# tataganesh/Query-Efficient-Approx-to-improve-OCR

Measured on AMD Instinct MI355X. Metric: patch-images/sec UNet->CRNN->CTC fwd+bwd, 32x128 grey, higher is better.
Workload: dtype f32 (GEMMs as scaled 2 x fp16 split products — three fp16 MFMAs per fp32 multiply-add — fp32 accumulate); 1 GPU; BASELINE configs[2]: full minibatch step of train_nn_area.py:212-287 — Phase A (UNet eval fwd, TopKCER k = 5 % of the minibatch, inner_limit = 4 jitter replicas fused in the batch dim, CRNN train-BN fwd+bwd, Adam(CRNN)) + Phase B (UNet train-BN -> CRNN BN-eval -> CTC mean + MSE -> backward -> Adam(UNet)) + greedy decode -> CER -> update_cer (:290-304) on synthetic POS-style 32x128 patches; batch_per_gpu=2048, global_batch=2048, full_step=True, crnn_wgrad=True, parallelism=dp1, hipgraph=False

## Files before the change

include/qea_hip.h:

```cpp
#ifndef QEA_HIP_H
#define QEA_HIP_H
#include <stddef.h>
#include <stdint.h>

#ifdef __cplusplus
extern "C" {
#endif

#define QEA_OK 0
#define QEA_ERR_INVALID (-1)
#define QEA_ERR_LAUNCH (-2)
#define QEA_ERR_WORKSPACE (-3)

int qea_version(void);
const char* qea_last_error(void);

#define QEA_PROF_CONV_IGEMM 0
#define QEA_PROF_CONV_WGRAD 1
#define QEA_PROF_LSTM_STEP 2
#define QEA_PROF_NCLASS 3
int qea_prof_enable(int klass, int on);
int qea_prof_reset(void);
int qea_prof_read(int klass, double* ms, double* flops, double* bytes, int64_t* launches);
int qea_prof_read_launches(int klass, double* ms, double* flops, int64_t capacity, int64_t* count);
#define QEA_PROF_TAG_HALO_BF3(cin_chunk, cout_group, stats) (24000 + ((cin_chunk) == 64 ? 1000 : 0) + (cout_group) + ((stats) ? 500 : 0))
int qea_prof_read_tagged(int klass, int32_t tag, double* ms, double* flops, double* bytes, int64_t* launches);
int qea_prof_read_split_bf16(int klass, double* flops);
int qea_prof_read_split_f16(int klass, double* flops);

#define QEA_MFMA_SPLIT_BF16 0
#define QEA_MFMA_F32 1
int qea_set_mfma_mode(int mode);

#define QEA_OUT_NHWC 0
#define QEA_OUT_TBC 1
#define QEA_OUT_CONVT 2

typedef struct qea_conv_desc {
  const float* x;
  const float* w;
  float* y;
  const float* scale;
  const float* bias;
  const float* mask;
  int32_t B, H, W, Cin;
  int32_t OH, OW, N;
  int32_t KH, KW, pad_h, pad_w, stride_h, stride_w;
  int32_t ldx, ldy, ldmask;
  int32_t relu;
  int32_t accumulate;
  int32_t out_mode;
  int32_t tile;
  const void* x_planes;
  const void* w_planes;
  double* stats;
  const void* w_frag_planes;
  const float* x_absmax;
  float* y_absmax;
  float* pool_y;
  int32_t ldpool;
  int32_t pool_kw;
  float* pool_absmax;
  const float* bst_y;
  int32_t ldbst;
  const double* bst_stat64;
  const float* bst_scale;
  const float* bst_shift;
} qea_conv_desc;

int qea_conv_igemm(const qea_conv_desc* d, void* stream);
int qea_conv_igemm_uses_split_bf16(const qea_conv_desc* d);
int qea_conv_igemm_stats_blocks(const qea_conv_desc* d);
int qea_conv_igemm_can_pool(const qea_conv_desc* d, int32_t kw);
int qea_conv_igemm_wants_frag_planes(const qea_conv_desc* d);
size_t qea_pack_frag_planes_f16_1x1_bytes(int32_t N, int32_t K);
int qea_pack_frag_planes_f16_1x1(const float* w, int32_t N, int32_t K, const float* wmax, void* planes, void* stream);
int qea_absmax(const float* x, int32_t ld, int64_t M, int32_t C, float* out, void* stream);
size_t qea_pack_frag_planes_f16_bytes(int32_t N, int32_t Cin);
size_t qea_split_planes_f16_bytes(int64_t M, int32_t C);
int qea_split_planes_f16(const float* x, int32_t ld, int64_t M, int32_t C, const float* xmax, void* planes, void* stream);
int qea_pack_frag_planes_f16(const float* w, int32_t N, int32_t Cin, const float* wmax, void* planes, void* stream);
size_t qea_pack_frag_planes_bytes(int32_t N, int32_t Cin);
int qea_pack_frag_planes(const float* w, int32_t N, int32_t Cin, void* planes, void* stream);

size_t qea_split_planes_bytes(int64_t M, int32_t C);
int qea_split_planes(const float* x, int32_t ld, int64_t M, int32_t C, void* planes, void* stream);

typedef struct qea_wgrad_desc {
  const float* p;
  const float* q;
  float* dw;
  void* workspace;
  size_t workspace_bytes;
  int32_t B, PH, PW, QH, QW, R, C;
  int32_t KH, KW, pad_h, pad_w, stride_h, stride_w;
  int32_t ldp, ldq;
  int32_t accumulate;
  int32_t splits;
  int32_t tile;
  const float* p_absmax;
  const float* q_absmax;
  float* dbias;
} qea_wgrad_desc;

int qea_conv_wgrad_fuses_bias(const qea_wgrad_desc* d);
int qea_conv_wgrad_wants_absmax(const qea_wgrad_desc* d);
size_t qea_conv_wgrad_workspace_bytes(const qea_wgrad_desc* d);
int qea_conv_wgrad(const qea_wgrad_desc* d, void* stream);

size_t qea_colreduce_workspace_bytes(int64_t M, int32_t C);
int qea_bn_train_stats(const float* y, int32_t ldy, int64_t M, int32_t C, const float* gamma, const float* beta,
                       float eps, float momentum, float* running_mean, float* running_var, float* mean_out,
                       float* invstd_out, float* scale_out, float* shift_out, double* stat64, void* workspace,
                       size_t workspace_bytes, void* stream);
#define QEA_BN_PARTIAL_SCRATCH_ROWS 256
int qea_bn_train_stats_from_partials(const double* partials, int32_t blocks, int64_t M, int32_t C, const float* gamma,
                                     const float* beta, float eps, float momentum, float* running_mean, float* running_var,
                                     float* mean_out, float* invstd_out, float* scale_out, float* shift_out, double* stat64,
                                     void* stream);
int qea_bn_eval_coeff(int32_t C, const float* gamma, const float* beta, const float* running_mean,
                      const float* running_var, float eps, const float* conv_bias, float* mean_out,
                      float* invstd_out, float* scale_out, float* shift_out, void* stream);
int qea_bn_apply(const float* y, int32_t ldy, float* a, int32_t lda, int64_t M, int32_t C, const float* scale,
                 const float* shift, int32_t relu, float* absmax_out, void* stream);
int qea_bn_bwd(const float* da, int32_t ldda, const float* a, int32_t lda, const float* relu_scale,
               const float* relu_shift, const float* y, int32_t ldy, int64_t M, int32_t C, const float* gamma, const float* mean, const float* invstd, const double* stat64,
               int32_t training, float* dgamma, float* dbeta, int32_t accumulate_param_grads, float* dy,
               int32_t lddy, void* workspace, size_t workspace_bytes, float* absmax_out, void* stream);
int qea_bn_bwd_pool(const float* da, int32_t ldda, const float* dpool, int32_t lddp, int32_t kw, const float* relu_scale,
                    const float* relu_shift, const float* y, int32_t ldy, int32_t B, int32_t H, int32_t W, int32_t C, const float* gamma,
                    const float* mean, const float* invstd, const double* stat64, int32_t training, float* dgamma, float* dbeta,
                    int32_t accumulate_param_grads, float* dy, int32_t lddy, void* workspace, size_t workspace_bytes, float* absmax_out,
                    void* stream);
int qea_bn_bwd_from_partials(const double* partials, int32_t blocks, const float* da, int32_t ldda, const float* relu_scale,
                             const float* relu_shift, const float* y, int32_t ldy, int64_t M, int32_t C, const float* gamma,
                             const float* mean, const float* invstd, const double* stat64, int32_t training, float* dgamma, float* dbeta,
                             int32_t accumulate_param_grads, float* dy, int32_t lddy, void* workspace, size_t workspace_bytes,
                             float* absmax_out, void* stream);
int qea_colsum(const float* x, int32_t ldx, int64_t M, int32_t C, float* out, int32_t accumulate, void* workspace,
               size_t workspace_bytes, void* stream);

int qea_maxpool_fwd(const float* x, int32_t ldx, float* y, int32_t ldy, int32_t B, int32_t H, int32_t W, int32_t C,
                    int32_t kh, int32_t kw, float* absmax_out, void* stream);
int qea_bn_apply_pool(const float* y, int32_t ldy, float* a, int32_t lda, float* pooled, int32_t ldp, int32_t B, int32_t H, int32_t W,
                      int32_t C, const float* scale, const float* shift, int32_t relu, int32_t kh, int32_t kw, float* absmax_a,
                      float* absmax_pooled, void* stream);
int qea_maxpool_bwd(const float* x, int32_t ldx, const float* dy, int32_t lddy, float* dx, int32_t lddx, int32_t B,
                    int32_t H, int32_t W, int32_t C, int32_t kh, int32_t kw, int32_t relu_mask, int32_t accumulate,
                    float* absmax_out, void* stream);

int qea_transpose2d(const float* in, float* out, int32_t R, int32_t Cc, void* stream);
int qea_filter_flip_transpose(const float* w, float* wt, int32_t Co, int32_t Ci, int32_t KH, int32_t KW, void* stream);

int qea_conv_c1_fwd(const float* x, const float* w, const float* bias, float* y, int32_t ldy, int32_t B, int32_t H,
                    int32_t W, int32_t Co, int32_t relu, void* stream);
int qea_conv_c1_fwd_pool(const float* x, const float* w, const float* bias, float* y, int32_t ldy, float* pooled, int32_t ldp, int32_t B,
                         int32_t H, int32_t W, int32_t Co, int32_t relu, float* absmax_pooled, void* stream);
size_t qea_conv_c1_pool_bwd_workspace_bytes(int32_t B, int32_t H, int32_t W, int32_t Co, int32_t need_dx);
int qea_conv_c1_pool_bwd(const float* x, const float* w, const float* bias, float* dpool, int32_t lddp, float* dw, float* db, float* dx,
                         int32_t B, int32_t H, int32_t W, int32_t Co, int32_t accumulate, void* workspace, size_t workspace_bytes, void* stream);
size_t qea_conv_c1_wgrad_workspace_bytes(int32_t B, int32_t H, int32_t W, int32_t Co);
int qea_conv_c1_wgrad(const float* x, const float* dy, int32_t lddy, float* dw, float* db, int32_t B, int32_t H,
                      int32_t W, int32_t Co, int32_t accumulate, void* workspace, size_t workspace_bytes,
                      void* stream);
int qea_conv_c1_dgrad(const float* dy, int32_t lddy, const float* w, float* dx, int32_t B, int32_t H, int32_t W,
                      int32_t Co, int32_t accumulate, void* stream);

int qea_head_fwd(const float* x, int32_t ldx, const float* w, const float* b, float* y, int64_t M, int32_t C,
                 void* stream);
size_t qea_head_bwd_workspace_bytes(int64_t M, int32_t C);
int qea_head_bwd(const float* x, int32_t ldx, const float* y, const float* dyy, const float* w, float* dx,
                 int32_t lddx, float* dw, float* db, int32_t accumulate, int64_t M, int32_t C, void* workspace,
                 size_t workspace_bytes, void* stream);

int qea_lstm_pack_whh(const float* w_hh, float* packed_fwd, float* packed_bwd, void* stream);
int qea_lstm_layer_fwd(float* gates, float* c, float* y, const float* packed_fwd, int32_t T, int32_t B, void* stream);
int qea_lstm_layer_bwd(float* gates, const float* c, const float* dy, const float* packed_bwd, float* dc_scratch,
                       int32_t T, int32_t B, void* stream);
size_t qea_lstm_pack_whh_split_bytes(void);
int qea_lstm_pack_whh_split(const float* w_hh, void* planes_fwd, void* planes_bwd, void* stream);
int qea_lstm_layer_fwd_split(float* gates, float* c, float* y, const void* planes_fwd, int32_t T, int32_t B, void* stream);
int qea_lstm_layer_bwd_split(float* gates, const float* c, const float* dy, const void* planes_bwd, float* dc_scratch,
                             int32_t T, int32_t B, void* stream);

size_t qea_lstm_seq_pack_bytes(void);
size_t qea_lstm_seq_workspace_bytes(int32_t B);
int qea_lstm_seq_pack(const float* w_hh, void* planes_fwd, void* planes_bwd, const float* w_absmax, void* stream);
int qea_lstm_seq_fwd(float* gates, float* c, float* y, const void* planes_fwd, const float* w_absmax, int32_t T, int32_t B,
                     void* workspace, float* y_absmax, void* stream);
int qea_lstm_seq_bwd(float* gates, const float* c, const float* dy, const void* planes_bwd, const float* w_absmax, int32_t T,
                     int32_t B, void* workspace, float* dgates_absmax, void* stream);
int qea_lstm_seq_timeout_index(int32_t B, int32_t backward);

typedef struct qea_wform_job {
  const float* src;
  void* dst;
  const float* amax;
  int32_t kind, a, b, c, d;
} qea_wform_job;
int qea_weight_forms_multi(const qea_wform_job* jobs, int32_t n, void* stream);

int qea_log_softmax_fwd(const float* x, int32_t ldx, float* y, int32_t ldy, int64_t M, int32_t C, void* stream);
int qea_log_softmax_bwd(const float* g, int32_t ldg, const float* lp, int32_t ldlp, float* dx, int32_t lddx, int64_t M,
                        int32_t C, int32_t Cpad, int32_t nan_scrub, void* stream);

size_t qea_ctc_workspace_bytes(int32_t T, int32_t N, int32_t S_max);
int qea_ctc_loss(const float* lp, int32_t ld_t, int32_t ld_n, const int32_t* targets, const int64_t* target_offsets,
                 const int32_t* input_lengths, const int32_t* target_lengths, int32_t T, int32_t N, int32_t C,
                 int32_t blank, int32_t S_max, int32_t reduction, float grad_scale, float* nll, float* loss,
                 float* grad, int32_t gld_t, int32_t gld_n, void* workspace, size_t workspace_bytes, void* stream);

int qea_adam_step(float* p, const float* g, float* m, float* v, int64_t n, float lr, float beta1, float beta2,
                  float eps, float weight_decay, int64_t step, float grad_scale, void* stream);
int qea_adam_step_capturable(float* p, const float* g, float* m, float* v, int64_t n, float lr, float beta1,
                             float beta2, float eps, float weight_decay, float* step, float* coef, float grad_scale,
                             void* stream);

int qea_jitter(const float* img, const float* sigma, float* out, float* noise_out, int32_t K, int32_t R, int32_t HW,
               float coef, uint64_t seed, uint64_t offset, void* stream);
int qea_jitter_apply(const float* img, const float* noise, float* out, int32_t K, int32_t R, int32_t HW, float coef,
                     void* stream);

int qea_topk_desc_stable(const float* keys, int32_t n, int32_t k, int64_t* idx_out, void* stream);

int qea_crop_pad_gather(const float* img, int32_t H, int32_t W, const int32_t* boxes, int32_t N, int32_t OH, int32_t OW,
                        float* out, void* stream);
int qea_crop_pad_scatter(const float* dout, const int32_t* boxes, int32_t N, int32_t OH, int32_t OW, float* dimg,
                         int32_t H, int32_t W, void* stream);

int qea_greedy_decode(const float* scores, int32_t ld_t, int32_t ld_n, int32_t T, int32_t N, int32_t C, int32_t blank,
                      int32_t* tokens, int32_t* lengths, void* stream);

int qea_ctc_beam_decode(const float* scores, int32_t ld_t, int32_t ld_n, int32_t T, int32_t N, int32_t C, int32_t blank, int32_t K,
                        int32_t* tokens, int32_t* lengths, double* beam_scores, void* stream);

int qea_ctc_beam_decode_lm(const float* scores, int32_t ld_t, int32_t ld_n, int32_t T, int32_t N, int32_t C, int32_t blank, int32_t K,
                           const double* lm_table, int32_t lm_context, int32_t* tokens, int32_t* lengths, double* ctc_scores,
                           double* total_scores, void* stream);

int qea_ctc_beam_decode_dfa(const float* scores, int32_t ld_t, int32_t ld_n, int32_t T, int32_t N, int32_t C, int32_t blank, int32_t K,
                            const int32_t* first, const int32_t* label, const int32_t* child, int32_t S, int32_t E, int32_t* tokens,
                            int32_t* lengths, double* beam_scores, int32_t* states, void* stream);

int qea_edit_distance(const int32_t* pred_tokens, int32_t ldp, const int32_t* pred_len, const int32_t* gt_tokens,
                      const int64_t* gt_offsets, const int32_t* gt_len, int32_t N, int32_t* out, void* stream);

size_t qea_facility_workspace_bytes(int32_t n, int32_t d);
int qea_facility_select(const double* x, int32_t n, int32_t d, int32_t k, int32_t* ranking_out, double* gain_out, void* workspace,
                        void* stream);
int qea_facility_status(const void* workspace, void* stream);

#define QEA_HISTORY_MAX_WINDOW 8
#define QEA_HISTORY_MAX_LEN 128
#define QEA_HISTORY_ATTN_MAX_TABLE 12288
#define QEA_HISTORY_ACT_SIGMOID 0
#define QEA_HISTORY_ACT_SOFTMAX 1
#define QEA_HISTORY_ACT_RELU 2
int qea_history_lev_weights(const int32_t* tokens, const int32_t* lens, const int32_t* count, int32_t n, int32_t W, float* out,
                            void* stream);
int qea_history_attn_weights(const int32_t* char_idx, const int32_t* count, int32_t n, int32_t W, int32_t n_chars,
                             const float* embedding, int32_t V1, int32_t E, const float* wq_weight, const float* wq_bias, int32_t Dq,
                             const float* coef_weight, const float* coef_bias, const float* positional_encodings, int32_t activation,
                             float* out, void* stream);

size_t qea_ctc_history_workspace_bytes(int32_t T, int32_t N, int32_t W, int32_t S_max);
int qea_ctc_history_loss(const float* lp, int32_t ld_t, int32_t ld_n, const int32_t* input_lengths, const int32_t* lens,
                         const int32_t* offs, const int32_t* chars, const int32_t* depth_n, const float* weights,
                         int32_t w_stride_n, int32_t w_stride_i, int32_t mean_by_length, int32_t T, int32_t N, int32_t C, int32_t W,
                         int32_t blank, int32_t S_max, float* loss, float* grad, int32_t gld_t, int32_t gld_n, float* nll,
                         void* workspace, size_t workspace_bytes, void* stream);

#define QEA_STRIP_ANCHOR_CENTRE 0
#define QEA_STRIP_ANCHOR_LEFT 1
int qea_strip_batch(const uint8_t* pixels, const int64_t* offset, const int32_t* h, const int32_t* w, int32_t n, const int64_t* idx,
                    int32_t B, int32_t OH, int32_t OW, int32_t anchor, const float* table, float* out, void* stream);

int qea_doc_crops_gather(const float* imgs, int32_t N, int32_t H, int32_t W, const int32_t* box, const int32_t* box_first, int32_t n_docs,
                         int32_t n_boxes, const int64_t* doc, const int32_t* strip_first, int32_t S, int32_t OH, int32_t OW, float* out,
                         void* stream);
int qea_doc_crops_scatter(const float* dout, int32_t S, int32_t OH, int32_t OW, const int32_t* box, const int32_t* box_first,
                          int32_t n_docs, int32_t n_boxes, const int64_t* doc, const int32_t* strip_first, float* dimg, int32_t N, int32_t H,
                          int32_t W, int32_t accumulate, void* stream);

#define QEA_SPREAD_WAVE_MAX_N 1536
#define QEA_SPREAD_LDS4_MAX_N 24576
#define QEA_SPREAD_LDS_MAX_N 32768
#define QEA_SPREAD_MAX_N (1 << 24)
size_t qea_spread_pick_workspace_bytes(int32_t n);
int qea_spread_pick(const float* est, int32_t n, const float* pts, int32_t k, int64_t* idx, void* workspace, void* stream);
int qea_seq_entropy(const float* lp, int64_t ld_t, int64_t ld_n, int32_t T, int32_t B, int32_t C, int32_t num_classes, float* out,
                    void* stream);

int qea_page_tiles_gather(const void* store, int32_t store_is_f32, int64_t store_elems, const int64_t* offset, const int32_t* h,
                          const int32_t* w, int32_t n_pages, const int32_t* tile, int32_t N, int32_t TH, int32_t TW, const float* table,
                          float* out, void* stream);
int qea_page_tiles_scatter(const float* tiles, int32_t N, int32_t TH, int32_t TW, const int32_t* tile, const int64_t* offset,
                           const int32_t* h, const int32_t* w, int32_t n_pages, int64_t store_elems, float* out_f32, uint8_t* out_u8,
                           void* stream);

#define QEA_BINARIZE_TILE_H 32
#define QEA_BINARIZE_TILE_W 64
#define QEA_BINARIZE_CHUNK 32768
#define QEA_BINARIZE_MAX_WINDOW 127
#define QEA_BINARIZE_MAX_PAGE_PIXELS (1 << 27)
int qea_binarize_sauvola(const void* store, int32_t store_is_f32, int64_t store_elems, const int64_t* offset, const int32_t* h,
                         const int32_t* w, int32_t n_pages, const int32_t* host_h, const int32_t* host_w, const int32_t* tile_first,
                         int32_t win, double k, double R, float* out_f32, uint8_t* out_u8, void* stream);
int qea_otsu_histogram(const void* store, int32_t store_is_f32, int64_t store_elems, const int64_t* offset, const int32_t* h,
                       const int32_t* w, int32_t n_pages, const int32_t* host_h, const int32_t* host_w, const int32_t* chunk_first,
                       uint32_t* hist, void* stream);
int qea_binarize_otsu(const void* store, int32_t store_is_f32, int64_t store_elems, const int64_t* offset, const int32_t* h,
                      const int32_t* w, int32_t n_pages, const int32_t* host_h, const int32_t* host_w, const int32_t* chunk_first,
                      const uint32_t* hist, float* out_f32, uint8_t* out_u8, int32_t* thresholds, void* stream);

#define QEA_CC_MAX_GAP 127
int qea_cc_label(const void* store, int32_t store_is_f32, int64_t store_elems, const int64_t* offset, const int32_t* h, const int32_t* w,
                 int32_t n_pages, const int32_t* host_h, const int32_t* host_w, const int32_t* tile_first, const uint8_t* ink_mask,
                 int32_t ink_max, int32_t connectivity, int32_t* labels, int32_t* area, void* stream);
int qea_cc_stats(const void* store, int32_t store_is_f32, int64_t store_elems, const int64_t* offset, const int32_t* h, const int32_t* w,
                 int32_t n_pages, const int32_t* host_h, const int32_t* host_w, const int32_t* tile_first, const int32_t* labels,
                 int32_t* area, void* stream);
int qea_cc_despeckle(const void* store, int32_t store_is_f32, int64_t store_elems, const int64_t* offset, const int32_t* h,
                     const int32_t* w, int32_t n_pages, const int32_t* host_h, const int32_t* host_w, const int32_t* tile_first,
                     const int32_t* labels, const int32_t* area, int32_t min_area, float* out_f32, uint8_t* out_u8, void* stream);
int qea_cc_smear(const void* store, int32_t store_is_f32, int64_t store_elems, const int64_t* offset, const int32_t* h, const int32_t* w,
                 int32_t n_pages, const int32_t* host_h, const int32_t* host_w, const int32_t* tile_first, const uint8_t* in_mask,
                 int32_t ink_max, int32_t gap, int32_t vertical, uint8_t* out_mask, void* stream);
int qea_cc_boxes(const void* store, int32_t store_is_f32, int64_t store_elems, const int64_t* offset, const int32_t* h, const int32_t* w,
                 int32_t n_pages, const int32_t* host_h, const int32_t* host_w, const int32_t* tile_first, const int32_t* labels,
                 const int32_t* roots, const int32_t* root_first, int32_t n_roots, int32_t* boxes, void* stream);

#define QEA_DESKEW_MAX_SIDE 32767
#define QEA_DESKEW_MAX_SLOPE 256
#define QEA_DESKEW_MAX_GAIN 10000
int qea_skew_strip_sums(const void* store, int32_t store_is_f32, int64_t store_elems, const int64_t* offset, const int32_t* h,
                        const int32_t* w, int32_t n_pages, const int32_t* host_h, const int32_t* host_w, const int32_t* ink_max_dev,
                        int32_t ink_max, uint8_t* C, void* stream);
int qea_skew_scores(const uint8_t* C, int64_t store_elems, const int64_t* offset, const int32_t* h, const int32_t* w, int32_t n_pages,
                    const int32_t* host_h, const int32_t* host_w, int32_t A, int64_t* scores, void* stream);
int qea_skew_pick(const int64_t* scores, int32_t n_pages, int32_t A, int32_t g, int32_t* slopes, void* stream);
int qea_deskew_rotate(const void* store, int32_t store_is_f32, int64_t store_elems, const int64_t* offset, const int32_t* h,
                      const int32_t* w, int32_t n_pages, const int32_t* host_h, const int32_t* host_w, const int32_t* tile_first,
                      const int32_t* slopes, const int32_t* table, int32_t A, int32_t nearest, int32_t fill, const float* norm,
                      float* out_f32, uint8_t* out_u8, void* stream);

#define QEA_WORD_STRIP_H 32
#define QEA_WORD_STRIP_MIN_W 64
#define QEA_WORD_STRIP_MAX_W 512
#define QEA_WORD_STRIP_MAX_BOXES (1 << 20)
#define QEA_WORD_STRIP_MAX_SIDE 32767
int qea_word_strips(const void* store, int32_t store_is_f32, int64_t store_elems, const int64_t* offset, const int32_t* h,
                    const int32_t* w, int32_t n_pages, const int32_t* boxes, int32_t n, int32_t OW, const float* norm, float* out,
                    void* stream);

#ifdef __cplusplus
}
#endif
#endif
```

query-efficient-approx-to-improve-ocr_amd/csrc/conv_c1.hip:

```cpp
#include "common.h"

namespace {

__global__ void conv_c1_fwd_kernel(const float* __restrict__ x, const float* __restrict__ w, const float* __restrict__ bias,
                                   float* __restrict__ y, int ldy, int B, int H, int W, int Co, int relu) {
  extern __shared__ __attribute__((aligned(16))) float sw[];
  for (int i = threadIdx.x; i < Co * 9; i += blockDim.x) {
    const int co = i / 9, tap = i - co * 9;
    sw[tap * Co + co] = w[i];
  }
  __syncthreads();
  const int cols = Co / 4;
  const long long n = (long long)B * H * W * cols;
  for (long long i = (long long)blockIdx.x * blockDim.x + threadIdx.x; i < n; i += (long long)gridDim.x * blockDim.x) {
    const int ct = (int)(i % cols);
    const long long pix = i / cols;
    const int pw = (int)(pix % W);
    const int ph = (int)((pix / W) % H);
    const float* xb = x + (pix - (long long)ph * W - pw);
    f32x4 acc = {0.f, 0.f, 0.f, 0.f};
    if (bias) acc = *reinterpret_cast<const f32x4*>(bias + ct * 4);
#pragma unroll
    for (int kh = 0; kh < 3; ++kh) {
      const int ih = ph + kh - 1;
#pragma unroll
      for (int kw = 0; kw < 3; ++kw) {
        const int iw = pw + kw - 1;
        float xv = 0.f;
        if ((unsigned)ih < (unsigned)H && (unsigned)iw < (unsigned)W) xv = xb[ih * W + iw];
        const f32x4 wv = *reinterpret_cast<const f32x4*>(sw + (kh * 3 + kw) * Co + ct * 4);
        acc += wv * xv;
      }
    }
    if (relu) {
#pragma unroll
      for (int k = 0; k < 4; ++k) acc[k] = fmaxf(acc[k], 0.f);
    }
    *reinterpret_cast<f32x4*>(y + pix * ldy + ct * 4) = acc;
  }
}

template <int COLS>
__global__ __launch_bounds__(256) void conv_c1_fwd4_kernel(const float* __restrict__ x, const float* __restrict__ w, const float* __restrict__ bias,
                                                           float* __restrict__ y, int ldy, int B, int H, int W, int relu) {
  constexpr int GPB = 256 / COLS;
  const int ct = threadIdx.x % COLS;
  f32x4 wr[9];
#pragma unroll
  for (int t = 0; t < 9; ++t)
#pragma unroll
    for (int k = 0; k < 4; ++k) wr[t][k] = w[(ct * 4 + k) * 9 + t];
  f32x4 bv = {0.f, 0.f, 0.f, 0.f};
  if (bias) bv = *reinterpret_cast<const f32x4*>(bias + ct * 4);
  const unsigned W4 = (unsigned)W >> 2;
  const unsigned groups = (unsigned)B * (unsigned)H * W4;
  const unsigned gstride = gridDim.x * GPB;
  for (unsigned g = blockIdx.x * GPB + threadIdx.x / COLS; g < groups; g += gstride) {
    const unsigned row = g / W4;
    const int pw0 = (int)(g - row * W4) * 4;
    const int ph = (int)(row % (unsigned)H);
    const float* xr = x + (size_t)row * W;
    float xv[3][6];
#pragma unroll
    for (int kh = 0; kh < 3; ++kh) {
      const bool rok = (unsigned)(ph + kh - 1) < (unsigned)H;
#pragma unroll
      for (int c = 0; c < 6; ++c) {
        const int iw = pw0 + c - 1;
        xv[kh][c] = (rok && (unsigned)iw < (unsigned)W) ? xr[(kh - 1) * W + iw] : 0.f;
      }
    }
    float* yo = y + ((size_t)row * W + pw0) * ldy + ct * 4;
#pragma unroll
    for (int j = 0; j < 4; ++j) {
      f32x4 acc = bv;
#pragma unroll
      for (int kh = 0; kh < 3; ++kh)
#pragma unroll
        for (int kw = 0; kw < 3; ++kw) acc += wr[kh * 3 + kw] * xv[kh][j + kw];
      if (relu) {
#pragma unroll
        for (int k = 0; k < 4; ++k) acc[k] = fmaxf(acc[k], 0.f);
      }
      *reinterpret_cast<f32x4*>(yo + (size_t)j * ldy) = acc;
    }
  }
}

template <int COLS>
__global__ __launch_bounds__(256) void conv_c1_fwd4_pool_kernel(const float* __restrict__ x, const float* __restrict__ w, const float* __restrict__ bias,
                                                                float* __restrict__ y, int ldy, float* __restrict__ pooled, int ldp, int B, int H,
                                                                int W, int relu, float* __restrict__ amax_p) {
  constexpr int GPB = 256 / COLS;
  const int ct = threadIdx.x % COLS;
  f32x4 wr[9];
#pragma unroll
  for (int t = 0; t < 9; ++t)
#pragma unroll
    for (int k = 0; k < 4; ++k) wr[t][k] = w[(ct * 4 + k) * 9 + t];
  f32x4 bv = {0.f, 0.f, 0.f, 0.f};
  if (bias) bv = *reinterpret_cast<const f32x4*>(bias + ct * 4);
  const unsigned W4 = (unsigned)W >> 2, H2 = (unsigned)H >> 1;
  const unsigned groups = (unsigned)B * H2 * W4;
  const unsigned gstride = gridDim.x * GPB;
  float pm = 0.f;
  for (unsigned g = blockIdx.x * GPB + threadIdx.x / COLS; g < groups; g += gstride) {
    const unsigned prow = g / W4;
    const int pw0 = (int)(g - prow * W4) * 4;
    const int ph = (int)(prow % H2) * 2;
    const size_t row = (size_t)prow * 2;
    const float* xr = x + row * W;
    float xv[4][6];
#pragma unroll
    for (int kh = 0; kh < 4; ++kh) {
      const bool rok = (unsigned)(ph + kh - 1) < (unsigned)H;
#pragma unroll
      for (int c = 0; c < 6; ++c) {
        const int iw = pw0 + c - 1;
        xv[kh][c] = (rok && (unsigned)iw < (unsigned)W) ? xr[(kh - 1) * W + iw] : 0.f;
      }
    }
    f32x4 o[2][4];
#pragma unroll
    for (int r = 0; r < 2; ++r)
#pragma unroll
      for (int j = 0; j < 4; ++j) {
        f32x4 acc = bv;
#pragma unroll
        for (int kh = 0; kh < 3; ++kh)
#pragma unroll
          for (int kw = 0; kw < 3; ++kw) acc += wr[kh * 3 + kw] * xv[r + kh][j + kw];
        if (relu) {
#pragma unroll
          for (int k = 0; k < 4; ++k) acc[k] = fmaxf(acc[k], 0.f);
        }
        o[r][j] = acc;
        if (y) *reinterpret_cast<f32x4*>(y + ((row + r) * W + pw0 + j) * ldy + ct * 4) = acc;
      }
#pragma unroll
    for (int q = 0; q < 2; ++q) {
      f32x4 m = {-INFINITY, -INFINITY, -INFINITY, -INFINITY};
#pragma unroll
      for (int r = 0; r < 2; ++r)
#pragma unroll
        for (int j = 0; j < 2; ++j)
#pragma unroll
          for (int k = 0; k < 4; ++k) {
            const float v = o[r][2 * q + j][k];
            m[k] = (v > m[k] || v != v) ? v : m[k];
          }
      *reinterpret_cast<f32x4*>(pooled + ((size_t)prow * (W >> 1) + (pw0 >> 1) + q) * ldp + ct * 4) = m;
#pragma unroll
      for (int k = 0; k < 4; ++k) pm = qea_amax_acc(pm, m[k]);
    }
  }
  qea_amax_commit_block(pm, amax_p);
}


__global__ __launch_bounds__(256) void conv_c1_wgrad_kernel(const float* __restrict__ x, const float* __restrict__ dy, int lddy, int B, int H,
                                                            int W, int Co, int rt_n, int rows_per_thread, float* __restrict__ ws) {
  extern __shared__ __attribute__((aligned(16))) float sacc[];
  const int cols = Co / 4;
  const int ct = threadIdx.x % cols, rt = threadIdx.x / cols;
  const long long M = (long long)B * H * W;
  f32x4 acc[10];
#pragma unroll
  for (int t = 0; t < 10; ++t) acc[t] = (f32x4){0.f, 0.f, 0.f, 0.f};
  if (rt < rt_n) {
    const long long r0 = (long long)blockIdx.x * rt_n * rows_per_thread;
    int pw = (int)((r0 + rt) % W);
    int ph = (int)(((r0 + rt) / W) % H);
    const int dph = rt_n / W, dpw = rt_n - dph * W;
    for (int j = 0; j < rows_per_thread; ++j) {
      const long long pix = r0 + (long long)j * rt_n + rt;
      if (pix >= M) break;
      if (j) {
        pw += dpw;
        ph += dph;
        if (pw >= W) {
          pw -= W;
          ++ph;
        }
        ph = ph >= H ? ph % H : ph;
      }
      const float* xb = x + (pix - (long long)ph * W - pw);
      const f32x4 g = *reinterpret_cast<const f32x4*>(dy + pix * lddy + ct * 4);
#pragma unroll
      for (int kh = 0; kh < 3; ++kh) {
        const int ih = ph + kh - 1;
#pragma unroll
        for (int kw = 0; kw < 3; ++kw) {
          const int iw = pw + kw - 1;
          float xv = 0.f;
          if ((unsigned)ih < (unsigned)H && (unsigned)iw < (unsigned)W) xv = xb[ih * W + iw];
          acc[kh * 3 + kw] += g * xv;
        }
      }
      acc[9] += g;
    }
#pragma unroll
    for (int t = 0; t < 10; ++t) *reinterpret_cast<f32x4*>(sacc + ((size_t)rt * 10 + t) * Co + ct * 4) = acc[t];
  }
  __syncthreads();
  for (int e = threadIdx.x; e < 10 * Co; e += blockDim.x) {
    float s = 0.f;
    for (int r = 0; r < rt_n; ++r) s += sacc[(size_t)r * 10 * Co + e];
    ws[(size_t)blockIdx.x * 10 * Co + e] = s;
  }
}

__global__ void conv_c1_wgrad_finalize_kernel(const float* __restrict__ ws, int nblk, int Co, float* dw, float* db, int accumulate) {
  const int e = blockIdx.x * (blockDim.x >> 6) + (threadIdx.x >> 6);
  if (e >= 10 * Co) return;
  const double s = qea_wave_partial_sum(ws, nblk, (size_t)10 * Co, e);
  if ((threadIdx.x & 63) != 0) return;
  const int tap = e / Co, co = e - tap * Co;
  if (tap < 9) {
    float* d = dw + co * 9 + tap;
    *d = accumulate ? *d + (float)s : (float)s;
  } else if (db) {
    db[co] = accumulate ? db[co] + (float)s : (float)s;
  }
}

template <bool NEED_T>
__global__ __launch_bounds__(256) void c1_pool_route_kernel(const float* __restrict__ x, const float* __restrict__ w, const float* __restrict__ bias,
                                                            float* __restrict__ g, int ldg, unsigned* __restrict__ idx, float* __restrict__ T, int B,
                                                            int H, int W) {
  constexpr int Co = 64;
  __shared__ __attribute__((aligned(16))) float Wl[Co * 12];
  for (int e = threadIdx.x; e < Co * 12; e += 256) {
    const int c = e / 12, t = e - c * 12;
    Wl[e] = t < 9 ? w[c * 9 + t] : (t == 9 && bias ? bias[c] : 0.f);
  }
  __syncthreads();
  const int OH = H >> 1, OW = W >> 1;
  const long long NW = (long long)B * OH * OW;
  const long long M = (long long)B * H * W;
  for (long long wi = (long long)blockIdx.x * 256 + threadIdx.x; wi < NW; wi += (long long)gridDim.x * 256) {
    const int ow = (int)(wi % OW);
    const int oh = (int)((wi / OW) % OH);
    const long long b = wi / ((long long)OW * OH);
    const int wy = oh * 2, wx = ow * 2;
    const float* xb = x + b * H * W;
    float xp[4][4];
#pragma unroll
    for (int r = 0; r < 4; ++r)
#pragma unroll
      for (int c = 0; c < 4; ++c) {
        const int iy = wy + r - 1, ix = wx + c - 1;
        xp[r][c] = ((unsigned)iy < (unsigned)H && (unsigned)ix < (unsigned)W) ? xb[iy * W + ix] : 0.f;
      }
    float Tacc[4][9];
    if (NEED_T) {
#pragma unroll
      for (int j = 0; j < 4; ++j)
#pragma unroll
        for (int t = 0; t < 9; ++t) Tacc[j][t] = 0.f;
    }
    float* grow = g + wi * ldg;
    unsigned* irow = idx + wi * (Co / 4);
#pragma unroll 2
    for (int c4 = 0; c4 < Co / 4; ++c4) {
      f32x4 gv = *reinterpret_cast<const f32x4*>(grow + c4 * 4);
      unsigned packed = 0;
#pragma unroll
      for (int k = 0; k < 4; ++k) {
        const float* wc = Wl + (c4 * 4 + k) * 12;
        const f32x4 w0 = *reinterpret_cast<const f32x4*>(wc), w1 = *reinterpret_cast<const f32x4*>(wc + 4), w2 = *reinterpret_cast<const f32x4*>(wc + 8);
        const float wt[9] = {w0[0], w0[1], w0[2], w0[3], w1[0], w1[1], w1[2], w1[3], w2[0]};
        float m = -INFINITY;
        int arg = 0;
#pragma unroll
        for (int j = 0; j < 4; ++j) {
          const int jr = j >> 1, jc = j & 1;
          float acc = w2[1];
#pragma unroll
          for (int kh = 0; kh < 3; ++kh)
#pragma unroll
            for (int kw = 0; kw < 3; ++kw) acc = __builtin_fmaf(wt[kh * 3 + kw], xp[jr + kh][jc + kw], acc);
          const float v = fmaxf(acc, 0.f);
          if (v > m || v != v) {
            m = v;
            arg = j;
          }
        }
        const float gm = (m > 0.f) ? gv[k] : 0.f;
        gv[k] = gm;
        packed |= (unsigned)arg << (8 * k);
        if (NEED_T) {
#pragma unroll
          for (int j = 0; j < 4; ++j) {
            const float mj = (arg == j) ? gm : 0.f;
#pragma unroll
            for (int t = 0; t < 9; ++t) Tacc[j][t] = __builtin_fmaf(mj, wt[t], Tacc[j][t]);
          }
        }
      }
      *reinterpret_cast<f32x4*>(grow + c4 * 4) = gv;
      irow[c4] = packed;
    }
    if (NEED_T) {
      const long long p0 = (b * H + wy) * (long long)W + wx;
#pragma unroll
      for (int t = 0; t < 9; ++t) {
        float* Tp = T + (long long)t * M;
        *reinterpret_cast<float2*>(Tp + p0) = make_float2(Tacc[0][t], Tacc[1][t]);
        *reinterpret_cast<float2*>(Tp + p0 + W) = make_float2(Tacc[2][t], Tacc[3][t]);
      }
    }
  }
}

__global__ __launch_bounds__(256) void c1_pool_wgrad_kernel(const float* __restrict__ x, const float* __restrict__ g, int ldg,
                                                            const unsigned char* __restrict__ idx, int B, int H, int W, int win_per_wave,
                                                            float* __restrict__ ws) {
  constexpr int Co = 64;
  const int c = threadIdx.x & 63;
  const int wave = __builtin_amdgcn_readfirstlane(threadIdx.x >> 6);
  const int OH = H >> 1, OW = W >> 1;
  const long long NW = (long long)B * OH * OW;
  const long long w0 = ((long long)blockIdx.x * 4 + wave) * win_per_wave;
  long long w1 = w0 + win_per_wave;
  if (w1 > NW) w1 = NW;
  float acc[10];
#pragma unroll
  for (int t = 0; t < 10; ++t) acc[t] = 0.f;
  float gq[4];
  int aq[4];
  auto load_group = [&](long long wi, float* gv, int* av) {
#pragma unroll
    for (int k = 0; k < 4; ++k) {
      gv[k] = g[(wi + k) * ldg + c];
      av[k] = idx[(wi + k) * Co + c];
    }
  };
  if (w0 < w1) load_group(w0, gq, aq);
  for (long long wi = w0; wi < w1; wi += 4) {
    float gn[4] = {0.f, 0.f, 0.f, 0.f};
    int an[4] = {0, 0, 0, 0};
    if (wi + 4 < w1) load_group(wi + 4, gn, an);
    const int ow = (int)(wi % OW);
    const int oh = (int)((wi / OW) % OH);
    const long long b = wi / ((long long)OW * OH);
    const int wy = oh * 2, wx = ow * 2;
    const float* xb = x + b * H * W;
    float xr[4][10];
#pragma unroll
    for (int r = 0; r < 4; ++r)
#pragma unroll
      for (int cc = 0; cc < 10; ++cc) {
        const int iy = wy + r - 1, ix = wx + cc - 1;
        xr[r][cc] = ((unsigned)iy < (unsigned)H && (unsigned)ix < (unsigned)W) ? xb[iy * W + ix] : 0.f;
      }
#pragma unroll
    for (int k = 0; k < 4; ++k) {
      const float gm = gq[k];
      const int arg = aq[k];
#pragma unroll
      for (int j = 0; j < 4; ++j) {
        const float mj = (arg == j) ? gm : 0.f;
        const int jr = j >> 1, jc = j & 1;
#pragma unroll
        for (int kh = 0; kh < 3; ++kh)
#pragma unroll
          for (int kw = 0; kw < 3; ++kw) acc[kh * 3 + kw] = __builtin_fmaf(mj, xr[jr + kh][2 * k + jc + kw], acc[kh * 3 + kw]);
      }
      acc[9] += gm;
    }
#pragma unroll
    for (int k = 0; k < 4; ++k) {
      gq[k] = gn[k];
      aq[k] = an[k];
    }
  }
  float* o = ws + ((size_t)blockIdx.x * 4 + wave) * 10 * Co;
#pragma unroll
  for (int t = 0; t < 10; ++t) o[t * Co + c] = acc[t];
}

__global__ void c1_pool_dx_kernel(const float* __restrict__ T, float* __restrict__ dx, int B, int H, int W, int accumulate) {
  const long long M = (long long)B * H * W;
  for (long long p = (long long)blockIdx.x * blockDim.x + threadIdx.x; p < M; p += (long long)gridDim.x * blockDim.x) {
    const int px = (int)(p % W);
    const int py = (int)((p / W) % H);
    float s = 0.f;
#pragma unroll
    for (int kh = 0; kh < 3; ++kh) {
      const int qy = py + 1 - kh;
#pragma unroll
      for (int kw = 0; kw < 3; ++kw) {
        const int qx = px + 1 - kw;
        if ((unsigned)qy < (unsigned)H && (unsigned)qx < (unsigned)W) s += T[(long long)(kh * 3 + kw) * M + p + (long long)(1 - kh) * W + (1 - kw)];
      }
    }
    dx[p] = accumulate ? dx[p] + s : s;
  }
}

template <int COLS>
__global__ __launch_bounds__(256) void conv_c1_dgrad_kernel(const float* __restrict__ dy, int lddy, const float* __restrict__ w,
                                                            float* __restrict__ dx, int B, int H, int W, int accumulate) {
  constexpr int Co = COLS * 4;
  const int ct = threadIdx.x % COLS;
  f32x4 wr[9];
#pragma unroll
  for (int t = 0; t < 9; ++t)
#pragma unroll
    for (int k = 0; k < 4; ++k) wr[t][k] = w[(ct * 4 + k) * 9 + t];
  const long long M = (long long)B * H * W;
  const long long n = M * COLS;
  const long long stride = (long long)gridDim.x * blockDim.x;
  for (long long i = (long long)blockIdx.x * blockDim.x + threadIdx.x; i < (n + stride - 1) / stride * stride; i += stride) {
    const bool live = i < n;
    const long long pix = live ? i / COLS : 0;
    const int pw = (int)(pix % W);
    const int ph = (int)((pix / W) % H);
    float s = 0.f;
    if (live) {
#pragma unroll
      for (int kh = 0; kh < 3; ++kh) {
        const int oh = ph + 1 - kh;
#pragma unroll
        for (int kw = 0; kw < 3; ++kw) {
          const int ow = pw + 1 - kw;
          if ((unsigned)oh < (unsigned)H && (unsigned)ow < (unsigned)W) {
            const f32x4 g = *reinterpret_cast<const f32x4*>(dy + (pix + (long long)(oh - ph) * W + (ow - pw)) * lddy + ct * 4);
            const f32x4 wv = wr[kh * 3 + kw];
            s += g[0] * wv[0] + g[1] * wv[1] + g[2] * wv[2] + g[3] * wv[3];
          }
        }
      }
    }
#pragma unroll
    for (int o = COLS / 2; o > 0; o >>= 1) s += __shfl_xor(s, o, 64);
    if (live && ct == 0) dx[pix] = accumulate ? dx[pix] + s : s;
  }
  (void)Co;
}

constexpr int C1D_TH = 8, C1D_TW = 64, C1D_HW = C1D_TW + 2, C1D_HP = (C1D_TH + 2) * C1D_HW;
template <int COLS>
__global__ __launch_bounds__(256) void conv_c1_dgrad_tile_kernel(const float* __restrict__ dy, int lddy, const float* __restrict__ w,
                                                                 float* __restrict__ dx, int H, int W, int tiles_x, int tiles_y, int accumulate) {
  __shared__ float T[C1D_HP * 9];
  __shared__ __attribute__((aligned(16))) float Wl[COLS * 9 * 4];
  for (int e = threadIdx.x; e < COLS * 36; e += 256) {
    const int k = e & 3, t = (e >> 2) % 9, c4 = e / 36;
    Wl[e] = w[(c4 * 4 + k) * 9 + t];
  }
  int bid = blockIdx.x;
  const int tx = bid % tiles_x;
  bid /= tiles_x;
  const int ty = bid % tiles_y;
  const int b = bid / tiles_y;
  const int x0 = tx * C1D_TW, y0 = ty * C1D_TH;
  const float* dyb = dy + (size_t)b * H * W * lddy;
  __syncthreads();
  for (int hq = threadIdx.x; hq < C1D_HP; hq += 256) {
    const int hy = hq / C1D_HW, hx = hq - hy * C1D_HW;
    const int iy = y0 + hy - 1, ix = x0 + hx - 1;
    float d[9];
#pragma unroll
    for (int t = 0; t < 9; ++t) d[t] = 0.f;
    if ((unsigned)iy < (unsigned)H && (unsigned)ix < (unsigned)W) {
      const float* row = dyb + ((size_t)iy * W + ix) * lddy;
#pragma unroll 4
      for (int c4 = 0; c4 < COLS; ++c4) {
        const f32x4 g = *reinterpret_cast<const f32x4*>(row + c4 * 4);
#pragma unroll
        for (int t = 0; t < 9; ++t) {
          const f32x4 wv = *reinterpret_cast<const f32x4*>(Wl + (c4 * 9 + t) * 4);
          d[t] += g[0] * wv[0] + g[1] * wv[1] + g[2] * wv[2] + g[3] * wv[3];
        }
      }
    }
#pragma unroll
    for (int t = 0; t < 9; ++t) T[hq * 9 + t] = d[t];
  }
  __syncthreads();
  float* dxb = dx + (size_t)b * H * W;
  for (int q = threadIdx.x; q < C1D_TH * C1D_TW; q += 256) {
    const int qy = q / C1D_TW, qx = q - qy * C1D_TW;
    const int oy = y0 + qy, ox = x0 + qx;
    if (oy >= H || ox >= W) continue;
    float sacc = 0.f;
#pragma unroll
    for (int kh = 0; kh < 3; ++kh)
#pragma unroll
      for (int kw = 0; kw < 3; ++kw) sacc += T[((qy + 2 - kh) * C1D_HW + qx + 2 - kw) * 9 + kh * 3 + kw];
    float* o = dxb + (size_t)oy * W + ox;
    *o = accumulate ? *o + sacc : sacc;
  }
}

template <int COLS>
__global__ __launch_bounds__(256) void head_fwd_kernel(const float* __restrict__ x, int ldx, const float* __restrict__ w,
                                                       const float* __restrict__ b, float* __restrict__ y, long long M) {
  const int ct = threadIdx.x % COLS;
  const f32x4 wv = *reinterpret_cast<const f32x4*>(w + ct * 4);
  const float bias = b[0];
  const long long n = M * COLS;
  const long long stride = (long long)gridDim.x * blockDim.x;
  for (long long i = (long long)blockIdx.x * blockDim.x + threadIdx.x; i < (n + stride - 1) / stride * stride; i += stride) {
    const bool live = i < n;
    const long long pix = live ? i / COLS : 0;
    float s = 0.f;
    if (live) {
      const f32x4 xv = *reinterpret_cast<const f32x4*>(x + pix * ldx + ct * 4);
      s = xv[0] * wv[0] + xv[1] * wv[1] + xv[2] * wv[2] + xv[3] * wv[3];
    }
#pragma unroll
    for (int o = COLS / 2; o > 0; o >>= 1) s += __shfl_xor(s, o, 64);
    if (live && ct == 0) y[pix] = 1.f / (1.f + expf(-(s + bias)));
  }
}

template <int COLS>
__global__ __launch_bounds__(256) void head_bwd_kernel(const float* __restrict__ x, int ldx, const float* __restrict__ y,
                                                       const float* __restrict__ dyy, const float* __restrict__ w, float* __restrict__ dx,
                                                       int lddx, long long M, double* __restrict__ ws) {
  constexpr int C = COLS * 4;
  constexpr int RT = 256 / COLS;
  __shared__ double sred[RT][C + 1];
  const int ct = threadIdx.x % COLS, rt = threadIdx.x / COLS;
  const f32x4 wv = *reinterpret_cast<const f32x4*>(w + ct * 4);
  double aw[4] = {0, 0, 0, 0}, ab = 0;
  const long long n = M * COLS;
  for (long long i = (long long)blockIdx.x * blockDim.x + threadIdx.x; i < n; i += (long long)gridDim.x * blockDim.x) {
    const long long pix = i / COLS;
    const float yy = y[pix];
    const float dz = dyy[pix] * yy * (1.f - yy);
    const f32x4 xv = *reinterpret_cast<const f32x4*>(x + pix * ldx + ct * 4);
    *reinterpret_cast<f32x4*>(dx + pix * lddx + ct * 4) = wv * dz;
#pragma unroll
    for (int k = 0; k < 4; ++k) aw[k] += (double)(dz * xv[k]);
    if (ct == 0) ab += (double)dz;
  }
#pragma unroll
  for (int k = 0; k < 4; ++k) sred[rt][ct * 4 + k] = aw[k];
  if (ct == 0) sred[rt][C] = ab;
  __syncthreads();
  for (int e = threadIdx.x; e <= C; e += blockDim.x) {
    double s = 0;
    for (int r = 0; r < RT; ++r) s += sred[r][e];
    ws[(size_t)blockIdx.x * (C + 1) + e] = s;
  }
}

__global__ void head_bwd_finalize_kernel(const double* __restrict__ ws, int nblk, int C, float* dw, float* db, int accumulate) {
  const int e = blockIdx.x * (blockDim.x >> 6) + (threadIdx.x >> 6);
  if (e > C) return;
  const double s = qea_wave_partial_sum(ws, nblk, (size_t)C + 1, e);
  if ((threadIdx.x & 63) != 0) return;
  float* d = (e < C) ? dw + e : db;
  *d = accumulate ? *d + (float)s : (float)s;
}

}

extern "C" int qea_conv_c1_fwd(const float* x, const float* w, const float* bias, float* y, int32_t ldy, int32_t B, int32_t H, int32_t W,
                               int32_t Co, int32_t relu, void* stream) {
  QEA_REQUIRE(x && w && y && B > 0 && H > 0 && W > 0 && Co > 0 && Co % 4 == 0 && ldy % 4 == 0 && ldy >= Co, "qea_conv_c1_fwd: bad arguments");
  const long long n = (long long)B * H * W * (Co / 4);
  if (W % 4 == 0 && (long long)B * H * W < 0x7fffffffLL && (Co == 32 || Co == 64 || Co == 128) && ((uintptr_t)y & 15) == 0 &&
      (!bias || ((uintptr_t)bias & 15) == 0)) {
    const int cols = Co / 4;
    const long long groups = (long long)B * H * (W / 4);
    const int grid = (int)((groups + 256 / cols - 1) / (256 / cols) > 16384 ? 16384 : (groups + 256 / cols - 1) / (256 / cols));
    hipStream_t s = (hipStream_t)stream;
    if (Co == 32) hipLaunchKernelGGL(conv_c1_fwd4_kernel<8>, dim3(grid), dim3(256), 0, s, x, w, bias, y, ldy, B, H, W, relu);
    else if (Co == 64) hipLaunchKernelGGL(conv_c1_fwd4_kernel<16>, dim3(grid), dim3(256), 0, s, x, w, bias, y, ldy, B, H, W, relu);
    else hipLaunchKernelGGL(conv_c1_fwd4_kernel<32>, dim3(grid), dim3(256), 0, s, x, w, bias, y, ldy, B, H, W, relu);
    QEA_CHECK_LAUNCH();
    return QEA_OK;
  }
  hipLaunchKernelGGL(conv_c1_fwd_kernel, dim3(qea_grid_for(n, 8192)), dim3(256), (size_t)Co * 9 * sizeof(float), (hipStream_t)stream, x, w, bias, y,
                     ldy, B, H, W, Co, relu);
  QEA_CHECK_LAUNCH();
  return QEA_OK;
}

extern "C" int qea_conv_c1_fwd_pool(const float* x, const float* w, const float* bias, float* y, int32_t ldy, float* pooled, int32_t ldp, int32_t B,
                                    int32_t H, int32_t W, int32_t Co, int32_t relu, float* absmax_pooled, void* stream) {
  QEA_REQUIRE(x && w && pooled && B > 0 && H > 0 && W > 0 && H % 2 == 0 && W % 4 == 0 && (Co == 32 || Co == 64 || Co == 128) && ldy % 4 == 0 &&
                  ldy >= Co && ldp % 4 == 0 && ldp >= Co && (long long)B * H * W < 0x7fffffffLL,
              "qea_conv_c1_fwd_pool: needs H %% 2 == 0, W %% 4 == 0, Co in {32, 64, 128}, fewer than 2^31 pixels");
  QEA_REQUIRE(((uintptr_t)y & 15) == 0 && ((uintptr_t)pooled & 15) == 0 && (!bias || ((uintptr_t)bias & 15) == 0), "qea_conv_c1_fwd_pool: 16-byte alignment");
  const int cols = Co / 4;
  const long long groups = (long long)B * (H / 2) * (W / 4);
  const long long blocks = (groups + 256 / cols - 1) / (256 / cols);
  const int grid = (int)(blocks > 16384 ? 16384 : blocks);
  hipStream_t s = (hipStream_t)stream;
  if (Co == 32) hipLaunchKernelGGL(conv_c1_fwd4_pool_kernel<8>, dim3(grid), dim3(256), 0, s, x, w, bias, y, ldy, pooled, ldp, B, H, W, relu, absmax_pooled);
  else if (Co == 64) hipLaunchKernelGGL(conv_c1_fwd4_pool_kernel<16>, dim3(grid), dim3(256), 0, s, x, w, bias, y, ldy, pooled, ldp, B, H, W, relu, absmax_pooled);
  else hipLaunchKernelGGL(conv_c1_fwd4_pool_kernel<32>, dim3(grid), dim3(256), 0, s, x, w, bias, y, ldy, pooled, ldp, B, H, W, relu, absmax_pooled);
  QEA_CHECK_LAUNCH();
  return QEA_OK;
}

static int c1_wgrad_geom(long long M, int Co, int* rt_n, int* rows_per_thread) {
  const int cols = Co / 4;
  *rt_n = 256 / cols;
  long long rpt = M / ((long long)(*rt_n) * 4096);
  rpt = rpt < 32 ? 32 : (rpt > 128 ? 128 : rpt);
  *rows_per_thread = (int)rpt;
  const long long per_block = (long long)(*rt_n) * rpt;
  return (int)((M + per_block - 1) / per_block);
}

extern "C" size_t qea_conv_c1_wgrad_workspace_bytes(int32_t B, int32_t H, int32_t W, int32_t Co) {
  if (B <= 0 || H <= 0 || W <= 0 || Co <= 0 || Co % 4 || Co / 4 > 256) return 0;
  int rt, rpt;
  const int grid = c1_wgrad_geom((long long)B * H * W, Co, &rt, &rpt);
  return (size_t)grid * 10 * Co * sizeof(float);
}

extern "C" int qea_conv_c1_wgrad(const float* x, const float* dy, int32_t lddy, float* dw, float* db, int32_t B, int32_t H, int32_t W,
                                 int32_t Co, int32_t accumulate, void* workspace, size_t workspace_bytes, void* stream) {
  QEA_REQUIRE(x && dy && dw && B > 0 && H > 0 && W > 0 && Co > 0 && Co % 4 == 0 && Co / 4 <= 256 && lddy % 4 == 0, "qea_conv_c1_wgrad: bad arguments");
  int rt, rpt;
  const int grid = c1_wgrad_geom((long long)B * H * W, Co, &rt, &rpt);
  QEA_REQUIRE(workspace && workspace_bytes >= (size_t)grid * 10 * Co * sizeof(float), "qea_conv_c1_wgrad: workspace too small");
  const size_t lds = (size_t)rt * 10 * Co * sizeof(float);
  QEA_REQUIRE(lds <= 160 * 1024, "qea_conv_c1_wgrad: Co too large for LDS");
  static bool attr = false;
  if (!attr) {
    (void)hipFuncSetAttribute((const void*)conv_c1_wgrad_kernel, hipFuncAttributeMaxDynamicSharedMemorySize, 160 * 1024);
    attr = true;
  }
  hipStream_t s = (hipStream_t)stream;
  hipLaunchKernelGGL(conv_c1_wgrad_kernel, dim3(grid), dim3(256), lds, s, x, dy, lddy, B, H, W, Co, rt, rpt, (float*)workspace);
  hipLaunchKernelGGL(conv_c1_wgrad_finalize_kernel, dim3(qea_cdiv(10 * Co, 4)), dim3(256), 0, s, (const float*)workspace, grid, Co, dw, db,
                     accumulate);
  QEA_CHECK_LAUNCH();
  return QEA_OK;
}

static long long c1pb_win_per_wave(long long NW) {
  long long wpw = (NW + 4 * 2048 - 1) / (4 * 2048);
  wpw = wpw < 16 ? 16 : wpw;
  return (wpw + 3) & ~3LL;
}

extern "C" size_t qea_conv_c1_pool_bwd_workspace_bytes(int32_t B, int32_t H, int32_t W, int32_t Co, int32_t need_dx) {
  if (B <= 0 || H <= 0 || W <= 0 || Co != 64 || H % 2 || W % 8) return 0;
  const long long NW = (long long)B * (H / 2) * (W / 2);
  const long long wpw = c1pb_win_per_wave(NW);
  const long long blocks = (NW + 4 * wpw - 1) / (4 * wpw);
  size_t b = ((size_t)NW * 64 + 255) & ~(size_t)255;
  if (need_dx) b += (size_t)9 * B * H * W * sizeof(float);
  b += (size_t)blocks * 4 * 640 * sizeof(float);
  return b;
}

extern "C" int qea_conv_c1_pool_bwd(const float* x, const float* w, const float* bias, float* dpool, int32_t lddp, float* dw, float* db, float* dx,
                                    int32_t B, int32_t H, int32_t W, int32_t Co, int32_t accumulate, void* workspace, size_t workspace_bytes,
                                    void* stream) {
  QEA_REQUIRE(x && w && dpool && B > 0 && H > 0 && W > 0 && H % 2 == 0 && W % 8 == 0 && Co == 64 && lddp % 4 == 0 && lddp >= Co &&
                  ((uintptr_t)dpool & 15) == 0 && ((uintptr_t)x & 7) == 0 && (long long)B * H * W < 0x7fffffffLL,
              "qea_conv_c1_pool_bwd: needs Co == 64, even H, W %% 8 == 0, 16-byte aligned dpool rows, fewer than 2^31 pixels");
  const size_t need = qea_conv_c1_pool_bwd_workspace_bytes(B, H, W, Co, dx != nullptr);
  QEA_REQUIRE(workspace && workspace_bytes >= need && ((uintptr_t)workspace & 255) == 0, "qea_conv_c1_pool_bwd: workspace of %zu bytes (256-byte aligned) required", need);
  const long long NW = (long long)B * (H / 2) * (W / 2);
  const long long wpw = c1pb_win_per_wave(NW);
  const long long blocks = (NW + 4 * wpw - 1) / (4 * wpw);
  char* wsb = (char*)workspace;
  unsigned* idx = (unsigned*)wsb;
  wsb += ((size_t)NW * 64 + 255) & ~(size_t)255;
  float* T = nullptr;
  if (dx) {
    T = (float*)wsb;
    wsb += (size_t)9 * B * H * W * sizeof(float);
  }
  float* part = (float*)wsb;
  hipStream_t s = (hipStream_t)stream;
  const int rgrid = qea_grid_for(NW, 8192);
  if (dx) hipLaunchKernelGGL(c1_pool_route_kernel<true>, dim3(rgrid), dim3(256), 0, s, x, w, bias, dpool, lddp, idx, T, B, H, W);
  else hipLaunchKernelGGL(c1_pool_route_kernel<false>, dim3(rgrid), dim3(256), 0, s, x, w, bias, dpool, lddp, idx, T, B, H, W);
  if (dw) {
    hipLaunchKernelGGL(c1_pool_wgrad_kernel, dim3((unsigned)blocks), dim3(256), 0, s, x, (const float*)dpool, lddp, (const unsigned char*)idx, B, H, W,
                       (int)wpw, part);
    hipLaunchKernelGGL(conv_c1_wgrad_finalize_kernel, dim3(qea_cdiv(10 * Co, 4)), dim3(256), 0, s, (const float*)part, (int)(blocks * 4), Co, dw, db,
                       accumulate);
  }
  if (dx) hipLaunchKernelGGL(c1_pool_dx_kernel, dim3(qea_grid_for((long long)B * H * W, 8192)), dim3(256), 0, s, (const float*)T, dx, B, H, W, 0);
  QEA_CHECK_LAUNCH();
  return QEA_OK;
}

extern "C" int qea_conv_c1_dgrad(const float* dy, int32_t lddy, const float* w, float* dx, int32_t B, int32_t H, int32_t W, int32_t Co,
                                 int32_t accumulate, void* stream) {
  QEA_REQUIRE(dy && w && dx && B > 0 && H > 0 && W > 0 && lddy % 4 == 0, "qea_conv_c1_dgrad: bad arguments");
  const long long n = (long long)B * H * W * (Co / 4);
  const int grid = qea_grid_for(n, 8192);
  hipStream_t s = (hipStream_t)stream;
  const int tiles_x = qea_cdiv(W, C1D_TW), tiles_y = qea_cdiv(H, C1D_TH);
  const long long tiles = (long long)B * tiles_x * tiles_y;
  if (tiles < 0x7fffffffLL && (Co == 32 || Co == 64 || Co == 128) && ((uintptr_t)dy & 15) == 0) {
    if (Co == 32) hipLaunchKernelGGL(conv_c1_dgrad_tile_kernel<8>, dim3((unsigned)tiles), dim3(256), 0, s, dy, lddy, w, dx, H, W, tiles_x, tiles_y, accumulate);
    else if (Co == 64) hipLaunchKernelGGL(conv_c1_dgrad_tile_kernel<16>, dim3((unsigned)tiles), dim3(256), 0, s, dy, lddy, w, dx, H, W, tiles_x, tiles_y, accumulate);
    else hipLaunchKernelGGL(conv_c1_dgrad_tile_kernel<32>, dim3((unsigned)tiles), dim3(256), 0, s, dy, lddy, w, dx, H, W, tiles_x, tiles_y, accumulate);
    QEA_CHECK_LAUNCH();
    return QEA_OK;
  }
  switch (Co) {
    case 32: hipLaunchKernelGGL(conv_c1_dgrad_kernel<8>, dim3(grid), dim3(256), 0, s, dy, lddy, w, dx, B, H, W, accumulate); break;
    case 64: hipLaunchKernelGGL(conv_c1_dgrad_kernel<16>, dim3(grid), dim3(256), 0, s, dy, lddy, w, dx, B, H, W, accumulate); break;
    case 128: hipLaunchKernelGGL(conv_c1_dgrad_kernel<32>, dim3(grid), dim3(256), 0, s, dy, lddy, w, dx, B, H, W, accumulate); break;
    default: qea_set_error("qea_conv_c1_dgrad: Co=%d not in {32,64,128}", Co); return QEA_ERR_INVALID;
  }
  QEA_CHECK_LAUNCH();
  return QEA_OK;
}

extern "C" int qea_head_fwd(const float* x, int32_t ldx, const float* w, const float* b, float* y, int64_t M, int32_t C, void* stream) {
  QEA_REQUIRE(x && w && b && y && M > 0 && ldx % 4 == 0, "qea_head_fwd: bad arguments");
  const int grid = qea_grid_for(M * (C / 4), 8192);
  hipStream_t s = (hipStream_t)stream;
  switch (C) {
    case 32: hipLaunchKernelGGL(head_fwd_kernel<8>, dim3(grid), dim3(256), 0, s, x, ldx, w, b, y, (long long)M); break;
    case 64: hipLaunchKernelGGL(head_fwd_kernel<16>, dim3(grid), dim3(256), 0, s, x, ldx, w, b, y, (long long)M); break;
    default: qea_set_error("qea_head_fwd: C=%d not in {32,64}", C); return QEA_ERR_INVALID;
  }
  QEA_CHECK_LAUNCH();
  return QEA_OK;
}

extern "C" size_t qea_head_bwd_workspace_bytes(int64_t M, int32_t C) {
  if (M <= 0 || C <= 0) return 0;
  return (size_t)qea_grid_for(M * (C / 4), 1024) * (C + 1) * sizeof(double);
}

extern "C" int qea_head_bwd(const float* x, int32_t ldx, const float* y, const float* dyy, const float* w, float* dx, int32_t lddx,
                            float* dw, float* db, int32_t accumulate, int64_t M, int32_t C, void* workspace, size_t workspace_bytes,
                            void* stream) {
  QEA_REQUIRE(x && y && dyy && w && dx && dw && db && M > 0 && ldx % 4 == 0 && lddx % 4 == 0, "qea_head_bwd: bad arguments");
  const int grid = qea_grid_for(M * (C / 4), 1024);
  QEA_REQUIRE(workspace && workspace_bytes >= (size_t)grid * (C + 1) * sizeof(double), "qea_head_bwd: workspace too small");
  hipStream_t s = (hipStream_t)stream;
  switch (C) {
    case 32: hipLaunchKernelGGL(head_bwd_kernel<8>, dim3(grid), dim3(256), 0, s, x, ldx, y, dyy, w, dx, lddx, (long long)M, (double*)workspace); break;
    case 64: hipLaunchKernelGGL(head_bwd_kernel<16>, dim3(grid), dim3(256), 0, s, x, ldx, y, dyy, w, dx, lddx, (long long)M, (double*)workspace); break;
    default: qea_set_error("qea_head_bwd: C=%d not in {32,64}", C); return QEA_ERR_INVALID;
  }
  hipLaunchKernelGGL(head_bwd_finalize_kernel, dim3(qea_cdiv(C + 1, 4)), dim3(256), 0, s, (const double*)workspace, grid, C, dw, db, accumulate);
  QEA_CHECK_LAUNCH();
  return QEA_OK;
}
```

query-efficient-approx-to-improve-ocr_amd/csrc/norm_pool.hip:

```cpp
#include "common.h"

namespace {

constexpr int RED_THREADS = 256;

struct ColGeom {
  int cols;
  int rt;
  int grid;
  int rows_per_block;
};

ColGeom col_geom(long long M, int C) {
  ColGeom g;
  g.cols = C / 4;
  g.rt = RED_THREADS / g.cols;
  if (g.rt < 1) g.rt = 1;
  long long want = (M + (long long)g.rt * 16 - 1) / ((long long)g.rt * 16);
  if (want > 1024) want = 1024;
  if (want < 1) want = 1;
  g.grid = (int)want;
  g.rows_per_block = (int)((M + g.grid - 1) / g.grid);
  g.grid = (int)((M + g.rows_per_block - 1) / g.rows_per_block);
  return g;
}

__device__ __forceinline__ float bn_affine(float v, float sc, float sh) { return __fmaf_rn(v, sc, sh); }

__device__ __forceinline__ float bn_masked_dz(float d, bool has_a, float av, bool remask = false, float yv = 0.f, float sc = 0.f, float sh = 0.f) {
  if (has_a) return av > 0.f ? d : 0.f;
  if (remask) return bn_affine(yv, sc, sh) > 0.f ? d : 0.f;
  return d;
}
__device__ __forceinline__ void bn_bwd_acc(double& s0, double& s1, float dz, float yv, double mu, double is) {
  s0 += (double)dz;
  s1 += (double)dz * (((double)yv - mu) * is);
}
__device__ __forceinline__ float bn_dy(double c0, double c1, double c2, float dz, float yv) {
  return (float)(c0 * (double)dz + (c1 * (double)yv + c2));
}
__device__ __forceinline__ void bn_load_mu_is(const double* __restrict__ stat64, const float* __restrict__ mean, const float* __restrict__ invstd,
                                              int C, int c4, double (&mu)[4], double (&is)[4]) {
#pragma unroll
  for (int k = 0; k < 4; ++k) {
    mu[k] = stat64 ? stat64[c4 + k] : (double)mean[c4 + k];
    is[k] = stat64 ? stat64[C + c4 + k] : (double)invstd[c4 + k];
  }
}
__device__ __forceinline__ void block_partials_store(double* sred, const double (&s0)[4], const double (&s1)[4], int rt, int rt_n, int ct, int C,
                                                     double* __restrict__ ws) {
  if (rt < rt_n) {
#pragma unroll
    for (int k = 0; k < 4; ++k) {
      sred[((size_t)rt * C + ct * 4 + k) * 2 + 0] = s0[k];
      sred[((size_t)rt * C + ct * 4 + k) * 2 + 1] = s1[k];
    }
  }
  __syncthreads();
  for (int c = threadIdx.x; c < C; c += blockDim.x) {
    double t0 = 0, t1 = 0;
    for (int r = 0; r < rt_n; ++r) {
      t0 += sred[((size_t)r * C + c) * 2 + 0];
      t1 += sred[((size_t)r * C + c) * 2 + 1];
    }
    ws[((size_t)blockIdx.x * C + c) * 2 + 0] = t0;
    ws[((size_t)blockIdx.x * C + c) * 2 + 1] = t1;
  }
}

__device__ __forceinline__ bool pool_take(float v, float m) { return v > m || v != v; }
__device__ __forceinline__ long long pool_window_origin(long long op, int OW, int W, int kh, int kw) {
  return (op / OW) * kh * W + (op % OW) * kw;
}

template <int MODE>
__global__ __launch_bounds__(RED_THREADS) void colreduce_kernel(const float* __restrict__ x, int ldx, const float* __restrict__ a,
                                                                  int lda, const float* __restrict__ y, int ldy,
                                                                  const float* __restrict__ mean, const float* __restrict__ invstd,
                                                                  const double* __restrict__ stat64, const float* __restrict__ msc,
                                                                  const float* __restrict__ msh, long long M, int C,
                                                                  int rows_per_block, int rt_n, double* __restrict__ ws) {
  extern __shared__ __attribute__((aligned(16))) double sred[];
  const int cols = C / 4;
  const int ct = threadIdx.x % cols, rt = threadIdx.x / cols;
  double s0[4] = {0, 0, 0, 0}, s1[4] = {0, 0, 0, 0};
  if (rt < rt_n) {
    const long long r0 = (long long)blockIdx.x * rows_per_block;
    long long r1 = r0 + rows_per_block;
    if (r1 > M) r1 = M;
    double mu[4] = {0, 0, 0, 0}, is[4] = {0, 0, 0, 0};
    const f32x4 zero = {0.f, 0.f, 0.f, 0.f};
    f32x4 sc = zero, sh = zero;
    const bool remask = !a && msc;
    if (MODE == 1) {
      bn_load_mu_is(stat64, mean, invstd, C, ct * 4, mu, is);
      if (remask) {
        sc = *reinterpret_cast<const f32x4*>(msc + ct * 4);
        sh = *reinterpret_cast<const f32x4*>(msh + ct * 4);
      }
    }
#pragma unroll 2
    for (long long r = r0 + rt; r < r1; r += rt_n) {
      const f32x4 v = *reinterpret_cast<const f32x4*>(x + r * ldx + ct * 4);
      if (MODE == 0) {
#pragma unroll
        for (int k = 0; k < 4; ++k) {
          s0[k] += (double)v[k];
          s1[k] += (double)v[k] * (double)v[k];
        }
      } else if (MODE == 1) {
        const f32x4 yv = *reinterpret_cast<const f32x4*>(y + r * ldy + ct * 4);
        const f32x4 av = a ? *reinterpret_cast<const f32x4*>(a + r * lda + ct * 4) : zero;
#pragma unroll
        for (int k = 0; k < 4; ++k)
          bn_bwd_acc(s0[k], s1[k], bn_masked_dz(v[k], a, av[k], remask, yv[k], sc[k], sh[k]), yv[k], mu[k], is[k]);
      } else {
#pragma unroll
        for (int k = 0; k < 4; ++k) s0[k] += (double)v[k];
      }
    }
  }
  block_partials_store(sred, s0, s1, rt, rt_n, ct, C, ws);
}

__device__ __forceinline__ void partial_sums(const double* __restrict__ ws, int nblk, int C, int c, double& s, double& q) {
  const int lane = threadIdx.x & 63;
  double a = 0, b = 0;
  for (int k = lane; k < nblk; k += 64) {
    a += ws[((size_t)k * C + c) * 2 + 0];
    b += ws[((size_t)k * C + c) * 2 + 1];
  }
  s = qea_wave_sum_d(a);
  q = qea_wave_sum_d(b);
}

__global__ void bn_stats_finalize_kernel(const double* __restrict__ ws, int nblk, int C, long long M, const float* __restrict__ gamma,
                                         const float* __restrict__ beta, float eps, float momentum, float* running_mean,
                                         float* running_var, float* mean_out, float* invstd_out, float* scale_out, float* shift_out,
                                         double* stat64) {
  const int c = blockIdx.x * (blockDim.x >> 6) + (threadIdx.x >> 6);
  if (c >= C) return;
  double s, q;
  partial_sums(ws, nblk, C, c, s, q);
  if ((threadIdx.x & 63) != 0) return;
  const double mean = s / (double)M;
  double var = q / (double)M - mean * mean;
  if (var < 0) var = 0;
  const double invstd_d = 1.0 / sqrt(var + (double)eps);
  if (stat64) {
    stat64[c] = mean;
    stat64[C + c] = invstd_d;
  }
  const float invstd = (float)invstd_d;
  const float g = gamma ? gamma[c] : 1.f, b = beta ? beta[c] : 0.f;
  mean_out[c] = (float)mean;
  invstd_out[c] = invstd;
  scale_out[c] = g * invstd;
  shift_out[c] = b - (float)mean * g * invstd;
  if (running_mean) {
    const double unb = (M > 1) ? var * (double)M / (double)(M - 1) : var;
    running_mean[c] = (1.f - momentum) * running_mean[c] + momentum * (float)mean;
    running_var[c] = (1.f - momentum) * running_var[c] + momentum * (float)unb;
  }
}

__global__ void bn_eval_coeff_kernel(int C, const float* __restrict__ gamma, const float* __restrict__ beta,
                                     const float* __restrict__ rmean, const float* __restrict__ rvar, float eps,
                                     const float* __restrict__ conv_bias, float* mean_out, float* invstd_out, float* scale_out,
                                     float* shift_out) {
  const int c = blockIdx.x * blockDim.x + threadIdx.x;
  if (c >= C) return;
  const float invstd = 1.f / sqrtf(rvar[c] + eps);
  const float g = gamma ? gamma[c] : 1.f, b = beta ? beta[c] : 0.f;
  mean_out[c] = rmean[c];
  invstd_out[c] = invstd;
  scale_out[c] = g * invstd;
  shift_out[c] = b + ((conv_bias ? conv_bias[c] : 0.f) - rmean[c]) * g * invstd;
}

__global__ void colsum_finalize_kernel(const double* __restrict__ ws, int nblk, int C, float* out, int accumulate) {
  const int c = blockIdx.x * (blockDim.x >> 6) + (threadIdx.x >> 6);
  if (c >= C) return;
  double s, q;
  partial_sums(ws, nblk, C, c, s, q);
  if ((threadIdx.x & 63) != 0) return;
  out[c] = accumulate ? out[c] + (float)s : (float)s;
}

__global__ void bn_bwd_finalize_kernel(const double* __restrict__ ws, int nblk, int C, long long M, const float* __restrict__ gamma,
                                       const float* __restrict__ mean, const float* __restrict__ invstd,
                                       const double* __restrict__ stat64, int training, float* dgamma, float* dbeta, int accumulate,
                                       double* k0, double* k1, double* k2) {
  const int c = blockIdx.x * (blockDim.x >> 6) + (threadIdx.x >> 6);
  if (c >= C) return;
  double s, q;
  partial_sums(ws, nblk, C, c, s, q);
  if ((threadIdx.x & 63) != 0) return;
  if (dgamma) dgamma[c] = accumulate ? dgamma[c] + (float)q : (float)q;
  if (dbeta) dbeta[c] = accumulate ? dbeta[c] + (float)s : (float)s;
  const double g = gamma ? (double)gamma[c] : 1.0;
  const double is = stat64 ? stat64[C + c] : (double)invstd[c];
  const double mu = stat64 ? stat64[c] : (double)mean[c];
  const double m0 = training ? s / (double)M : 0.0;
  const double m1 = training ? q / (double)M : 0.0;
  k0[c] = g * is;
  k1[c] = -g * is * is * m1;
  k2[c] = g * is * (mu * is * m1 - m0);
}

__global__ void bn_apply_kernel(const float* __restrict__ y, int ldy, float* __restrict__ a, int lda, long long M, int C,
                                const float* __restrict__ scale, const float* __restrict__ shift, int relu, float* __restrict__ amax) {
  const int cols = C / 4;
  const long long n = M * cols;
  float am = 0.f;
  for (long long i = (long long)blockIdx.x * blockDim.x + threadIdx.x; i < n; i += (long long)gridDim.x * blockDim.x) {
    const long long r = i / cols;
    const int ct = (int)(i - r * cols);
    const f32x4 v = *reinterpret_cast<const f32x4*>(y + r * ldy + ct * 4);
    const f32x4 sc = *reinterpret_cast<const f32x4*>(scale + ct * 4);
    const f32x4 sh = *reinterpret_cast<const f32x4*>(shift + ct * 4);
    f32x4 o;
#pragma unroll
    for (int k = 0; k < 4; ++k) {
      o[k] = bn_affine(v[k], sc[k], sh[k]);
      if (relu) o[k] = fmaxf(o[k], 0.f);
      am = qea_amax_acc(am, o[k]);
    }
    *reinterpret_cast<f32x4*>(a + r * lda + ct * 4) = o;
  }
  qea_amax_commit_block(am, amax);
}

__global__ __launch_bounds__(RED_THREADS) void bn_bwd_apply_kernel(const float* __restrict__ da, int ldda, const float* __restrict__ a, int lda,
                                                                    const float* __restrict__ y, int ldy, float* __restrict__ dy, int lddy,
                                                                    long long M, int C, const float* __restrict__ msc,
                                                                    const float* __restrict__ msh, const double* __restrict__ k0,
                                                                    const double* __restrict__ k1, const double* __restrict__ k2,
                                                                    int rows_per_block, int rt_n, float* __restrict__ amax) {
  const int cols = C / 4;
  const int ct = threadIdx.x % cols, rt = threadIdx.x / cols;
  const bool idle = rt >= rt_n;
  float am = 0.f;
  double c0[4], c1[4], c2[4];
#pragma unroll
  for (int k = 0; k < 4; ++k) {
    c0[k] = k0[ct * 4 + k];
    c1[k] = k1[ct * 4 + k];
    c2[k] = k2[ct * 4 + k];
  }
  f32x4 sc = {0.f, 0.f, 0.f, 0.f}, sh = {0.f, 0.f, 0.f, 0.f};
  const bool remask = !a && msc;
  if (remask) {
    sc = *reinterpret_cast<const f32x4*>(msc + ct * 4);
    sh = *reinterpret_cast<const f32x4*>(msh + ct * 4);
  }
  const long long r0 = (long long)blockIdx.x * rows_per_block;
  long long r1 = r0 + rows_per_block;
  if (r1 > M) r1 = M;
  auto one = [&](long long r, f32x4 dz, const f32x4 yv, const f32x4 av) {
    f32x4 o;
#pragma unroll
    for (int k = 0; k < 4; ++k) {
      o[k] = bn_dy(c0[k], c1[k], c2[k], bn_masked_dz(dz[k], a, av[k], remask, yv[k], sc[k], sh[k]), yv[k]);
      am = qea_amax_acc(am, o[k]);
    }
    *reinterpret_cast<f32x4*>(dy + r * lddy + ct * 4) = o;
  };
  const f32x4 zero = {0.f, 0.f, 0.f, 0.f};
  long long r = idle ? r1 : r0 + rt;
  for (; r + rt_n < r1; r += 2 * rt_n) {
    const long long rb = r + rt_n;
    const f32x4 dza = *reinterpret_cast<const f32x4*>(da + r * ldda + ct * 4);
    const f32x4 dzb = *reinterpret_cast<const f32x4*>(da + rb * ldda + ct * 4);
    const f32x4 ya = *reinterpret_cast<const f32x4*>(y + r * ldy + ct * 4);
    const f32x4 yb = *reinterpret_cast<const f32x4*>(y + rb * ldy + ct * 4);
    f32x4 aa = zero, ab = zero;
    if (a) {
      aa = *reinterpret_cast<const f32x4*>(a + r * lda + ct * 4);
      ab = *reinterpret_cast<const f32x4*>(a + rb * lda + ct * 4);
    }
    one(r, dza, ya, aa);
    one(rb, dzb, yb, ab);
  }
  if (r < r1) {
    const f32x4 dza = *reinterpret_cast<const f32x4*>(da + r * ldda + ct * 4);
    const f32x4 ya = *reinterpret_cast<const f32x4*>(y + r * ldy + ct * 4);
    const f32x4 aa = a ? *reinterpret_cast<const f32x4*>(a + r * lda + ct * 4) : zero;
    one(r, dza, ya, aa);
  }
  qea_amax_commit_block(am, amax);
}

template <int KW, bool APPLY>
__global__ __launch_bounds__(RED_THREADS) void bn_bwd_pool_kernel(const float* __restrict__ da, int ldda, const float* __restrict__ dpool, int lddp,
                                                                   const float* __restrict__ y, int ldy, float* __restrict__ dy, int lddy, int B, int H,
                                                                   int W, int C, const float* __restrict__ msc, const float* __restrict__ msh,
                                                                   const float* __restrict__ mean, const float* __restrict__ invstd,
                                                                   const double* __restrict__ stat64, const double* __restrict__ k0,
                                                                   const double* __restrict__ k1, const double* __restrict__ k2,
                                                                   int win_per_block, int rt_n, double* __restrict__ ws, float* __restrict__ amax) {
  extern __shared__ __attribute__((aligned(16))) double sred[];
  constexpr int NP = 2 * KW;
  const int cols = C / 4;
  const int ct = threadIdx.x % cols, rt = threadIdx.x / cols;
  const int OH = H / 2, OW = W / KW;
  const long long NWIN = (long long)B * OH * OW;
  const bool idle = rt >= rt_n;
  float am = 0.f;
  double s0[4] = {0, 0, 0, 0}, s1[4] = {0, 0, 0, 0};
  double mu[4] = {0, 0, 0, 0}, is[4] = {0, 0, 0, 0}, c0[4] = {0, 0, 0, 0}, c1[4] = {0, 0, 0, 0}, c2[4] = {0, 0, 0, 0};
  const f32x4 sc = *reinterpret_cast<const f32x4*>(msc + ct * 4);
  const f32x4 sh = *reinterpret_cast<const f32x4*>(msh + ct * 4);
  if constexpr (APPLY) {
#pragma unroll
    for (int k = 0; k < 4; ++k) {
      c0[k] = k0[ct * 4 + k];
      c1[k] = k1[ct * 4 + k];
      c2[k] = k2[ct * 4 + k];
    }
  } else {
    bn_load_mu_is(stat64, mean, invstd, C, ct * 4, mu, is);
  }
  const long long w0 = (long long)blockIdx.x * win_per_block;
  long long w1 = w0 + win_per_block;
  if (w1 > NWIN) w1 = NWIN;
  for (long long wi = idle ? w1 : w0 + rt; wi < w1; wi += rt_n) {
    const long long r00 = pool_window_origin(wi, OW, W, 2, KW);
    long long rows[NP];
#pragma unroll
    for (int j = 0; j < NP; ++j) rows[j] = r00 + (j / KW) * (long long)W + (j % KW);
    f32x4 yv[NP], dv[NP];
#pragma unroll
    for (int j = 0; j < NP; ++j) {
      yv[j] = *reinterpret_cast<const f32x4*>(y + rows[j] * ldy + ct * 4);
      const f32x4 zero = {0.f, 0.f, 0.f, 0.f};
      dv[j] = da ? *reinterpret_cast<const f32x4*>(da + rows[j] * ldda + ct * 4) : zero;
    }
    const f32x4 g = *reinterpret_cast<const f32x4*>(dpool + wi * lddp + ct * 4);
    f32x4 m = {-INFINITY, -INFINITY, -INFINITY, -INFINITY};
    int arg[4] = {0, 0, 0, 0};
    f32x4 av[NP];
#pragma unroll
    for (int j = 0; j < NP; ++j)
#pragma unroll
      for (int k = 0; k < 4; ++k) {
        const float v = fmaxf(bn_affine(yv[j][k], sc[k], sh[k]), 0.f);
        av[j][k] = v;
        if (pool_take(v, m[k])) {
          m[k] = v;
          arg[k] = j;
        }
      }
#pragma unroll
    for (int j = 0; j < NP; ++j) {
      f32x4 o;
#pragma unroll
      for (int k = 0; k < 4; ++k) {
        const float d = bn_masked_dz((arg[k] == j ? g[k] : 0.f) + dv[j][k], true, av[j][k]);
        if (APPLY) {
          o[k] = bn_dy(c0[k], c1[k], c2[k], d, yv[j][k]);
          am = qea_amax_acc(am, o[k]);
        } else {
          bn_bwd_acc(s0[k], s1[k], d, yv[j][k], mu[k], is[k]);
        }
      }
      if (APPLY) *reinterpret_cast<f32x4*>(dy + rows[j] * lddy + ct * 4) = o;
    }
  }
  if constexpr (APPLY) {
    qea_amax_commit_block(am, amax);
  } else {
    block_partials_store(sred, s0, s1, rt, rt_n, ct, C, ws);
  }
}

__global__ void maxpool_fwd_kernel(const float* __restrict__ x, int ldx, float* __restrict__ y, int ldy, int B, int H, int W, int C,
                                   int kh, int kw, float* __restrict__ amax) {
  const int OH = H / kh, OW = W / kw, cols = C / 4;
  const long long n = (long long)B * OH * OW * cols;
  float am = 0.f;
  for (long long i = (long long)blockIdx.x * blockDim.x + threadIdx.x; i < n; i += (long long)gridDim.x * blockDim.x) {
    const int ct = (int)(i % cols);
    const long long op = i / cols;
    const long long ip0 = pool_window_origin(op, OW, W, kh, kw);
    f32x4 m = {-INFINITY, -INFINITY, -INFINITY, -INFINITY};
    for (int i2 = 0; i2 < kh; ++i2)
      for (int j2 = 0; j2 < kw; ++j2) {
        const f32x4 v = *reinterpret_cast<const f32x4*>(x + (ip0 + i2 * W + j2) * ldx + ct * 4);
#pragma unroll
        for (int k = 0; k < 4; ++k) m[k] = pool_take(v[k], m[k]) ? v[k] : m[k];
      }
    *reinterpret_cast<f32x4*>(y + op * ldy + ct * 4) = m;
#pragma unroll
    for (int k = 0; k < 4; ++k) am = qea_amax_acc(am, m[k]);
  }
  qea_amax_commit_block(am, amax);
}

__global__ void bn_apply_pool_kernel(const float* __restrict__ y, int ldy, float* __restrict__ a, int lda, float* __restrict__ pooled, int ldp,
                                     int B, int H, int W, int C, const float* __restrict__ scale, const float* __restrict__ shift, int relu,
                                     int kh, int kw, float* __restrict__ amax_a, float* __restrict__ amax_p) {
  const int OH = H / kh, OW = W / kw, cols = C / 4;
  const long long n = (long long)B * OH * OW * cols;
  float am = 0.f, pm = 0.f;
  for (long long i = (long long)blockIdx.x * blockDim.x + threadIdx.x; i < n; i += (long long)gridDim.x * blockDim.x) {
    const int ct = (int)(i % cols);
    const long long op = i / cols;
    const long long ip0 = pool_window_origin(op, OW, W, kh, kw);
    const f32x4 sc = *reinterpret_cast<const f32x4*>(scale + ct * 4);
    const f32x4 sh = *reinterpret_cast<const f32x4*>(shift + ct * 4);
    f32x4 m = {-INFINITY, -INFINITY, -INFINITY, -INFINITY};
    for (int i2 = 0; i2 < kh; ++i2)
      for (int j2 = 0; j2 < kw; ++j2) {
        const long long ip = ip0 + i2 * W + j2;
        const f32x4 v = *reinterpret_cast<const f32x4*>(y + ip * ldy + ct * 4);
        f32x4 o;
#pragma unroll
        for (int k = 0; k < 4; ++k) {
          o[k] = bn_affine(v[k], sc[k], sh[k]);
          if (relu) o[k] = fmaxf(o[k], 0.f);
          am = qea_amax_acc(am, o[k]);
          m[k] = pool_take(o[k], m[k]) ? o[k] : m[k];
        }
        *reinterpret_cast<f32x4*>(a + ip * lda + ct * 4) = o;
      }
    *reinterpret_cast<f32x4*>(pooled + op * ldp + ct * 4) = m;
#pragma unroll
    for (int k = 0; k < 4; ++k) pm = qea_amax_acc(pm, m[k]);
  }
  qea_amax_commit_block(am, amax_a);
  qea_amax_commit_block(pm, amax_p);
}

__global__ void maxpool_bwd_kernel(const float* __restrict__ x, int ldx, const float* __restrict__ dy, int lddy, float* __restrict__ dx,
                                   int lddx, int B, int H, int W, int C, int kh, int kw, int relu_mask, int accumulate,
                                   float* __restrict__ amax) {
  const int OH = H / kh, OW = W / kw, cols = C / 4;
  const long long n = (long long)B * OH * OW * cols;
  float am = 0.f;
  for (long long i = (long long)blockIdx.x * blockDim.x + threadIdx.x; i < n; i += (long long)gridDim.x * blockDim.x) {
    const int ct = (int)(i % cols);
    const long long op = i / cols;
    const long long ip0 = pool_window_origin(op, OW, W, kh, kw);
    f32x4 m = {-INFINITY, -INFINITY, -INFINITY, -INFINITY};
    int arg[4] = {0, 0, 0, 0};
    for (int i2 = 0; i2 < kh; ++i2)
      for (int j2 = 0; j2 < kw; ++j2) {
        const f32x4 v = *reinterpret_cast<const f32x4*>(x + (ip0 + i2 * W + j2) * ldx + ct * 4);
#pragma unroll
        for (int k = 0; k < 4; ++k)
          if (pool_take(v[k], m[k])) {
            m[k] = v[k];
            arg[k] = i2 * kw + j2;
          }
      }
    const f32x4 g = *reinterpret_cast<const f32x4*>(dy + op * lddy + ct * 4);
    for (int i2 = 0; i2 < kh; ++i2)
      for (int j2 = 0; j2 < kw; ++j2) {
        f32x4 o;
#pragma unroll
        for (int k = 0; k < 4; ++k) {
          float t = (arg[k] == i2 * kw + j2) ? g[k] : 0.f;
          if (relu_mask && !(m[k] > 0.f)) t = 0.f;
          o[k] = t;
        }
        f32x4* dst = reinterpret_cast<f32x4*>(dx + (ip0 + i2 * W + j2) * lddx + ct * 4);
        if (accumulate) o += *dst;
        *dst = o;
#pragma unroll
        for (int k = 0; k < 4; ++k) am = qea_amax_acc(am, o[k]);
      }
  }
  qea_amax_commit_block(am, amax);
}

__global__ void transpose_kernel(const float* __restrict__ in, float* __restrict__ out, int R, int Cc) {
  __shared__ float t[32][33];
  const int bx = blockIdx.x * 32, by = blockIdx.y * 32;
  const int tx = threadIdx.x & 31, ty = threadIdx.x >> 5;
  for (int j = ty; j < 32; j += 8) {
    const int r = by + j, c = bx + tx;
    t[j][tx] = (r < R && c < Cc) ? in[(size_t)r * Cc + c] : 0.f;
  }
  __syncthreads();
  for (int j = ty; j < 32; j += 8) {
    const int c = bx + j, r = by + tx;
    if (c < Cc && r < R) out[(size_t)c * R + r] = t[tx][j];
  }
}

size_t ws_need(int rows, int consts, int C) { return ((size_t)rows * 2 + consts) * C * sizeof(double); }

int check_cols(const char* who, long long M, int C, int strides, const void* ws, size_t ws_bytes, int consts, ColGeom* g) {
  QEA_REQUIRE(M > 0 && C > 0 && C % 4 == 0 && C / 4 <= RED_THREADS, "%s: need C %% 4 == 0 and C <= %d (C=%d)", who, 4 * RED_THREADS, C);
  QEA_REQUIRE(strides % 4 == 0, "%s: strides must be multiples of 4", who);
  const int rows = g ? (*g = col_geom(M, C)).grid : 0;
  QEA_REQUIRE(ws && ws_bytes >= ws_need(rows, consts, C), "%s: workspace too small (%zu bytes)", who, ws_need(rows, consts, C));
  return QEA_OK;
}

struct ApplyGeom {
  unsigned grid;
  int per_block;
};
ApplyGeom apply_geom(long long items, int rt, int per_thread) {
  long long grid = (items + (long long)rt * per_thread - 1) / ((long long)rt * per_thread);
  if (grid > 4096) grid = 4096;
  if (grid < 1) grid = 1;
  const int per = (int)((items + grid - 1) / grid);
  return {(unsigned)((items + per - 1) / per), per};
}

}

extern "C" size_t qea_colreduce_workspace_bytes(int64_t M, int32_t C) {
  if (M <= 0 || C <= 0 || C % 4) return 0;
  return ws_need(col_geom(M, C).grid, 3, C);
}

extern "C" int qea_bn_train_stats(const float* y, int32_t ldy, int64_t M, int32_t C, const float* gamma, const float* beta, float eps,
                                  float momentum, float* running_mean, float* running_var, float* mean_out, float* invstd_out,
                                  float* scale_out, float* shift_out, double* stat64, void* workspace, size_t workspace_bytes,
                                  void* stream) {
  QEA_REQUIRE(y && mean_out && invstd_out && scale_out && shift_out, "qea_bn_train_stats: null pointer");
  QEA_REQUIRE(((uintptr_t)y & 15) == 0, "qea_bn_train_stats: alignment");
  ColGeom g;
  if (int rc = check_cols("qea_bn_train_stats", M, C, ldy, workspace, workspace_bytes, 0, &g)) return rc;
  hipStream_t s = (hipStream_t)stream;
  const size_t lds = (size_t)g.rt * C * 2 * sizeof(double);
  hipLaunchKernelGGL(colreduce_kernel<0>, dim3(g.grid), dim3(RED_THREADS), lds, s, y, ldy, nullptr, 0, nullptr, 0, nullptr, nullptr,
                     nullptr, nullptr, nullptr, (long long)M, C, g.rows_per_block, g.rt, (double*)workspace);
  hipLaunchKernelGGL(bn_stats_finalize_kernel, dim3(qea_cdiv(C, 4)), dim3(256), 0, s, (const double*)workspace, g.grid, C,
                     (long long)M, gamma, beta, eps, momentum, running_mean, running_var, mean_out, invstd_out, scale_out, shift_out,
                     stat64);
  QEA_CHECK_LAUNCH();
  return QEA_OK;
}

__global__ __launch_bounds__(256) void partials_reduce_kernel(const double* __restrict__ ws, int nblk, int C, int per, double* __restrict__ out) {
  extern __shared__ __attribute__((aligned(16))) double sp[];
  const int b0 = blockIdx.x * per;
  const int b1 = min(nblk, b0 + per);
  for (int cbase = 0; cbase < C; cbase += 256) {
    const int cw = min(256, C - cbase);
    const int st = cw < 256 ? 256 / cw : 1;
    const int c = threadIdx.x % cw, stripe = threadIdx.x / cw;
    double a = 0, b = 0;
    if (stripe < st) {
      for (int k = b0 + stripe; k < b1; k += st) {
        const double* src = ws + ((size_t)k * C + cbase + c) * 2;
        a += src[0];
        b += src[1];
      }
      sp[((size_t)stripe * cw + c) * 2 + 0] = a;
      sp[((size_t)stripe * cw + c) * 2 + 1] = b;
    }
    __syncthreads();
    if (threadIdx.x < cw) {
      double t0 = 0, t1 = 0;
      for (int r = 0; r < st; ++r) {
        t0 += sp[((size_t)r * cw + threadIdx.x) * 2 + 0];
        t1 += sp[((size_t)r * cw + threadIdx.x) * 2 + 1];
      }
      out[((size_t)blockIdx.x * C + cbase + threadIdx.x) * 2 + 0] = t0;
      out[((size_t)blockIdx.x * C + cbase + threadIdx.x) * 2 + 1] = t1;
    }
    __syncthreads();
  }
}

namespace {

void fold_partials(const double* partials, int blocks, int C, hipStream_t s, const double** src, int* nblk) {
  *src = partials;
  *nblk = blocks;
  if (blocks <= QEA_BN_PARTIAL_SCRATCH_ROWS * 2) return;
  const int per = qea_cdiv(blocks, QEA_BN_PARTIAL_SCRATCH_ROWS);
  *nblk = qea_cdiv(blocks, per);
  double* scratch = const_cast<double*>(partials) + (size_t)blocks * C * 2;
  hipLaunchKernelGGL(partials_reduce_kernel, dim3(*nblk), dim3(256), (size_t)256 * 2 * sizeof(double), s, partials, blocks, C, per, scratch);
  *src = scratch;
}

struct BnChannels {
  const float *gamma, *mean, *invstd;
  const double* stat64;
  int training;
  float *dgamma, *dbeta;
  int accumulate;
};

template <class Apply>
int bn_bwd_tail(const double* rows, int nrows, double* k, long long M, int C, const BnChannels& ch, hipStream_t s, Apply apply) {
  double *k0 = k, *k1 = k0 + C, *k2 = k1 + C;
  hipLaunchKernelGGL(bn_bwd_finalize_kernel, dim3(qea_cdiv(C, 4)), dim3(256), 0, s, rows, nrows, C, M, ch.gamma, ch.mean, ch.invstd, ch.stat64,
                     ch.training, ch.dgamma, ch.dbeta, ch.accumulate, k0, k1, k2);
  apply(k0, k1, k2);
  QEA_CHECK_LAUNCH();
  return QEA_OK;
}

void bn_bwd_apply_launch(const float* da, int ldda, const float* a, int lda, const float* y, int ldy, float* dy, int lddy, long long M, int C,
                         const float* relu_scale, const float* relu_shift, const double* k0, const double* k1, const double* k2, int rt,
                         float* absmax_out, hipStream_t s) {
  const ApplyGeom ag = apply_geom(M, rt, 8);
  hipLaunchKernelGGL(bn_bwd_apply_kernel, dim3(ag.grid), dim3(RED_THREADS), 0, s, da, ldda, a, lda, y, ldy, dy, lddy, M, C, relu_scale, relu_shift,
                     k0, k1, k2, ag.per_block, rt, absmax_out);
}

}

extern "C" int qea_bn_train_stats_from_partials(const double* partials, int32_t blocks, int64_t M, int32_t C, const float* gamma,
                                                const float* beta, float eps, float momentum, float* running_mean, float* running_var,
                                                float* mean_out, float* invstd_out, float* scale_out, float* shift_out, double* stat64,
                                                void* stream) {
  QEA_REQUIRE(partials && blocks > 0 && M > 0 && C > 0 && mean_out && invstd_out && scale_out && shift_out,
              "qea_bn_train_stats_from_partials: bad arguments");
  hipStream_t s = (hipStream_t)stream;
  const double* src;
  int nblk;
  fold_partials(partials, blocks, C, s, &src, &nblk);
  hipLaunchKernelGGL(bn_stats_finalize_kernel, dim3(qea_cdiv(C, 4)), dim3(256), 0, s, src, nblk, C, (long long)M,
                     gamma, beta, eps, momentum, running_mean, running_var, mean_out, invstd_out, scale_out, shift_out, stat64);
  QEA_CHECK_LAUNCH();
  return QEA_OK;
}

extern "C" int qea_bn_eval_coeff(int32_t C, const float* gamma, const float* beta, const float* running_mean, const float* running_var,
                                 float eps, const float* conv_bias, float* mean_out, float* invstd_out, float* scale_out,
                                 float* shift_out, void* stream) {
  QEA_REQUIRE(C > 0 && running_mean && running_var && mean_out && invstd_out && scale_out && shift_out, "qea_bn_eval_coeff: null pointer");
  hipLaunchKernelGGL(bn_eval_coeff_kernel, dim3(qea_cdiv(C, 128)), dim3(128), 0, (hipStream_t)stream, C, gamma, beta, running_mean,
                     running_var, eps, conv_bias, mean_out, invstd_out, scale_out, shift_out);
  QEA_CHECK_LAUNCH();
  return QEA_OK;
}

extern "C" int qea_bn_apply(const float* y, int32_t ldy, float* a, int32_t lda, int64_t M, int32_t C, const float* scale,
                            const float* shift, int32_t relu, float* absmax_out, void* stream) {
  QEA_REQUIRE(y && a && scale && shift && M > 0 && C > 0 && C % 4 == 0 && ldy % 4 == 0 && lda % 4 == 0, "qea_bn_apply: bad arguments");
  hipLaunchKernelGGL(bn_apply_kernel, dim3(qea_grid_for(M * (C / 4))), dim3(256), 0, (hipStream_t)stream, y, ldy, a, lda, (long long)M, C,
                     scale, shift, relu, absmax_out);
  QEA_CHECK_LAUNCH();
  return QEA_OK;
}

extern "C" int qea_bn_bwd(const float* da, int32_t ldda, const float* a, int32_t lda, const float* relu_scale, const float* relu_shift,
                          const float* y, int32_t ldy, int64_t M, int32_t C, const float* gamma, const float* mean, const float* invstd, const double* stat64, int32_t training,
                          float* dgamma, float* dbeta, int32_t accumulate_param_grads, float* dy, int32_t lddy, void* workspace,
                          size_t workspace_bytes, float* absmax_out, void* stream) {
  QEA_REQUIRE(da && y && mean && invstd && dy, "qea_bn_bwd: null pointer");
  QEA_REQUIRE(!a || !relu_scale, "qea_bn_bwd: give the ReLU mask either as a or as relu_scale/relu_shift, not both");
  QEA_REQUIRE((relu_scale == nullptr) == (relu_shift == nullptr), "qea_bn_bwd: relu_scale and relu_shift go together");
  ColGeom g;
  if (int rc = check_cols("qea_bn_bwd", M, C, ldda | ldy | lddy | (a ? lda : 0), workspace, workspace_bytes, 3, &g)) return rc;
  hipStream_t s = (hipStream_t)stream;
  double* ws = (double*)workspace;
  const size_t lds = (size_t)g.rt * C * 2 * sizeof(double);
  hipLaunchKernelGGL(colreduce_kernel<1>, dim3(g.grid), dim3(RED_THREADS), lds, s, da, ldda, a, lda, y, ldy, mean, invstd, stat64,
                     relu_scale, relu_shift, (long long)M, C, g.rows_per_block, g.rt, ws);
  return bn_bwd_tail(ws, g.grid, ws + (size_t)g.grid * C * 2, M, C, {gamma, mean, invstd, stat64, training, dgamma, dbeta, accumulate_param_grads}, s,
                     [&](const double* k0, const double* k1, const double* k2) {
                       bn_bwd_apply_launch(da, ldda, a, lda, y, ldy, dy, lddy, M, C, relu_scale, relu_shift, k0, k1, k2, g.rt, absmax_out, s);
                     });
}

extern "C" int qea_bn_bwd_pool(const float* da, int32_t ldda, const float* dpool, int32_t lddp, int32_t kw, const float* relu_scale,
                               const float* relu_shift, const float* y, int32_t ldy, int32_t B, int32_t H, int32_t W, int32_t C,
                               const float* gamma, const float* mean, const float* invstd, const double* stat64, int32_t training, float* dgamma,
                               float* dbeta, int32_t accumulate_param_grads, float* dy, int32_t lddy, void* workspace, size_t workspace_bytes,
                               float* absmax_out, void* stream) {
  QEA_REQUIRE(dpool && y && mean && invstd && dy && relu_scale && relu_shift, "qea_bn_bwd_pool: null pointer (relu_scale / relu_shift are required)");
  QEA_REQUIRE(B > 0 && H > 0 && W > 0 && H % 2 == 0 && (kw == 1 || kw == 2) && W % kw == 0, "qea_bn_bwd_pool: 2 x kw windows, kw in {1, 2}, H and W multiples");
  const long long M = (long long)B * H * W;
  const long long NWIN = M / (2 * kw);
  ColGeom gm;
  if (int rc = check_cols("qea_bn_bwd_pool", M, C, ldy | lddy | lddp | (da ? ldda : 0), workspace, workspace_bytes, 3, &gm)) return rc;
  ColGeom g = gm;
  g.rows_per_block = (g.rows_per_block + 2 * kw - 1) / (2 * kw);
  if (g.rows_per_block < 1) g.rows_per_block = 1;
  g.grid = (int)((NWIN + g.rows_per_block - 1) / g.rows_per_block);
  QEA_REQUIRE(g.grid <= gm.grid, "qea_bn_bwd_pool: more window blocks than partial rows in the workspace");
  hipStream_t s = (hipStream_t)stream;
  double* ws = (double*)workspace;
  const size_t lds = (size_t)g.rt * C * 2 * sizeof(double);
  auto red = kw == 2 ? bn_bwd_pool_kernel<2, false> : bn_bwd_pool_kernel<1, false>;
  hipLaunchKernelGGL(red, dim3(g.grid), dim3(RED_THREADS), lds, s, da, ldda, dpool, lddp, y, ldy, (float*)nullptr, 0, B, H, W, C, relu_scale, relu_shift,
                     mean, invstd, stat64, (const double*)nullptr, (const double*)nullptr, (const double*)nullptr, g.rows_per_block, g.rt, ws,
                     (float*)nullptr);
  return bn_bwd_tail(ws, g.grid, ws + (size_t)gm.grid * C * 2, M, C, {gamma, mean, invstd, stat64, training, dgamma, dbeta, accumulate_param_grads}, s,
                     [&](const double* k0, const double* k1, const double* k2) {
                       const ApplyGeom ag = apply_geom(NWIN, g.rt, 4);
                       auto app = kw == 2 ? bn_bwd_pool_kernel<2, true> : bn_bwd_pool_kernel<1, true>;
                       hipLaunchKernelGGL(app, dim3(ag.grid), dim3(RED_THREADS), 0, s, da, ldda, dpool, lddp, y, ldy, dy, lddy, B, H, W, C, relu_scale,
                                          relu_shift, mean, invstd, stat64, k0, k1, k2, ag.per_block, g.rt, (double*)nullptr, absmax_out);
                     });
}

extern "C" int qea_bn_bwd_from_partials(const double* partials, int32_t blocks, const float* da, int32_t ldda, const float* relu_scale,
                                        const float* relu_shift, const float* y, int32_t ldy, int64_t M, int32_t C, const float* gamma,
                                        const float* mean, const float* invstd, const double* stat64, int32_t training, float* dgamma,
                                        float* dbeta, int32_t accumulate_param_grads, float* dy, int32_t lddy, void* workspace,
                                        size_t workspace_bytes, float* absmax_out, void* stream) {
  QEA_REQUIRE(partials && blocks > 0 && da && y && mean && invstd && dy && stat64 && relu_scale && relu_shift,
              "qea_bn_bwd_from_partials: null pointer / no blocks (stat64 and relu_scale / relu_shift are required)");
  if (int rc = check_cols("qea_bn_bwd_from_partials", M, C, ldda | ldy | lddy, workspace, workspace_bytes, 3, nullptr)) return rc;
  hipStream_t s = (hipStream_t)stream;
  const double* src;
  int nblk;
  fold_partials(partials, blocks, C, s, &src, &nblk);
  return bn_bwd_tail(src, nblk, (double*)workspace, M, C, {gamma, mean, invstd, stat64, training, dgamma, dbeta, accumulate_param_grads}, s,
                     [&](const double* k0, const double* k1, const double* k2) {
                       bn_bwd_apply_launch(da, ldda, nullptr, 0, y, ldy, dy, lddy, M, C, relu_scale, relu_shift, k0, k1, k2, col_geom(M, C).rt,
                                           absmax_out, s);
                     });
}

extern "C" int qea_colsum(const float* x, int32_t ldx, int64_t M, int32_t C, float* out, int32_t accumulate, void* workspace,
                          size_t workspace_bytes, void* stream) {
  QEA_REQUIRE(x && out, "qea_colsum: null pointer");
  ColGeom g;
  if (int rc = check_cols("qea_colsum", M, C, ldx, workspace, workspace_bytes, 0, &g)) return rc;
  hipStream_t s = (hipStream_t)stream;
  const size_t lds = (size_t)g.rt * C * 2 * sizeof(double);
  hipLaunchKernelGGL(colreduce_kernel<2>, dim3(g.grid), dim3(RED_THREADS), lds, s, x, ldx, nullptr, 0, nullptr, 0, nullptr, nullptr,
                     nullptr, nullptr, nullptr, (long long)M, C, g.rows_per_block, g.rt, (double*)workspace);
  hipLaunchKernelGGL(colsum_finalize_kernel, dim3(qea_cdiv(C, 4)), dim3(256), 0, s, (const double*)workspace, g.grid, C, out, accumulate);
  QEA_CHECK_LAUNCH();
  return QEA_OK;
}

extern "C" int qea_maxpool_fwd(const float* x, int32_t ldx, float* y, int32_t ldy, int32_t B, int32_t H, int32_t W, int32_t C, int32_t kh,
                               int32_t kw, float* absmax_out, void* stream) {
  QEA_REQUIRE(x && y && B > 0 && C > 0 && C % 4 == 0 && kh > 0 && kw > 0 && H % kh == 0 && W % kw == 0 && ldx % 4 == 0 && ldy % 4 == 0,
              "qea_maxpool_fwd: bad arguments (H,W must be multiples of the window; C, ld multiples of 4)");
  const long long n = (long long)B * (H / kh) * (W / kw) * (C / 4);
  hipLaunchKernelGGL(maxpool_fwd_kernel, dim3(qea_grid_for(n)), dim3(256), 0, (hipStream_t)stream, x, ldx, y, ldy, B, H, W, C, kh, kw, absmax_out);
  QEA_CHECK_LAUNCH();
  return QEA_OK;
}

extern "C" int qea_bn_apply_pool(const float* y, int32_t ldy, float* a, int32_t lda, float* pooled, int32_t ldp, int32_t B, int32_t H, int32_t W,
                                 int32_t C, const float* scale, const float* shift, int32_t relu, int32_t kh, int32_t kw, float* absmax_a,
                                 float* absmax_pooled, void* stream) {
  QEA_REQUIRE(y && a && pooled && scale && shift && B > 0 && C > 0 && C % 4 == 0 && kh > 0 && kw > 0 && H > 0 && W > 0 && H % kh == 0 && W % kw == 0 &&
                  ldy % 4 == 0 && lda % 4 == 0 && ldp % 4 == 0,
              "qea_bn_apply_pool: bad arguments (H,W must be multiples of the window; C, ld multiples of 4)");
  const long long n = (long long)B * (H / kh) * (W / kw) * (C / 4);
  hipLaunchKernelGGL(bn_apply_pool_kernel, dim3(qea_grid_for(n)), dim3(256), 0, (hipStream_t)stream, y, ldy, a, lda, pooled, ldp, B, H, W, C, scale, shift,
                     relu, kh, kw, absmax_a, absmax_pooled);
  QEA_CHECK_LAUNCH();
  return QEA_OK;
}

extern "C" int qea_maxpool_bwd(const float* x, int32_t ldx, const float* dy, int32_t lddy, float* dx, int32_t lddx, int32_t B, int32_t H,
                               int32_t W, int32_t C, int32_t kh, int32_t kw, int32_t relu_mask, int32_t accumulate, float* absmax_out,
                               void* stream) {
  QEA_REQUIRE(x && dy && dx && B > 0 && C > 0 && C % 4 == 0 && kh > 0 && kw > 0 && H % kh == 0 && W % kw == 0 && ldx % 4 == 0 &&
                  lddy % 4 == 0 && lddx % 4 == 0,
              "qea_maxpool_bwd: bad arguments");
  const long long n = (long long)B * (H / kh) * (W / kw) * (C / 4);
  hipLaunchKernelGGL(maxpool_bwd_kernel, dim3(qea_grid_for(n)), dim3(256), 0, (hipStream_t)stream, x, ldx, dy, lddy, dx, lddx, B, H, W, C, kh,
                     kw, relu_mask, accumulate, absmax_out);
  QEA_CHECK_LAUNCH();
  return QEA_OK;
}

extern "C" int qea_transpose2d(const float* in, float* out, int32_t R, int32_t Cc, void* stream) {
  QEA_REQUIRE(in && out && R > 0 && Cc > 0, "qea_transpose2d: bad arguments");
  hipLaunchKernelGGL(transpose_kernel, dim3(qea_cdiv(Cc, 32), qea_cdiv(R, 32)), dim3(256), 0, (hipStream_t)stream, in, out, R, Cc);
  QEA_CHECK_LAUNCH();
  return QEA_OK;
}
```

query-efficient-approx-to-improve-ocr_amd/qea/batchnorm.py:

```python
import torch

from . import ops

BN_EPS = 1e-5
BN_MOMENTUM = 0.1


def partition(groups, B):
    if isinstance(groups, int):
        if groups < 1 or B % groups:
            raise ValueError(f"batch {B} is not a multiple of groups={groups}")
        sizes = [B // groups] * groups
    else:
        sizes = [int(v) for v in groups]
        if sum(sizes) != B or any(v <= 0 for v in sizes):
            raise ValueError(f"group sizes {sizes} do not partition the batch of {B}")
    return [(sum(sizes[:i]), n) for i, n in enumerate(sizes)]


class Stage:

    def __init__(self, y, h, w, C, parts, coef, stat64, training):
        self.y, self.h, self.w, self.C, self.parts, self.coef, self.stat64, self.training = y, h, w, C, parts, coef, stat64, training

    @property
    def single(self):
        return len(self.parts) == 1

    def rows(self, t, b0, nb, per=None):
        per = per or self.h * self.w
        return t[b0 * per:(b0 + nb) * per] if t is not None else None

    def restricted(self, b0, nb):
        g = self.parts.index((b0, nb)) if self.training else 0
        return Stage(self.rows(self.y, b0, nb), self.h, self.w, self.C, [(0, nb)], self.coef[g:g + 1],
                     self.stat64[g:g + 1] if self.stat64 is not None else None, self.training)

    def producer_sums(self):
        have = self.training and self.single and self.stat64 is not None
        return (self.y, self.C, self.stat64[0], self.coef[0, 2], self.coef[0, 3]) if have else None


def eval_scale_shift(C, gamma, beta, running_mean, running_var):
    coef = torch.empty(4, C, device=gamma.device)
    ops.bn_eval_coeff(C, gamma, beta, running_mean, running_var, BN_EPS, None, coef[0], coef[1], coef[2], coef[3])
    return coef[2], coef[3]


def forward(y, out, ldo, h, w, C, gamma, beta, running_mean, running_var, training, parts, keep, amax=None, partials=None, pool=None):
    if not training:
        parts = [(0, sum(nb for _, nb in parts))]
    if partials is not None and len(parts) > 1:
        raise ValueError("statistics from the conv's partials cover the whole batch: one statistics group only")
    coef = torch.empty(len(parts), 4, C, device=y.device)
    stat64 = torch.empty(len(parts), 2, C, device=y.device, dtype=torch.float64) if (training and keep) else None
    st = Stage(y, h, w, C, parts, coef, stat64, training)
    for g, (b0, nb) in enumerate(parts):
        mean, invstd, scale, shift = coef[g]
        yg, s64 = st.rows(y, b0, nb), stat64[g] if stat64 is not None else None
        if not training:
            ops.bn_eval_coeff(C, gamma, beta, running_mean, running_var, BN_EPS, None, mean, invstd, scale, shift)
        elif partials is not None:
            ops.bn_train_stats_from_partials(partials[0], partials[1], nb * h * w, C, gamma, beta, BN_EPS, BN_MOMENTUM, running_mean,
                                             running_var, mean, invstd, scale, shift, s64)
        else:
            ops.bn_train_stats(yg, C, nb * h * w, C, gamma, beta, BN_EPS, BN_MOMENTUM, running_mean, running_var, mean, invstd, scale,
                               shift, s64)
        if pool is not None:
            pooled, ldp, kh, kw, pooled_amax = pool
            ops.bn_apply_pool(yg, C, st.rows(out, b0, nb), ldo, st.rows(pooled, b0, nb, (h // kh) * (w // kw)), ldp, nb, h, w, C, scale,
                              shift, kh, kw, relu=True, amax=amax, pooled_amax=pooled_amax)
        else:
            ops.bn_apply(yg, C, st.rows(out, b0, nb), ldo, nb * h * w, C, scale, shift, relu=True, amax=amax)
    return st, pool is not None


def backward(st, da, ldda, dy, gamma, dgamma, dbeta, amax=None, partials=None, pool=None):
    for g, (b0, nb) in enumerate(st.parts):
        mean, invstd, scale, shift = st.coef[g]
        rest = dict(accumulate=True, stat64=st.stat64[g] if st.stat64 is not None else None, relu_scale=scale, relu_shift=shift, amax=amax)
        yg, dyg = st.rows(st.y, b0, nb), st.rows(dy, b0, nb)
        if pool is not None:
            dpool, lddp, kw = pool
            ops.bn_bwd_pool(st.rows(da, b0, nb), ldda, st.rows(dpool, b0, nb, (st.h // 2) * (st.w // kw)), lddp, kw, yg, st.C, nb, st.h, st.w,
                            st.C, gamma, mean, invstd, st.training, dgamma, dbeta, dyg, st.C, **rest)
        else:
            ops.bn_bwd(st.rows(da, b0, nb), ldda, None, 0, yg, st.C, nb * st.h * st.w, st.C, gamma, mean, invstd, st.training, dgamma, dbeta,
                       dyg, st.C, partials=partials, **rest)
```

query-efficient-approx-to-improve-ocr_amd/qea/ops.py:

```python
import ctypes as C
import os
import weakref
from collections import namedtuple

import numpy as np
import torch

from . import _lib, beam

OUT_NHWC, OUT_TBC, OUT_CONVT = 0, 1, 2
PROF_CONV_IGEMM, PROF_CONV_WGRAD, PROF_LSTM_STEP = 0, 1, 2

_ws = {}


def _stream():
    return torch.cuda.current_stream().cuda_stream


def _ptr(t):
    if t is None:
        return None
    if not t.is_cuda:
        raise _lib.QeaError("qea ops need CUDA tensors (there is no CPU path)")
# ... 247 lines not shown
    if pool is not None:
        d.pool_y, d.ldpool, d.pool_kw = pool[0].data_ptr(), pool[1], pool[2]
        d.pool_absmax = pool[3].data_ptr() if pool[3] is not None else None
    partials = None
    if bwd_stats is not None and wants == 1 and d.x_absmax and FUSE_BN_STATS["on"]:
        blocks = L.qea_conv_igemm_stats_blocks(C.byref(d))
        if blocks > 0:
            partials = torch.empty(blocks + 256, N, 2, dtype=torch.float64, device=x.device)
            d.stats = partials.data_ptr()
            d.bst_y, d.ldbst, d.bst_stat64 = bwd_stats[0].data_ptr(), bwd_stats[1], bwd_stats[2].data_ptr()
            d.bst_scale, d.bst_shift = bwd_stats[3].data_ptr(), bwd_stats[4].data_ptr()
    elif want_stats and FUSE_BN_STATS["on"]:
        blocks = L.qea_conv_igemm_stats_blocks(C.byref(d))
        if blocks > 0:
            partials = torch.empty(blocks + 256, N, 2, dtype=torch.float64, device=x.device)
            d.stats = partials.data_ptr()
    _lib.check(L.qea_conv_igemm(C.byref(d), _stream()), "qea_conv_igemm")
    return (partials, partials.shape[0] - 256) if partials is not None else None


def conv_can_pool(*, B, H, W, Cin, N, kw, ldx, ldy, mask=None):
    if not (PRESPLIT["on"] and SPLIT_F16["on"] and mfma_mode() == "split_f16") or mask is not None:
        return False
    d = _conv_desc(None, None, None, B=B, H=H, W=W, Cin=Cin, OH=H, OW=W, N=N, KH=3, KW=3, pad=(1, 1), stride=(1, 1), ldx=ldx, ldy=ldy)
    return bool(_lib.lib().qea_conv_igemm_can_pool(C.byref(d), kw))


def conv_wgrad(p, q, dw, *, B, PH, PW, QH, QW, R, Cc, KH, KW, pad=(0, 0), stride=(1, 1), ldp, ldq,
               accumulate=False, splits=0, tile=0, p_amax=None, q_amax=None, dbias=None):
    L = _lib.lib()
    d = _lib.WgradDesc(p=_ptr(p), q=_ptr(q), dw=_ptr(dw), workspace=None, workspace_bytes=0,
                       B=B, PH=PH, PW=PW, QH=QH, QW=QW, R=R, C=Cc, KH=KH, KW=KW, pad_h=pad[0], pad_w=pad[1],
                       stride_h=stride[0], stride_w=stride[1], ldp=ldp, ldq=ldq, accumulate=int(accumulate),
                       splits=splits, tile=tile)
    if SPLIT_F16["on"] and mfma_mode() != "f32" and L.qea_conv_wgrad_wants_absmax(C.byref(d)):
        if p_amax is None:
            p_amax = absmax(p, ldp, B * PH * PW, R)
        if q_amax is None:
            q_amax = absmax(q, ldq, B * QH * QW, Cc)
        d.p_absmax, d.q_absmax = p_amax.data_ptr(), q_amax.data_ptr()
    fused = dbias is not None and bool(L.qea_conv_wgrad_fuses_bias(C.byref(d)))
    if fused:
        d.dbias = dbias.data_ptr()
    need = L.qea_conv_wgrad_workspace_bytes(C.byref(d))
    if need:
        ws = workspace(need, p.device)
        d.workspace = ws.data_ptr()
        d.workspace_bytes = ws.numel()
    _lib.check(L.qea_conv_wgrad(C.byref(d), _stream()), "qea_conv_wgrad")
    if dbias is not None and not fused:
        colsum(p, ldp, B * PH * PW, R, dbias, accumulate=accumulate)


SPLIT_F16 = {"on": os.environ.get("QEA_SPLIT", "f16").lower() != "bf16"}


def set_mfma_mode(mode):
    lib_mode = {"split_bf16": 0, "split_f16": 0, "f32": 1}[mode]
    prev_name = mfma_mode()
    prev = _lib.lib().qea_set_mfma_mode(lib_mode)
    if prev < 0:
        _lib.check(prev, "qea_set_mfma_mode")
    SPLIT_F16["on"] = mode == "split_f16"
    return prev_name


def mfma_mode():
    m = ("split_bf16", "f32")[_lib.lib().qea_set_mfma_mode(-1)]
    return "split_f16" if (m == "split_bf16" and SPLIT_F16["on"]) else m


class AmaxPool:

    def __init__(self, device, n=192, on=True):
        self.on = on
        self.buf = torch.zeros(n, device=device) if on else None
        self.full = []
        self.used = 0

    def __call__(self):
        if not self.on:
            return None
        if self.used == self.buf.numel():
            self.full.append(self.buf)
            self.buf = torch.zeros(self.buf.numel(), device=self.buf.device)
            self.used = 0
        self.used += 1
        return self.buf[self.used - 1:self.used]


def amax_pool(device):
    return AmaxPool(device, on=SPLIT_F16["on"] and mfma_mode() == "split_f16")


def filter_absmax(w_src, w, ld, M, Cc):
    from .params import flat_state_of
    fs = flat_state_of(w_src[1], check=False) if w_src is not None else None
    if fs is None or fs.total % 4 or fs.data.data_ptr() > w_src[1].data_ptr() or w_src[1].data_ptr() >= fs.data.data_ptr() + 4 * fs.total:
        return absmax(w, ld, M, Cc)
    return weight_cached("flat_absmax", fs.data, lambda: absmax(fs.data, fs.total, 1, fs.total), extra=(fs.vsum, fs.epoch))


def split_planes_f16(x, ld, M, Cc, w_src=None):
    L = _lib.lib()
    out = torch.empty(L.qea_split_planes_f16_bytes(M, Cc), dtype=torch.uint8, device=x.device)
    xmax = filter_absmax(w_src, x, ld, M, Cc)
    _lib.check(L.qea_split_planes_f16(_ptr(x), ld, M, Cc, _ptr(xmax), out.data_ptr(), _stream()), "qea_split_planes_f16")
    return out


def absmax(x, ld, M, Cc):
    out = torch.empty(1, device=x.device)
    _lib.check(_lib.lib().qea_absmax(_ptr(x), ld, M, Cc, _ptr(out), _stream()), "qea_absmax")
    return out


_overlap = {"on": None}


def set_overlap(on):
    _overlap["on"] = bool(on)


def overlap_enabled():
    if _overlap["on"] is None:
        import os
        _overlap["on"] = os.environ.get("QEA_OVERLAP", "1") != "0"
    return _overlap["on"]


class SideStream:

    def __init__(self, device):
        self.side = torch.cuda.Stream(device)

    @classmethod
    def of(cls, owner, device):
        side = owner.__dict__.get("_side")
        if side is None or side.side is not None and side.side.device != device:
            side = owner._side = cls(device)
        return side

    @property
    def enabled(self):
        return overlap_enabled()

    def run(self, fn, *reads):
        if not self.enabled:
            fn()
            return
        main = torch.cuda.current_stream()
        ev = torch.cuda.Event()
        ev.record(main)
        with torch.cuda.stream(self.side):
            self.side.wait_event(ev)
            fn()
        for t in reads:
            if t is not None:
                t.record_stream(self.side)

    def join(self):
        if self.enabled:
            ev = torch.cuda.Event()
            ev.record(self.side)
            torch.cuda.current_stream().wait_event(ev)


def prof_enable(klass, on=True):
    _lib.check(_lib.lib().qea_prof_enable(klass, int(on)), "qea_prof_enable")


def prof_reset():
    _lib.check(_lib.lib().qea_prof_reset(), "qea_prof_reset")


def prof_read(klass):
    ms, fl, by, n = C.c_double(), C.c_double(), C.c_double(), C.c_int64()
    _lib.check(_lib.lib().qea_prof_read(klass, C.byref(ms), C.byref(fl), C.byref(by), C.byref(n)), "qea_prof_read")
    sp, sf = C.c_double(), C.c_double()
    _lib.check(_lib.lib().qea_prof_read_split_bf16(klass, C.byref(sp)), "qea_prof_read_split_bf16")
    _lib.check(_lib.lib().qea_prof_read_split_f16(klass, C.byref(sf)), "qea_prof_read_split_f16")
    return {"ms": ms.value, "flops": fl.value, "bytes": by.value, "launches": n.value, "flops_split_bf16": sp.value, "flops_split_f16": sf.value}


def prof_tag_halo_bf3(cin_chunk, cout_group, stats, f16=False):
    return 24000 + (1000 if cin_chunk == 64 else 0) + cout_group + (500 if stats else 0) + (5 if f16 else 0)


def prof_read_tagged(klass, tag):
    ms, fl, by, n = C.c_double(), C.c_double(), C.c_double(), C.c_int64()
    _lib.check(_lib.lib().qea_prof_read_tagged(klass, tag, C.byref(ms), C.byref(fl), C.byref(by), C.byref(n)), "qea_prof_read_tagged")
    return {"ms": ms.value, "flops": fl.value, "bytes": by.value, "launches": n.value}


def _colws(M, C_, device):
    need = _lib.lib().qea_colreduce_workspace_bytes(M, C_)
    ws = workspace(need, device)
    return ws.data_ptr(), ws.numel()


def bn_train_stats(y, ldy, M, C_, gamma, beta, eps, momentum, running_mean, running_var, mean, invstd, scale, shift, stat64=None):
    wp, wn = _colws(M, C_, y.device)
    _lib.check(_lib.lib().qea_bn_train_stats(_ptr(y), ldy, M, C_, _ptr(gamma), _ptr(beta), eps, momentum,
                                             _ptr(running_mean), _ptr(running_var), _ptr(mean), _ptr(invstd),
                                             _ptr(scale), _ptr(shift), _ptr(stat64), wp, wn, _stream()), "qea_bn_train_stats")


def bn_train_stats_from_partials(partials, blocks, M, C_, gamma, beta, eps, momentum, running_mean, running_var, mean, invstd, scale, shift,
                                 stat64=None):
    _lib.check(_lib.lib().qea_bn_train_stats_from_partials(_ptr(partials), blocks, M, C_, _ptr(gamma), _ptr(beta), eps, momentum,
                                                           _ptr(running_mean), _ptr(running_var), _ptr(mean), _ptr(invstd),
                                                           _ptr(scale), _ptr(shift), _ptr(stat64), _stream()),
               "qea_bn_train_stats_from_partials")


def bn_eval_coeff(C_, gamma, beta, running_mean, running_var, eps, conv_bias, mean, invstd, scale, shift):
    _lib.check(_lib.lib().qea_bn_eval_coeff(C_, _ptr(gamma), _ptr(beta), _ptr(running_mean), _ptr(running_var), eps,
                                            _ptr(conv_bias), _ptr(mean), _ptr(invstd), _ptr(scale), _ptr(shift),
                                            _stream()), "qea_bn_eval_coeff")


def bn_apply(y, ldy, a, lda, M, C_, scale, shift, relu=True, amax=None):
    _lib.check(_lib.lib().qea_bn_apply(_ptr(y), ldy, _ptr(a), lda, M, C_, _ptr(scale), _ptr(shift), int(relu), _ptr(amax), _stream()),
               "qea_bn_apply")


def bn_bwd(da, ldda, a, lda, y, ldy, M, C_, gamma, mean, invstd, training, dgamma, dbeta, dy, lddy, accumulate=False, stat64=None,
           relu_scale=None, relu_shift=None, amax=None, partials=None):
    wp, wn = _colws(M, C_, da.device)
    if partials is not None:
        _lib.check(_lib.lib().qea_bn_bwd_from_partials(partials[0].data_ptr(), partials[1], _ptr(da), ldda, _ptr(relu_scale), _ptr(relu_shift), _ptr(y),
                                                       ldy, M, C_, _ptr(gamma), _ptr(mean), _ptr(invstd), _ptr(stat64), int(training), _ptr(dgamma),
                                                       _ptr(dbeta), int(accumulate), _ptr(dy), lddy, wp, wn, _ptr(amax), _stream()),
                   "qea_bn_bwd_from_partials")
        return
    _lib.check(_lib.lib().qea_bn_bwd(_ptr(da), ldda, _ptr(a), lda, _ptr(relu_scale), _ptr(relu_shift), _ptr(y), ldy, M, C_, _ptr(gamma), _ptr(mean),
                                     _ptr(invstd), _ptr(stat64), int(training), _ptr(dgamma), _ptr(dbeta), int(accumulate),
                                     _ptr(dy), lddy, wp, wn, _ptr(amax), _stream()), "qea_bn_bwd")


def bn_bwd_pool(da, ldda, dpool, lddp, kw, y, ldy, B, H, W, C_, gamma, mean, invstd, training, dgamma, dbeta, dy, lddy, accumulate=False,
                stat64=None, relu_scale=None, relu_shift=None, amax=None):
    wp, wn = _colws(B * H * W, C_, y.device)
    _lib.check(_lib.lib().qea_bn_bwd_pool(_ptr(da), ldda, _ptr(dpool), lddp, kw, _ptr(relu_scale), _ptr(relu_shift), _ptr(y), ldy, B, H, W, C_,
                                          _ptr(gamma), _ptr(mean), _ptr(invstd), _ptr(stat64), int(training), _ptr(dgamma), _ptr(dbeta),
                                          int(accumulate), _ptr(dy), lddy, wp, wn, _ptr(amax), _stream()), "qea_bn_bwd_pool")


def colsum(x, ldx, M, C_, out, accumulate=False):
    wp, wn = _colws(M, C_, x.device)
    _lib.check(_lib.lib().qea_colsum(_ptr(x), ldx, M, C_, _ptr(out), int(accumulate), wp, wn, _stream()), "qea_colsum")


def bn_apply_pool(y, ldy, a, lda, pooled, ldp, B, H, W, C_, scale, shift, kh, kw, relu=True, amax=None, pooled_amax=None):
    _lib.check(_lib.lib().qea_bn_apply_pool(_ptr(y), ldy, _ptr(a), lda, _ptr(pooled), ldp, B, H, W, C_, _ptr(scale), _ptr(shift), int(relu), kh, kw,
                                            _ptr(amax), _ptr(pooled_amax), _stream()), "qea_bn_apply_pool")


def maxpool_fwd(x, ldx, y, ldy, B, H, W, C_, kh, kw, amax=None):
    _lib.check(_lib.lib().qea_maxpool_fwd(_ptr(x), ldx, _ptr(y), ldy, B, H, W, C_, kh, kw, _ptr(amax), _stream()), "qea_maxpool_fwd")


def conv_c1_pool_bwd(x, w, bias, dpool, lddp, dw, db, dx, B, H, W, Co, accumulate=False):
    L = _lib.lib()
    need = L.qea_conv_c1_pool_bwd_workspace_bytes(B, H, W, Co, int(dx is not None))
    ws = torch.empty(max(need, 256), dtype=torch.uint8, device=x.device)
    _lib.check(L.qea_conv_c1_pool_bwd(_ptr(x), _ptr(w), _ptr(bias), _ptr(dpool), lddp, _ptr(dw), _ptr(db), _ptr(dx), B, H, W, Co, int(accumulate),
                                      ws.data_ptr(), ws.numel(), _stream()), "qea_conv_c1_pool_bwd")


def maxpool_bwd(x, ldx, dy, lddy, dx, lddx, B, H, W, C_, kh, kw, relu_mask=False, accumulate=False, amax=None):
    _lib.check(_lib.lib().qea_maxpool_bwd(_ptr(x), ldx, _ptr(dy), lddy, _ptr(dx), lddx, B, H, W, C_, kh, kw,
                                          int(relu_mask), int(accumulate), _ptr(amax), _stream()), "qea_maxpool_bwd")


def transpose2d(src, dst, R, Cc):
    _lib.check(_lib.lib().qea_transpose2d(_ptr(src), _ptr(dst), R, Cc, _stream()), "qea_transpose2d")


def filter_flip_transpose(w, wt, Co, Ci, KH, KW):
    _lib.check(_lib.lib().qea_filter_flip_transpose(_ptr(w), _ptr(wt), Co, Ci, KH, KW, _stream()), "qea_filter_flip_transpose")


def conv_c1_fwd(x, w, bias, y, ldy, B, H, W, Co, relu=False):
    _lib.check(_lib.lib().qea_conv_c1_fwd(_ptr(x), _ptr(w), _ptr(bias), _ptr(y), ldy, B, H, W, Co, int(relu), _stream()),
               "qea_conv_c1_fwd")


def conv_c1_fwd_pool(x, w, bias, y, ldy, pooled, ldp, B, H, W, Co, relu=False, pooled_amax=None):
    if H % 2 or W % 4 or Co not in (32, 64, 128):
        return False
    _lib.check(_lib.lib().qea_conv_c1_fwd_pool(_ptr(x), _ptr(w), _ptr(bias), _ptr(y), ldy, _ptr(pooled), ldp, B, H, W, Co, int(relu),
                                               _ptr(pooled_amax), _stream()), "qea_conv_c1_fwd_pool")
    return True


def conv_c1_wgrad(x, dy, lddy, dw, db, B, H, W, Co, accumulate=False):
    L = _lib.lib()
    ws = workspace(L.qea_conv_c1_wgrad_workspace_bytes(B, H, W, Co), x.device)
    _lib.check(L.qea_conv_c1_wgrad(_ptr(x), _ptr(dy), lddy, _ptr(dw), _ptr(db), B, H, W, Co, int(accumulate),
                                   ws.data_ptr(), ws.numel(), _stream()), "qea_conv_c1_wgrad")


def conv_c1_dgrad(dy, lddy, w, dx, B, H, W, Co, accumulate=False):
    _lib.check(_lib.lib().qea_conv_c1_dgrad(_ptr(dy), lddy, _ptr(w), _ptr(dx), B, H, W, Co, int(accumulate), _stream()),
               "qea_conv_c1_dgrad")


def head_fwd(x, ldx, w, b, y, M, C_):
    _lib.check(_lib.lib().qea_head_fwd(_ptr(x), ldx, _ptr(w), _ptr(b), _ptr(y), M, C_, _stream()), "qea_head_fwd")


def head_bwd(x, ldx, y, dyy, w, dx, lddx, dw, db, M, C_, accumulate=False):
    L = _lib.lib()
    ws = workspace(L.qea_head_bwd_workspace_bytes(M, C_), x.device)
    _lib.check(L.qea_head_bwd(_ptr(x), ldx, _ptr(y), _ptr(dyy), _ptr(w), _ptr(dx), lddx, _ptr(dw), _ptr(db),
                              int(accumulate), M, C_, ws.data_ptr(), ws.numel(), _stream()), "qea_head_bwd")


def lstm_pack_whh(w_hh, packed_fwd, packed_bwd):
    _lib.check(_lib.lib().qea_lstm_pack_whh(_ptr(w_hh), _ptr(packed_fwd), _ptr(packed_bwd), _stream()), "qea_lstm_pack_whh")


def lstm_layer_fwd(gates, c, y, packed_fwd, T, B):
    _lib.check(_lib.lib().qea_lstm_layer_fwd(_ptr(gates), _ptr(c), _ptr(y), _ptr(packed_fwd), T, B, _stream()), "qea_lstm_layer_fwd")


def lstm_layer_bwd(gates, c, dy, packed_bwd, dc_scratch, T, B):
    _lib.check(_lib.lib().qea_lstm_layer_bwd(_ptr(gates), _ptr(c), _ptr(dy), _ptr(packed_bwd), _ptr(dc_scratch), T, B,
                                             _stream()), "qea_lstm_layer_bwd")


def lstm_pack_whh_split(w_hh, planes_fwd, planes_bwd):
    _lib.check(_lib.lib().qea_lstm_pack_whh_split(_ptr(w_hh), _ptr(planes_fwd), _ptr(planes_bwd), _stream()), "qea_lstm_pack_whh_split")


LSTM_SEQ = {"on": os.environ.get("QEA_LSTM", "seq") != "step"}


def lstm_mode():
    m = mfma_mode()
    if m == "f32":
        return "f32"
    return "seq" if (m == "split_f16" and LSTM_SEQ["on"]) else "bf3"


def lstm_packs(whf, whr):
    mode = lstm_mode()
    dev = whf.device

    def pack():
        if mode == "seq":
            nb = _lib.lib().qea_lstm_seq_pack_bytes()
            pf_ = torch.empty(2, nb, dtype=torch.uint8, device=dev)
            pb_ = torch.empty(2, nb, dtype=torch.uint8, device=dev)
            bounds = [filter_absmax(("fwd", wh), wh, 256, 1024, 256) for wh in (whf, whr)]
            am = torch.cat([b.reshape(1) for b in bounds])
            for d_, wh in enumerate((whf, whr)):
                _lib.check(_lib.lib().qea_lstm_seq_pack(_ptr(wh), _ptr(pf_[d_]), _ptr(pb_[d_]), _ptr(am[d_:]), _stream()), "qea_lstm_seq_pack")
            return (pf_, am), (pb_, am)
        if mode == "bf3":
            nb = _lib.lib().qea_lstm_pack_whh_split_bytes()
            pf_ = torch.empty(2, nb, dtype=torch.uint8, device=dev)
            pb_ = torch.empty(2, nb, dtype=torch.uint8, device=dev)
            for d_, wh in enumerate((whf, whr)):
                lstm_pack_whh_split(wh, pf_[d_], pb_[d_])
        else:
            pf_ = torch.empty(2, whf.numel(), device=dev)
            pb_ = torch.empty(2, whf.numel(), device=dev)
            for d_, wh in enumerate((whf, whr)):
                lstm_pack_whh(wh, pf_[d_], pb_[d_])
        return pf_, pb_
    pf, pb = weight_cached(("whh_pack", mode), whf, pack, also=(whr,))
    return pf, pb, mode


_LSTM_SEQ_LAST = {"fwd": None, "bwd": None}


def _lstm_seq_ws(B, dev, which):
    ws = torch.empty(_lib.lib().qea_lstm_seq_workspace_bytes(B), dtype=torch.uint8, device=dev)
    _LSTM_SEQ_LAST[which] = (ws, B)
    return ws


def lstm_seq_timed_out(which):
    last = _LSTM_SEQ_LAST[which]
    if last is None:
        raise _lib.QeaError(f"no \"seq\" {which} pass has run in this process")
    ws, B = last
    idx = _lib.lib().qea_lstm_seq_timeout_index(B, int(which == "bwd"))
    return bool(ws.view(torch.int32)[idx].item() != 0)


def lstm_layer_fwd_any(gates, c, y, pack, mode, T, B, y_amax=None):
    if os.environ.get("QEA_LSTM_TRACE"):
        print("lstm fwd", mode, T, B, flush=True)
    if mode == "seq":
        planes, am = pack
        ws = _lstm_seq_ws(B, gates.device, "fwd")
        _lib.check(_lib.lib().qea_lstm_seq_fwd(_ptr(gates), _ptr(c), _ptr(y), _ptr(planes), _ptr(am), T, B, _ptr(ws), _ptr(y_amax), _stream()), "qea_lstm_seq_fwd")
        return y_amax is not None
    elif mode is True or mode == "bf3":
        _lib.check(_lib.lib().qea_lstm_layer_fwd_split(_ptr(gates), _ptr(c), _ptr(y), _ptr(pack), T, B, _stream()), "qea_lstm_layer_fwd_split")
    else:
        lstm_layer_fwd(gates, c, y, pack, T, B)


def lstm_layer_bwd_any(gates, c, dy, pack, mode, dc_scratch, T, B, g_amax=None):
    if mode == "seq":
        planes, am = pack
        ws = _lstm_seq_ws(B, gates.device, "bwd")
        _lib.check(_lib.lib().qea_lstm_seq_bwd(_ptr(gates), _ptr(c), _ptr(dy), _ptr(planes), _ptr(am), T, B, _ptr(ws), _ptr(g_amax), _stream()), "qea_lstm_seq_bwd")
        return g_amax is not None
    elif mode is True or mode == "bf3":
        _lib.check(_lib.lib().qea_lstm_layer_bwd_split(_ptr(gates), _ptr(c), _ptr(dy), _ptr(pack), _ptr(dc_scratch), T, B, _stream()),
                   "qea_lstm_layer_bwd_split")
    else:
        lstm_layer_bwd(gates, c, dy, pack, dc_scratch, T, B)


def log_softmax_fwd(x, ldx, y, ldy, M, C_):
    _lib.check(_lib.lib().qea_log_softmax_fwd(_ptr(x), ldx, _ptr(y), ldy, M, C_, _stream()), "qea_log_softmax_fwd")


def log_softmax_bwd(g, ldg, lp, ldlp, dx, lddx, M, C_, Cpad, nan_scrub):
    _lib.check(_lib.lib().qea_log_softmax_bwd(_ptr(g), ldg, _ptr(lp), ldlp, _ptr(dx), lddx, M, C_, Cpad, int(nan_scrub),
                                              _stream()), "qea_log_softmax_bwd")


def ctc_loss(lp, ld_t, ld_n, targets, target_offsets, input_lengths, target_lengths, T, N, C_, blank, S_max, reduction,
             grad_scale, nll, loss, grad, gld_t, gld_n):
    L = _lib.lib()
    ws = workspace(L.qea_ctc_workspace_bytes(T, N, S_max), lp.device)
    _lib.check(L.qea_ctc_loss(_ptr(lp), ld_t, ld_n, _ptr(targets), _ptr(target_offsets), _ptr(input_lengths),
                              _ptr(target_lengths), T, N, C_, blank, S_max, reduction, grad_scale, _ptr(nll), _ptr(loss),
                              _ptr(grad), gld_t, gld_n, ws.data_ptr(), ws.numel(), _stream()), "qea_ctc_loss")


def adam_step(p, g, m, v, n, lr, beta1, beta2, eps, weight_decay, step, grad_scale=1.0):
    _lib.check(_lib.lib().qea_adam_step(_ptr(p), _ptr(g), _ptr(m), _ptr(v), n, lr, beta1, beta2, eps, weight_decay, step,
                                        grad_scale, _stream()), "qea_adam_step")


def adam_step_capturable(p, g, m, v, n, lr, beta1, beta2, eps, weight_decay, step, coef, grad_scale=1.0):
    _lib.check(_lib.lib().qea_adam_step_capturable(_ptr(p), _ptr(g), _ptr(m), _ptr(v), n, lr, beta1, beta2, eps, weight_decay,
                                                   _ptr(step), _ptr(coef), grad_scale, _stream()), "qea_adam_step_capturable")


def jitter(img, sigma, out, noise_out, K, R, HW, coef, seed, offset):
    _lib.check(_lib.lib().qea_jitter(_ptr(img), _ptr(sigma), _ptr(out), _ptr(noise_out), K, R, HW, coef, seed, offset,
                                     _stream()), "qea_jitter")


def jitter_apply(img, noise, out, K, R, HW, coef):
    _lib.check(_lib.lib().qea_jitter_apply(_ptr(img), _ptr(noise), _ptr(out), K, R, HW, coef, _stream()), "qea_jitter_apply")


def topk_desc_stable(keys, n, k, idx_out):
    _lib.check(_lib.lib().qea_topk_desc_stable(_ptr(keys), n, k, _ptr(idx_out), _stream()), "qea_topk_desc_stable")


def crop_pad_gather(img, H, W, boxes, N, OH, OW, out):
    _lib.check(_lib.lib().qea_crop_pad_gather(_ptr(img), H, W, _ptr(boxes), N, OH, OW, _ptr(out), _stream()), "qea_crop_pad_gather")


def crop_pad_scatter(dout, boxes, N, OH, OW, dimg, H, W):
    _lib.check(_lib.lib().qea_crop_pad_scatter(_ptr(dout), _ptr(boxes), N, OH, OW, _ptr(dimg), H, W, _stream()), "qea_crop_pad_scatter")


def greedy_decode(scores, ld_t, ld_n, T, N, C_, blank, tokens, lengths):
    _lib.check(_lib.lib().qea_greedy_decode(_ptr(scores), ld_t, ld_n, T, N, C_, blank, _ptr(tokens), _ptr(lengths), _stream()),
               "qea_greedy_decode")


def _beam_search(name, scores, K, blank, mode=None, extra=None):
    who = name[len("qea_"):]
    if scores.dim() != 3 or not scores.is_cuda or scores.dtype != torch.float32:
        raise _lib.QeaError(f"{who} needs a CUDA float32 tensor [T,N,C] (there is no CPU path here: qea.beam has one)")
    if scores.stride(2) != 1:
        raise _lib.QeaError(f"{who} needs a unit class stride: make the last dimension contiguous")
    if not (0 <= scores.stride(0) < 2 ** 31 and 0 <= scores.stride(1) < 2 ** 31):
        raise _lib.QeaError(f"{who}: the T and N strides must fit 32 bits")
    T, N, C_ = scores.shape
    K = int(K)
    args = mode() if mode else ()
    rows = max(K, 1)
    out = [torch.empty(N, rows, T, dtype=torch.int32, device=scores.device), torch.empty(N, rows, dtype=torch.int32, device=scores.device),
           torch.empty(N, rows, dtype=torch.float64, device=scores.device)]
    if extra is not None:
        out.append(torch.empty(N, rows, dtype=extra, device=scores.device))
    _lib.check(getattr(_lib.lib(), name)(_ptr(scores), scores.stride(0), scores.stride(1), T, N, C_, int(blank), K, *args,
                                         *[_ptr(t) for t in out], _stream()), name)
    return tuple(out)


def ctc_beam_decode(scores, K, blank=0):
    return _beam_search("qea_ctc_beam_decode", scores, K, blank)


def ctc_beam_decode_lm(scores, K, table, context, blank=0):
    def mode():
        C_, m = scores.shape[2], int(context)
        beam.check_lm_limits(C_, m)
        if not (torch.is_tensor(table) and table.is_cuda and table.device == scores.device and table.dtype == torch.float64
                and table.is_contiguous() and tuple(table.shape) == (C_ ** m, C_)):
            raise _lib.QeaError(f"ctc_beam_decode_lm needs a contiguous CUDA float64 table [C**context, C] = {(C_ ** m, C_)} on the scores' device")
        return _ptr(table), m
    return _beam_search("qea_ctc_beam_decode_lm", scores, K, blank, mode, torch.float64)


def ctc_beam_decode_dfa(scores, K, automaton, blank=0):
    def mode():
        from .lexicon import DeviceAutomaton
        a = automaton
        if not isinstance(a, DeviceAutomaton):
            raise _lib.QeaError("ctc_beam_decode_dfa takes the object Lexicon.device() returns: the tables it holds are validated")
        if a.device != scores.device:
            raise _lib.QeaError(f"ctc_beam_decode_dfa: the automaton is on {a.device}, the scores on {scores.device}")
        if a.num_classes != scores.shape[2] or a.blank != int(blank):
            raise _lib.QeaError(f"ctc_beam_decode_dfa: the automaton has {a.num_classes} classes and blank {a.blank}, "
                                f"the scores {scores.shape[2]} and {int(blank)}")
        return _ptr(a.first), _ptr(a.label), _ptr(a.child), a.num_states, a.num_edges
    return _beam_search("qea_ctc_beam_decode_dfa", scores, K, blank, mode, torch.int32)


def prof_read_launches(klass, capacity=4096):
    import numpy as np
    ms = np.zeros(capacity)
    fl = np.zeros(capacity)
    n = C.c_int64()
    _lib.check(_lib.lib().qea_prof_read_launches(klass, ms.ctypes.data, fl.ctypes.data, capacity, C.byref(n)), "qea_prof_read_launches")
    k = min(n.value, capacity)
    return ms[:k], fl[:k]


def edit_distance(pred_tokens, ldp, pred_len, gt_tokens, gt_offsets, gt_len, N, out):
    _lib.check(_lib.lib().qea_edit_distance(_ptr(pred_tokens), ldp, _ptr(pred_len), _ptr(gt_tokens), _ptr(gt_offsets), _ptr(gt_len), N,
                                            _ptr(out), _stream()), "qea_edit_distance")


def facility_select(x, k):
    if x.dim() == 1:
        x = x[:, None]
    if not x.is_cuda or x.dtype != torch.float64 or x.dim() != 2:
        raise _lib.QeaError("facility_select needs a CUDA float64 tensor [n][d] (there is no CPU path here: pruning.methods has one)")
    x = x.contiguous()
    n, d = x.shape
    L = _lib.lib()
    ranking = torch.empty(max(int(k), 1), dtype=torch.int32, device=x.device)
    gains = torch.empty(max(int(k), 1), dtype=torch.float64, device=x.device)
    nbytes = L.qea_facility_workspace_bytes(n, d)
    ws = workspace(max(nbytes, 16), x.device)
    _lib.check(L.qea_facility_select(_ptr(x), n, d, int(k), _ptr(ranking), _ptr(gains), ws.data_ptr(), _stream()), "qea_facility_select")
    out = ranking.cpu(), gains.cpu()
    _lib.check(L.qea_facility_status(ws.data_ptr(), _stream()), "qea_facility_select")
    return out


HISTORY_MAX_WINDOW, HISTORY_MAX_LEN, HISTORY_ATTN_MAX_TABLE = 8, 128, 12288
HISTORY_ACTIVATIONS = {"sigmoid": 0, "softmax": 1, "relu": 2}
HISTORY_LAUNCHES = {"lev": 0, "attn": 0}


def history_lev_weights(tokens, lens, count, n, W, out):
    _lib.check(_lib.lib().qea_history_lev_weights(_ptr(tokens), _ptr(lens), _ptr(count), n, W, _ptr(out), _stream()), "qea_history_lev_weights")
    HISTORY_LAUNCHES["lev"] += 1


def history_attn_weights(char_idx, count, n, W, n_chars, embedding, wq_weight, wq_bias, coef_weight, coef_bias, pos, activation, out):
    if activation not in HISTORY_ACTIVATIONS:
        raise ValueError(f"unknown attn_activation {activation!r}")
    V1, E = embedding.shape
    Dq = wq_weight.shape[0]
    _lib.check(_lib.lib().qea_history_attn_weights(_ptr(char_idx), _ptr(count), n, W, n_chars, _ptr(embedding), V1, E, _ptr(wq_weight),
                                                   _ptr(wq_bias), Dq, _ptr(coef_weight), _ptr(coef_bias), _ptr(pos),
                                                   HISTORY_ACTIVATIONS[activation], _ptr(out), _stream()), "qea_history_attn_weights")
    HISTORY_LAUNCHES["attn"] += 1


HISTORY_CTC_LAUNCHES = {"ctc": 0}


def ctc_history_workspace_bytes(T, N, W, S_max):
    return _lib.lib().qea_ctc_history_workspace_bytes(T, N, W, S_max)


def ctc_history_loss(lp, input_lengths, lens, offs, chars, depth_n, weights, w_stride_n, w_stride_i, mean_by_length, S_max, blank=0,
                     need_grad=True):
    T, N, C_ = lp.shape
    W = depth_n.numel()
    if lp.dtype != torch.float32 or lp.stride(2) != 1 or weights.dtype != torch.float32:
        raise _lib.QeaError("ctc_history_loss needs fp32 log-probs with a unit class stride and fp32 weights")
    if any(t.dtype != torch.int32 or not t.is_contiguous() for t in (input_lengths, lens, offs, chars, depth_n)):
        raise _lib.QeaError("ctc_history_loss needs contiguous int32 lengths, offsets, characters and depth counts")
    if input_lengths.numel() != N or lens.numel() != N * W or offs.numel() != N * W:
        raise _lib.QeaError(f"ctc_history_loss: tables of {lens.numel()} / {offs.numel()} entries for N={N}, W={W}")
    if W < 1 or (N - 1) * w_stride_n + (W - 1) * w_stride_i >= weights.untyped_storage().nbytes() // 4 - weights.storage_offset():
        raise _lib.QeaError("ctc_history_loss: the weight strides reach past the weight tensor")
    if chars.numel() == 0:
        chars = torch.zeros(1, dtype=torch.int32, device=lp.device)
    L = _lib.lib()
    dev = lp.device
    loss = torch.empty(1, device=dev)
    nll = torch.empty(N, W, device=dev)
    grad = torch.empty(T, N, C_, device=dev) if need_grad else None
# ... 361 lines not shown
```

query-efficient-approx-to-improve-ocr_amd/qea/unet_engine.py:

```python
import torch

from . import batchnorm, conv, ops
from .params import ensure_flat

FUSE_EVAL_BN = True
FUSE_BN_BWD_SUMS = True
FUSE_BN_POOL = True
FUSE_POOL_BWD = True


class _Block:

    def __init__(self, mod, name, cin, cout):
        self.mod, self.name, self.cin, self.cout = mod, name, cin, cout

    def key(self, i, leaf):
        kind = "conv" if leaf == "w" else "norm"
        suffix = {"w": "weight", "gamma": "weight", "beta": "bias", "rm": "running_mean", "rv": "running_var"}[leaf]
        return f"{self.mod}.{self.name}{kind}{i}.{suffix}"


class UNetEngine:
    def __init__(self, module, features=32):
        self.m = module
        f = features
        self.f = f
        self.enc = [_Block("encoder1", "enc1", 1, f), _Block("encoder2", "enc2", f, 2 * f), _Block("encoder3", "enc3", 2 * f, 4 * f),
                    _Block("encoder4", "enc4", 4 * f, 8 * f)]
        self.bott = _Block("bottleneck", "bottleneck", 8 * f, 16 * f)
        self.dec = {l: _Block(f"decoder{l}", f"dec{l}", 2 * c, c) for l, c in ((4, 8 * f), (3, 4 * f), (2, 2 * f), (1, f))}

    def _conv_bn_relu(self, P, Bf, blk, i, x, ldx, cv, out, ldo, training, keep, parts, x_amax=None, out_amax=None, pool=None):
        B, H, W, cin, cout = cv.B, cv.H, cv.W, cv.Cin, cv.N
        w = P[blk.key(i, "w")]
        bn = (P[blk.key(i, "gamma")], P[blk.key(i, "beta")], Bf[blk.key(i, "rm")], Bf[blk.key(i, "rv")])
        if not training and not keep and cin != 1 and FUSE_EVAL_BN:
            scale, shift = batchnorm.eval_scale_shift(cout, *bn)
            fused_pool = None
            if pool is not None and cv.can_pool(2, ldx, ldo):
                fused_pool = (pool[0], cout, 2, pool[1])
            cv.fwd(x, ldx, w, out, ldo, scale=scale, bias=shift, relu=True, x_amax=x_amax, y_amax=out_amax, pool=fused_pool)
            return None, fused_pool is not None
        y = torch.empty(B * H * W, cout, device=x.device)
        fused = None
        if cin == 1:
            ops.conv_c1_fwd(x, w, None, y, cout, B, H, W, cout, relu=False)
        else:
            fused = cv.fwd(x, ldx, w, y, cout, want_stats=training and len(parts) == 1, x_amax=x_amax)
        return batchnorm.forward(y, out, ldo, H, W, cout, *bn, training, parts, keep, amax=out_amax, partials=fused,
                                 pool=(pool[0], cout, 2, 2, pool[1]) if pool is not None else None)

    def forward(self, x, training, need_grad, groups=1):
        fs = ensure_flat(self.m)
        P, Bf = dict(self.m.named_parameters()), dict(self.m.named_buffers())
        B, _, H, W = x.shape
        if H % 16 or W % 16:
            raise ValueError(f"UNet input {H}x{W} must be a multiple of 16 in both dimensions")
        dev = x.device
        f = self.f
        parts = batchnorm.partition(int(groups) if training else 1, B)
        ctx = {"x": x, "B": B, "H": H, "W": W, "blocks": {}} if need_grad else None

        slot = ops.amax_pool(dev)

        def run_block(blk, xin, ldx, cin, h, w, out, ldo, xin_amax, out_amax, pool=None):
            a1 = torch.empty(B * h * w, blk.cout, device=dev)
            a1_amax = slot()
            c1, c2 = (conv.Conv(B, h, w, ci, blk.cout, 3, 3, pad=(1, 1)) for ci in (cin, blk.cout))
            bn1, _ = self._conv_bn_relu(P, Bf, blk, 1, xin, ldx, c1, a1, blk.cout, training, need_grad, parts, xin_amax, a1_amax)
            bn2, pooled_here = self._conv_bn_relu(P, Bf, blk, 2, a1, blk.cout, c2, out, ldo, training, need_grad, parts, a1_amax, out_amax, pool)
            if need_grad:
                ctx["blocks"][blk.mod] = {"xin": xin, "ldx": ldx, "c1": c1, "c2": c2, "h": h, "w": w, "a1": a1, "out": out, "ldo": ldo,
                                          "bn1": bn1, "bn2": bn2, "xin_amax": xin_amax, "a1_amax": a1_amax,
                                          "y1": bn1.y, "y2": bn2.y}
            return pooled_here

        cats, cat_amax = {}, {}
        xin, ldx, cin, xin_amax = x, 1, 1, None
        h, w = H, W
        for l, blk in enumerate(self.enc, start=1):
            c = blk.cout
            cat = torch.empty(B * h * w, 2 * c, device=dev)
            cats[l] = (cat, h, w, c)
            cat_amax[l] = slot()
            skip = cat[:, c:]
            pooled = torch.empty(B * (h // 2) * (w // 2), c, device=dev)
            xin_in, xin_amax = xin_amax, slot()
            if not run_block(blk, xin, ldx, cin, h, w, skip, 2 * c, xin_in, cat_amax[l], pool=(pooled, xin_amax) if FUSE_BN_POOL else None):
                ops.maxpool_fwd(skip, 2 * c, pooled, c, B, h, w, c, 2, 2, amax=xin_amax)
            xin, ldx, cin = pooled, c, c
            h, w = h // 2, w // 2
        d = torch.empty(B * h * w, self.bott.cout, device=dev)
        d_amax = slot()
        run_block(self.bott, xin, ldx, cin, h, w, d, self.bott.cout, xin_amax, d_amax)
        dcin = self.bott.cout
        ups = {}
        for l in (4, 3, 2, 1):
            cat, hh, ww, c = cats[l]
            up = conv.Conv(B, hh, ww, c, dcin, 2, 2, stride=(2, 2))
            up.scatter_adjoint(d, dcin, P[f"upconv{l}.weight"], cat, 2 * c, bias=P[f"upconv{l}.bias"], x_amax=d_amax, y_amax=cat_amax[l])
            ups[l] = (d, up, d_amax)
            h, w = hh, ww
            dnew = torch.empty(B * h * w, c, device=dev)
            d_amax = slot()
            run_block(self.dec[l], cat, 2 * c, 2 * c, h, w, dnew, c, cat_amax[l], d_amax)
            d, dcin = dnew, c
        out = torch.empty(B, 1, H, W, device=dev)
        ops.head_fwd(d, f, P["conv.weight"], P["conv.bias"], out, B * H * W, f)
        if training:
            fs.ibuf.add_(len(parts))
        if need_grad:
            ctx.update(cats=cats, ups=ups, d1=d, out=out)
        return out, ctx

    def backward(self, ctx, dout):
        fs = ensure_flat(self.m)
        fs.attach_grads()
        P = dict(self.m.named_parameters())
        G = {n: p.grad for n, p in P.items()}
        B, H, W = ctx["B"], ctx["H"], ctx["W"]
        dev = dout.device
        f = self.f
        dout = dout.contiguous()
        side = ops.SideStream.of(self, dev)
        slot = ops.amax_pool(dev)

        last_amax = [None]

        def block_bwd(blk, da2, ldda, pool=None):
            s = ctx["blocks"][blk.mod]
            c1, c2 = s["c1"], s["c2"]
            h, w, cin, cout = c1.H, c1.W, c1.Cin, c1.N
            M = B * h * w
            dy2 = torch.empty(M, cout, device=dev)
            dy2_amax, dy1_amax = slot(), slot()
            batchnorm.backward(s["bn2"], da2, ldda, dy2, P[blk.key(2, "gamma")], G[blk.key(2, "gamma")], G[blk.key(2, "beta")], amax=dy2_amax,
                               pool=pool)
            side.run(lambda: c2.wgrad(dy2, cout, s["a1"], cout, G[blk.key(2, "w")], accumulate=True, p_amax=dy2_amax, q_amax=s.get("a1_amax")), dy2)
            da1 = torch.empty(M, cout, device=dev)
            bst = s["bn1"].producer_sums() if FUSE_BN_BWD_SUMS else None
            part = c2.dgrad(dy2, cout, P[blk.key(2, "w")], da1, cout, x_amax=dy2_amax, bwd_stats=bst)
            dy1 = torch.empty(M, cout, device=dev)
            batchnorm.backward(s["bn1"], da1, cout, dy1, P[blk.key(1, "gamma")], G[blk.key(1, "gamma")], G[blk.key(1, "beta")], amax=dy1_amax,
                               partials=part if bst is not None else None)
            if cin == 1:
                side.run(lambda: ops.conv_c1_wgrad(s["xin"], dy1, cout, G[blk.key(1, "w")], None, B, h, w, cout, accumulate=True), dy1)
                return None
            side.run(lambda: c1.wgrad(dy1, cout, s["xin"], s["ldx"], G[blk.key(1, "w")], accumulate=True, p_amax=dy1_amax,
                                      q_amax=s.get("xin_amax")), dy1)
            dxin = torch.empty(M, cin, device=dev)
            last_amax[0] = slot()
            c1.dgrad(dy1, cout, P[blk.key(1, "w")], dxin, cin, x_amax=dy1_amax, y_amax=last_amax[0])
            return dxin

        d1 = ctx["d1"]
        M0 = B * H * W
        dd = torch.empty(M0, f, device=dev)
        ops.head_bwd(d1, f, ctx["out"], dout, P["conv.weight"], dd, f, G["conv.weight"], G["conv.bias"], M0, f, accumulate=True)

        dcats = {}
        for l in (1, 2, 3, 4):
            dcat = block_bwd(self.dec[l], dd, self.dec[l].cout)
            cat, hh, ww, c = ctx["cats"][l]
            dcats[l] = dcat
            dprev, up, dprev_amax = ctx["ups"][l]
            dcin = up.N
            def up_grads(dcat=dcat, dprev=dprev, l=l, c=c, hh=hh, ww=ww, up=up, pa=dprev_amax, qa=last_amax[0]):
                ops.colsum(dcat, 2 * c, B * hh * ww, c, G[f"upconv{l}.bias"], accumulate=True)
                up.wgrad(dprev, up.N, dcat, 2 * c, G[f"upconv{l}.weight"], accumulate=True, p_amax=pa, q_amax=qa)
            side.run(up_grads, dcat)
            dd = torch.empty(B * up.OH * up.OW, dcin, device=dev)
            up.fwd(dcat, 2 * c, P[f"upconv{l}.weight"], dd, dcin, x_amax=last_amax[0])
        dpool = block_bwd(self.bott, dd, self.bott.cout)
        for l in (4, 3, 2, 1):
            cat, hh, ww, c = ctx["cats"][l]
            dskip = dcats[l][:, c:]
            if FUSE_POOL_BWD and ctx["blocks"][self.enc[l - 1].mod]["bn2"].single:
                dpool = block_bwd(self.enc[l - 1], dskip, 2 * c, pool=(dpool, c, 2))
            else:
                ops.maxpool_bwd(cat[:, c:], 2 * c, dpool, c, dskip, 2 * c, B, hh, ww, c, 2, 2, relu_mask=False, accumulate=True)
                dpool = block_bwd(self.enc[l - 1], dskip, 2 * c)
        side.join()
        return None
```

Before: 22700 patch-images/s.

## Recompute first-layer cin=1 conv inside fused BN stats/apply/backward kernels

For the first UNet conv (single input channel), the pre-BN activation is no longer stored. Instead the conv is recomputed from the grey input inside fused kernels: one computes BN statistics, one applies BN+ReLU, and one runs the backward that produces dgamma/dbeta and the weight gradient. This removes writes and reads of a large B*H*W*Cout fp32 tensor in both forward and backward. The cost is extra 9-tap conv arithmetic recomputed about three times, plus fp64 partial reductions. It is gated on the tensor being at least 32 MiB and a supported channel count.

```diff
diff --git a/include/qea_hip.h b/include/qea_hip.h
--- a/include/qea_hip.h
+++ b/include/qea_hip.h
@@ -165,6 +165,17 @@
                       void* stream);
 int qea_conv_c1_dgrad(const float* dy, int32_t lddy, const float* w, float* dx, int32_t B, int32_t H, int32_t W,
                       int32_t Co, int32_t accumulate, void* stream);
+size_t qea_c1_bn_stats_workspace_bytes(int32_t B, int32_t H, int32_t W, int32_t Co);
+int qea_c1_bn_stats(const float* x, const float* w, int32_t B, int32_t H, int32_t W, int32_t Co, const float* gamma, const float* beta,
+                    float eps, float momentum, float* running_mean, float* running_var, float* mean_out, float* invstd_out,
+                    float* scale_out, float* shift_out, double* stat64, void* workspace, size_t workspace_bytes, void* stream);
+int qea_c1_bn_apply(const float* x, const float* w, const float* scale, const float* shift, float* a, int32_t lda, int32_t B, int32_t H,
+                    int32_t W, int32_t Co, int32_t relu, float* absmax_out, void* stream);
+size_t qea_c1_bn_bwd_workspace_bytes(int32_t B, int32_t H, int32_t W, int32_t Co);
+int qea_c1_bn_bwd(const float* da, int32_t ldda, const float* x, const float* w, const float* relu_scale, const float* relu_shift,
+                  int32_t B, int32_t H, int32_t W, int32_t Co, const float* gamma, const float* mean, const float* invstd,
+                  const double* stat64, int32_t training, float* dgamma, float* dbeta, int32_t accumulate_param_grads, float* dw,
+                  int32_t accumulate_dw, void* workspace, size_t workspace_bytes, void* stream);
 
 int qea_head_fwd(const float* x, int32_t ldx, const float* w, const float* b, float* y, int64_t M, int32_t C,
                  void* stream);
diff --git a/query-efficient-approx-to-improve-ocr_amd/csrc/bn_core.h b/query-efficient-approx-to-improve-ocr_amd/csrc/bn_core.h
--- /dev/null
+++ b/query-efficient-approx-to-improve-ocr_amd/csrc/bn_core.h
@@ -0,0 +1,140 @@
+#pragma once
+#include "common.h"
+
+namespace {
+
+constexpr int RED_THREADS = 256;
+
+struct ColGeom {
+  int cols;
+  int rt;
+  int grid;
+  int rows_per_block;
+};
+
+inline ColGeom col_geom(long long M, int C) {
+  ColGeom g;
+  g.cols = C / 4;
+  g.rt = RED_THREADS / g.cols;
+  if (g.rt < 1) g.rt = 1;
+  long long want = (M + (long long)g.rt * 16 - 1) / ((long long)g.rt * 16);
+  if (want > 1024) want = 1024;
+  if (want < 1) want = 1;
+  g.grid = (int)want;
+  g.rows_per_block = (int)((M + g.grid - 1) / g.grid);
+  g.grid = (int)((M + g.rows_per_block - 1) / g.rows_per_block);
+  return g;
+}
+
+__device__ __forceinline__ float bn_affine(float v, float sc, float sh) { return __fmaf_rn(v, sc, sh); }
+
+__device__ __forceinline__ float bn_masked_dz(float d, bool has_a, float av, bool remask = false, float yv = 0.f, float sc = 0.f, float sh = 0.f) {
+  if (has_a) return av > 0.f ? d : 0.f;
+  if (remask) return bn_affine(yv, sc, sh) > 0.f ? d : 0.f;
+  return d;
+}
+__device__ __forceinline__ void bn_stats_acc(double& s0, double& s1, float v) {
+  s0 += (double)v;
+  s1 += (double)v * (double)v;
+}
+__device__ __forceinline__ void bn_bwd_acc(double& s0, double& s1, float dz, float yv, double mu, double is) {
+  s0 += (double)dz;
+  s1 += (double)dz * (((double)yv - mu) * is);
+}
+__device__ __forceinline__ float bn_dy(double c0, double c1, double c2, float dz, float yv) {
+  return (float)(c0 * (double)dz + (c1 * (double)yv + c2));
+}
+__device__ __forceinline__ void bn_load_mu_is(const double* __restrict__ stat64, const float* __restrict__ mean, const float* __restrict__ invstd,
+                                              int C, int c4, double (&mu)[4], double (&is)[4]) {
+#pragma unroll
+  for (int k = 0; k < 4; ++k) {
+    mu[k] = stat64 ? stat64[c4 + k] : (double)mean[c4 + k];
+    is[k] = stat64 ? stat64[C + c4 + k] : (double)invstd[c4 + k];
+  }
+}
+__device__ __forceinline__ void block_partials_store(double* sred, const double (&s0)[4], const double (&s1)[4], int rt, int rt_n, int ct, int C,
+                                                     double* __restrict__ ws) {
+  if (rt < rt_n) {
+#pragma unroll
+    for (int k = 0; k < 4; ++k) {
+      sred[((size_t)rt * C + ct * 4 + k) * 2 + 0] = s0[k];
+      sred[((size_t)rt * C + ct * 4 + k) * 2 + 1] = s1[k];
+    }
+  }
+  __syncthreads();
+  for (int c = threadIdx.x; c < C; c += blockDim.x) {
+    double t0 = 0, t1 = 0;
+    for (int r = 0; r < rt_n; ++r) {
+      t0 += sred[((size_t)r * C + c) * 2 + 0];
+      t1 += sred[((size_t)r * C + c) * 2 + 1];
+    }
+    ws[((size_t)blockIdx.x * C + c) * 2 + 0] = t0;
+    ws[((size_t)blockIdx.x * C + c) * 2 + 1] = t1;
+  }
+}
+
+__device__ __forceinline__ void partial_sums(const double* __restrict__ ws, int nblk, int C, int c, double& s, double& q) {
+  const int lane = threadIdx.x & 63;
+  double a = 0, b = 0;
+  for (int k = lane; k < nblk; k += 64) {
+    a += ws[((size_t)k * C + c) * 2 + 0];
+    b += ws[((size_t)k * C + c) * 2 + 1];
+  }
+  s = qea_wave_sum_d(a);
+  q = qea_wave_sum_d(b);
+}
+
+__global__ void bn_stats_finalize_kernel(const double* __restrict__ ws, int nblk, int C, long long M, const float* __restrict__ gamma,
+                                         const float* __restrict__ beta, float eps, float momentum, float* running_mean,
+                                         float* running_var, float* mean_out, float* invstd_out, float* scale_out, float* shift_out,
+                                         double* stat64) {
+  const int c = blockIdx.x * (blockDim.x >> 6) + (threadIdx.x >> 6);
+  if (c >= C) return;
+  double s, q;
+  partial_sums(ws, nblk, C, c, s, q);
+  if ((threadIdx.x & 63) != 0) return;
+  const double mean = s / (double)M;
+  double var = q / (double)M - mean * mean;
+  if (var < 0) var = 0;
+  const double invstd_d = 1.0 / sqrt(var + (double)eps);
+  if (stat64) {
+    stat64[c] = mean;
+    stat64[C + c] = invstd_d;
+  }
+  const float invstd = (float)invstd_d;
+  const float g = gamma ? gamma[c] : 1.f, b = beta ? beta[c] : 0.f;
+  mean_out[c] = (float)mean;
+  invstd_out[c] = invstd;
+  scale_out[c] = g * invstd;
+  shift_out[c] = b - (float)mean * g * invstd;
+  if (running_mean) {
+    const double unb = (M > 1) ? var * (double)M / (double)(M - 1) : var;
+    running_mean[c] = (1.f - momentum) * running_mean[c] + momentum * (float)mean;
+    running_var[c] = (1.f - momentum) * running_var[c] + momentum * (float)unb;
+  }
+}
+
+__global__ void bn_bwd_finalize_kernel(const double* __restrict__ ws, int nblk, int C, long long M, const float* __restrict__ gamma,
+                                       const float* __restrict__ mean, const float* __restrict__ invstd,
+                                       const double* __restrict__ stat64, int training, float* dgamma, float* dbeta, int accumulate,
+                                       double* k0, double* k1, double* k2) {
+  const int c = blockIdx.x * (blockDim.x >> 6) + (threadIdx.x >> 6);
+  if (c >= C) return;
+  double s, q;
+  partial_sums(ws, nblk, C, c, s, q);
+  if ((threadIdx.x & 63) != 0) return;
+  if (dgamma) dgamma[c] = accumulate ? dgamma[c] + (float)q : (float)q;
+  if (dbeta) dbeta[c] = accumulate ? dbeta[c] + (float)s : (float)s;
+  const double g = gamma ? (double)gamma[c] : 1.0;
+  const double is = stat64 ? stat64[C + c] : (double)invstd[c];
+  const double mu = stat64 ? stat64[c] : (double)mean[c];
+  const double m0 = training ? s / (double)M : 0.0;
+  const double m1 = training ? q / (double)M : 0.0;
+  k0[c] = g * is;
+  k1[c] = -g * is * is * m1;
+  k2[c] = g * is * (mu * is * m1 - m0);
+}
+
+inline size_t ws_need(int rows, int consts, int C) { return ((size_t)rows * 2 + consts) * C * sizeof(double); }
+
+}
diff --git a/query-efficient-approx-to-improve-ocr_amd/csrc/conv_c1.hip b/query-efficient-approx-to-improve-ocr_amd/csrc/conv_c1.hip
--- a/query-efficient-approx-to-improve-ocr_amd/csrc/conv_c1.hip
+++ b/query-efficient-approx-to-improve-ocr_amd/csrc/conv_c1.hip
@@ -1,6 +1,85 @@
-#include "common.h"
+#include "bn_core.h"
 
 namespace {
+
+__device__ __forceinline__ void c1_load_w(const float* __restrict__ w, int ct, f32x4 (&wr)[9]) {
+#pragma unroll
+  for (int t = 0; t < 9; ++t)
+#pragma unroll
+    for (int k = 0; k < 4; ++k) wr[t][k] = w[(ct * 4 + k) * 9 + t];
+}
+
+template <int R, int CW>
+__device__ __forceinline__ f32x4 c1_preact(f32x4 acc, const f32x4 (&wr)[9], const float (&xv)[R][CW], int r, int j) {
+#pragma unroll
+  for (int kh = 0; kh < 3; ++kh)
+#pragma unroll
+    for (int kw = 0; kw < 3; ++kw) {
+      const float xs = xv[r + kh][j + kw];
+      acc = __builtin_elementwise_fma(wr[kh * 3 + kw], (f32x4){xs, xs, xs, xs}, acc);
+    }
+  return acc;
+}
+
+__device__ __forceinline__ void c1_window_issue(const float* __restrict__ xb, int ph, int pw, int H, int W, float (&t)[3][3]) {
+#pragma unroll
+  for (int kh = 0; kh < 3; ++kh) {
+    const int ihc = min(max(ph + kh - 1, 0), H - 1);
+#pragma unroll
+    for (int kw = 0; kw < 3; ++kw) t[kh][kw] = xb[ihc * W + min(max(pw + kw - 1, 0), W - 1)];
+  }
+}
+__device__ __forceinline__ void c1_window_finish(float (&t)[3][3], int ph, int pw, int H, int W, float (&xv)[3][3]) {
+  asm volatile("" : "+v"(t[0][0]), "+v"(t[0][1]), "+v"(t[0][2]), "+v"(t[1][0]), "+v"(t[1][1]), "+v"(t[1][2]), "+v"(t[2][0]), "+v"(t[2][1]),
+               "+v"(t[2][2]));
+#pragma unroll
+  for (int kh = 0; kh < 3; ++kh)
+#pragma unroll
+    for (int kw = 0; kw < 3; ++kw)
+      xv[kh][kw] = ((unsigned)(ph + kh - 1) < (unsigned)H && (unsigned)(pw + kw - 1) < (unsigned)W) ? t[kh][kw] : 0.f;
+}
+
+__device__ __forceinline__ void c1_advance(int& ph, int& pw, int dph, int dpw, int H, int W) {
+  pw += dpw;
+  ph += dph;
+  if (pw >= W) {
+    pw -= W;
+    ++ph;
+  }
+  ph = ph >= H ? ph % H : ph;
+}
+
+template <class Row, class Body>
+__device__ __forceinline__ void c1_walk(const float* __restrict__ x, int H, int W, long long first, int step, long long end, Row row, Body body) {
+  if (first >= end) return;
+  int pw = (int)(first % W);
+  int ph = (int)((first / W) % H);
+  const int dph = step / W, dpw = step - dph * W;
+  float t[3][3];
+  c1_window_issue(x + (first - (long long)ph * W - pw), ph, pw, H, W, t);
+  f32x4 v = row(first);
+  for (long long p = first; p < end; p += step) {
+    int nph = ph, npw = pw;
+    c1_advance(nph, npw, dph, dpw, H, W);
+    const bool more = p + step < end;
+    const long long pn = more ? p + step : p;
+    nph = more ? nph : ph;
+    npw = more ? npw : pw;
+    float tn[3][3];
+    c1_window_issue(x + (pn - (long long)nph * W - npw), nph, npw, H, W, tn);
+    const f32x4 vn = row(pn);
+    float xv[3][3];
+    c1_window_finish(t, ph, pw, H, W, xv);
+    body(p, xv, v);
+#pragma unroll
+    for (int kh = 0; kh < 3; ++kh)
+#pragma unroll
+      for (int kw = 0; kw < 3; ++kw) t[kh][kw] = tn[kh][kw];
+    v = vn;
+    ph = nph;
+    pw = npw;
+  }
+}
 
 __global__ void conv_c1_fwd_kernel(const float* __restrict__ x, const float* __restrict__ w, const float* __restrict__ bias,
                                    float* __restrict__ y, int ldy, int B, int H, int W, int Co, int relu) {
@@ -40,16 +119,13 @@
   }
 }
 
-template <int COLS>
-__global__ __launch_bounds__(256) void conv_c1_fwd4_kernel(const float* __restrict__ x, const float* __restrict__ w, const float* __restrict__ bias,
-                                                           float* __restrict__ y, int ldy, int B, int H, int W, int relu) {
+template <int COLS, class Out>
+__device__ __forceinline__ void c1_fwd4_walk(const float* __restrict__ x, const float* __restrict__ w, const float* __restrict__ bias, int B, int H,
+                                             int W, Out out) {
   constexpr int GPB = 256 / COLS;
   const int ct = threadIdx.x % COLS;
   f32x4 wr[9];
-#pragma unroll
-  for (int t = 0; t < 9; ++t)
-#pragma unroll
-    for (int k = 0; k < 4; ++k) wr[t][k] = w[(ct * 4 + k) * 9 + t];
+  c1_load_w(w, ct, wr);
   f32x4 bv = {0.f, 0.f, 0.f, 0.f};
   if (bias) bv = *reinterpret_cast<const f32x4*>(bias + ct * 4);
   const unsigned W4 = (unsigned)W >> 2;
@@ -70,21 +146,45 @@
         xv[kh][c] = (rok && (unsigned)iw < (unsigned)W) ? xr[(kh - 1) * W + iw] : 0.f;
       }
     }
-    float* yo = y + ((size_t)row * W + pw0) * ldy + ct * 4;
-#pragma unroll
-    for (int j = 0; j < 4; ++j) {
-      f32x4 acc = bv;
-#pragma unroll
-      for (int kh = 0; kh < 3; ++kh)
-#pragma unroll
-        for (int kw = 0; kw < 3; ++kw) acc += wr[kh * 3 + kw] * xv[kh][j + kw];
-      if (relu) {
-#pragma unroll
-        for (int k = 0; k < 4; ++k) acc[k] = fmaxf(acc[k], 0.f);
-      }
-      *reinterpret_cast<f32x4*>(yo + (size_t)j * ldy) = acc;
-    }
-  }
+    const size_t p0 = (size_t)row * W + pw0;
+#pragma unroll
+    for (int j = 0; j < 4; ++j) out(p0 + j, c1_preact(bv, wr, xv, 0, j));
+  }
+}
+
+template <int COLS>
+__global__ __launch_bounds__(256) void conv_c1_fwd4_kernel(const float* __restrict__ x, const float* __restrict__ w, const float* __restrict__ bias,
+                                                           float* __restrict__ y, int ldy, int B, int H, int W, int relu) {
+  float* yo = y + (threadIdx.x % COLS) * 4;
+  c1_fwd4_walk<COLS>(x, w, bias, B, H, W, [&](size_t pix, f32x4 acc) {
+    if (relu) {
+#pragma unroll
+      for (int k = 0; k < 4; ++k) acc[k] = fmaxf(acc[k], 0.f);
+    }
+    *reinterpret_cast<f32x4*>(yo + pix * ldy) = acc;
+  });
+}
+
+template <int COLS>
+__global__ __launch_bounds__(256) void c1_bn_apply_kernel(const float* __restrict__ x, const float* __restrict__ w, const float* __restrict__ scale,
+                                                          const float* __restrict__ shift, float* __restrict__ a, int lda, int B, int H, int W,
+                                                          int relu, float* __restrict__ amax) {
+  const int ct = threadIdx.x % COLS;
+  const f32x4 sc = *reinterpret_cast<const f32x4*>(scale + ct * 4);
+  const f32x4 sh = *reinterpret_cast<const f32x4*>(shift + ct * 4);
+  float* ao = a + ct * 4;
+  float am = 0.f;
+  c1_fwd4_walk<COLS>(x, w, nullptr, B, H, W, [&](size_t pix, f32x4 acc) {
+    f32x4 o;
+#pragma unroll
+    for (int k = 0; k < 4; ++k) {
+      o[k] = bn_affine(acc[k], sc[k], sh[k]);
+      if (relu) o[k] = fmaxf(o[k], 0.f);
+      am = qea_amax_acc(am, o[k]);
+    }
+    *reinterpret_cast<f32x4*>(ao + pix * lda) = o;
+  });
+  qea_amax_commit_block(am, amax);
 }
 
 template <int COLS>
@@ -125,11 +225,7 @@
     for (int r = 0; r < 2; ++r)
 #pragma unroll
       for (int j = 0; j < 4; ++j) {
-        f32x4 acc = bv;
-#pragma unroll
-        for (int kh = 0; kh < 3; ++kh)
-#pragma unroll
-          for (int kw = 0; kw < 3; ++kw) acc += wr[kh * 3 + kw] * xv[r + kh][j + kw];
+        f32x4 acc = c1_preact(bv, wr, xv, r, j);
         if (relu) {
 #pragma unroll
           for (int k = 0; k < 4; ++k) acc[k] = fmaxf(acc[k], 0.f);
@@ -158,8 +254,9 @@
 }
 
 
-__global__ __launch_bounds__(256) void conv_c1_wgrad_kernel(const float* __restrict__ x, const float* __restrict__ dy, int lddy, int B, int H,
-                                                            int W, int Co, int rt_n, int rows_per_thread, float* __restrict__ ws) {
+template <class Row, class Grad>
+__device__ __forceinline__ void c1_wgrad_body(const float* __restrict__ x, int B, int H, int W, int Co, int rt_n, int rows_per_thread,
+                                              float* __restrict__ ws, Row row, Grad grad) {
   extern __shared__ __attribute__((aligned(16))) float sacc[];
   const int cols = Co / 4;
   const int ct = threadIdx.x % cols, rt = threadIdx.x / cols;
@@ -169,36 +266,15 @@
   for (int t = 0; t < 10; ++t) acc[t] = (f32x4){0.f, 0.f, 0.f, 0.f};
   if (rt < rt_n) {
     const long long r0 = (long long)blockIdx.x * rt_n * rows_per_thread;
-    int pw = (int)((r0 + rt) % W);
-    int ph = (int)(((r0 + rt) / W) % H);
-    const int dph = rt_n / W, dpw = rt_n - dph * W;
-    for (int j = 0; j < rows_per_thread; ++j) {
-      const long long pix = r0 + (long long)j * rt_n + rt;
-      if (pix >= M) break;
-      if (j) {
-        pw += dpw;
-        ph += dph;
-        if (pw >= W) {
-          pw -= W;
-          ++ph;
-        }
-        ph = ph >= H ? ph % H : ph;
-      }
-      const float* xb = x + (pix - (long long)ph * W - pw);
-      const f32x4 g = *reinterpret_cast<const f32x4*>(dy + pix * lddy + ct * 4);
-#pragma unroll
-      for (int kh = 0; kh < 3; ++kh) {
-        const int ih = ph + kh - 1;
-#pragma unroll
-        for (int kw = 0; kw < 3; ++kw) {
-          const int iw = pw + kw - 1;
-          float xv = 0.f;
-          if ((unsigned)ih < (unsigned)H && (unsigned)iw < (unsigned)W) xv = xb[ih * W + iw];
-          acc[kh * 3 + kw] += g * xv;
-        }
-      }
+    const long long r1 = r0 + (long long)rt_n * rows_per_thread;
+    c1_walk(x, H, W, r0 + rt, rt_n, r1 < M ? r1 : M, row, [&](long long, const float (&xv)[3][3], const f32x4 v) {
+      const f32x4 g = grad(v, xv);
+#pragma unroll
+      for (int kh = 0; kh < 3; ++kh)
+#pragma unroll
+        for (int kw = 0; kw < 3; ++kw) acc[kh * 3 + kw] += g * xv[kh][kw];
       acc[9] += g;
-    }
+    });
 #pragma unroll
     for (int t = 0; t < 10; ++t) *reinterpret_cast<f32x4*>(sacc + ((size_t)rt * 10 + t) * Co + ct * 4) = acc[t];
   }
@@ -208,6 +284,80 @@
     for (int r = 0; r < rt_n; ++r) s += sacc[(size_t)r * 10 * Co + e];
     ws[(size_t)blockIdx.x * 10 * Co + e] = s;
   }
+}
+
+__global__ __launch_bounds__(256) void conv_c1_wgrad_kernel(const float* __restrict__ x, const float* __restrict__ dy, int lddy, int B, int H,
+                                                            int W, int Co, int rt_n, int rows_per_thread, float* __restrict__ ws) {
+  const float* dyc = dy + (threadIdx.x % (Co / 4)) * 4;
+  c1_wgrad_body(x, B, H, W, Co, rt_n, rows_per_thread, ws, [&](long long pix) { return *reinterpret_cast<const f32x4*>(dyc + pix * lddy); },
+                [](const f32x4 g, const float (&)[3][3]) { return g; });
+}
+
+template <int MODE>
+__global__ __launch_bounds__(RED_THREADS) void c1_bn_reduce_kernel(const float* __restrict__ x, const float* __restrict__ w,
+                                                                     const float* __restrict__ da, int ldda, const float* __restrict__ mean,
+                                                                     const float* __restrict__ invstd, const double* __restrict__ stat64,
+                                                                     const float* __restrict__ msc, const float* __restrict__ msh, int B, int H,
+                                                                     int W, int C, int rows_per_block, int rt_n, double* __restrict__ ws) {
+  extern __shared__ __attribute__((aligned(16))) double sred[];
+  const int cols = C / 4;
+  const int ct = threadIdx.x % cols, rt = threadIdx.x / cols;
+  double s0[4] = {0, 0, 0, 0}, s1[4] = {0, 0, 0, 0};
+  if (rt < rt_n) {
+    const long long M = (long long)B * H * W;
+    const long long r0 = (long long)blockIdx.x * rows_per_block;
+    long long r1 = r0 + rows_per_block;
+    if (r1 > M) r1 = M;
+    f32x4 wr[9];
+    c1_load_w(w, ct, wr);
+    double mu[4] = {0, 0, 0, 0}, is[4] = {0, 0, 0, 0};
+    const f32x4 zero = {0.f, 0.f, 0.f, 0.f};
+    f32x4 sc = zero, sh = zero;
+    if (MODE == 1) {
+      bn_load_mu_is(stat64, mean, invstd, C, ct * 4, mu, is);
+      sc = *reinterpret_cast<const f32x4*>(msc + ct * 4);
+      sh = *reinterpret_cast<const f32x4*>(msh + ct * 4);
+    }
+    c1_walk(x, H, W, r0 + rt, rt_n, r1, [&](long long r) { return MODE == 1 ? *reinterpret_cast<const f32x4*>(da + r * ldda + ct * 4) : zero; },
+            [&](long long, const float (&xv)[3][3], const f32x4 v) {
+              const f32x4 yv = c1_preact(zero, wr, xv, 0, 0);
+#pragma unroll
+              for (int k = 0; k < 4; ++k) {
+                if (MODE == 0) bn_stats_acc(s0[k], s1[k], yv[k]);
+                else bn_bwd_acc(s0[k], s1[k], bn_masked_dz(v[k], false, 0.f, true, yv[k], sc[k], sh[k]), yv[k], mu[k], is[k]);
+              }
+            });
+  }
+  block_partials_store(sred, s0, s1, rt, rt_n, ct, C, ws);
+}
+
+__global__ __launch_bounds__(256) void c1_bn_bwd_wgrad_kernel(const float* __restrict__ x, const float* __restrict__ w, const float* __restrict__ da,
+                                                              int ldda, const float* __restrict__ msc, const float* __restrict__ msh,
+                                                              const double* __restrict__ k0, const double* __restrict__ k1,
+                                                              const double* __restrict__ k2, int B, int H, int W, int Co, int rt_n,
+                                                              int rows_per_thread, float* __restrict__ ws) {
+  const int ct = threadIdx.x % (Co / 4);
+  f32x4 wr[9];
+  c1_load_w(w, ct, wr);
+  const f32x4 sc = *reinterpret_cast<const f32x4*>(msc + ct * 4);
+  const f32x4 sh = *reinterpret_cast<const f32x4*>(msh + ct * 4);
+  double c0[4], c1[4], c2[4];
+#pragma unroll
+  for (int k = 0; k < 4; ++k) {
+    c0[k] = k0[ct * 4 + k];
+    c1[k] = k1[ct * 4 + k];
+    c2[k] = k2[ct * 4 + k];
+  }
+  const float* dac = da + ct * 4;
+  c1_wgrad_body(x, B, H, W, Co, rt_n, rows_per_thread, ws, [&](long long pix) { return *reinterpret_cast<const f32x4*>(dac + pix * ldda); },
+                [&](const f32x4 dz, const float (&xv)[3][3]) {
+    const f32x4 zero = {0.f, 0.f, 0.f, 0.f};
+    const f32x4 yv = c1_preact(zero, wr, xv, 0, 0);
+    f32x4 g;
+#pragma unroll
+    for (int k = 0; k < 4; ++k) g[k] = bn_dy(c0[k], c1[k], c2[k], bn_masked_dz(dz[k], false, 0.f, true, yv[k], sc[k], sh[k]), yv[k]);
+    return g;
+  });
 }
 
 __global__ void conv_c1_wgrad_finalize_kernel(const float* __restrict__ ws, int nblk, int Co, float* dw, float* db, int accumulate) {
@@ -634,6 +784,92 @@
   hipLaunchKernelGGL(conv_c1_wgrad_kernel, dim3(grid), dim3(256), lds, s, x, dy, lddy, B, H, W, Co, rt, rpt, (float*)workspace);
   hipLaunchKernelGGL(conv_c1_wgrad_finalize_kernel, dim3(qea_cdiv(10 * Co, 4)), dim3(256), 0, s, (const float*)workspace, grid, Co, dw, db,
                      accumulate);
+  QEA_CHECK_LAUNCH();
+  return QEA_OK;
+}
+
+static int c1_bn_check(const char* who, const float* x, const float* w, int B, int H, int W, int Co) {
+  QEA_REQUIRE(x && w && B > 0 && H > 0 && W > 0 && W % 4 == 0 && (Co == 32 || Co == 64 || Co == 128) && (long long)B * H * W < 0x7fffffffLL,
+              "%s: needs W %% 4 == 0, Co in {32, 64, 128}, fewer than 2^31 pixels", who);
+  return QEA_OK;
+}
+
+extern "C" size_t qea_c1_bn_stats_workspace_bytes(int32_t B, int32_t H, int32_t W, int32_t Co) {
+  if (B <= 0 || H <= 0 || W <= 0 || (Co != 32 && Co != 64 && Co != 128)) return 0;
+  return ws_need(col_geom((long long)B * H * W, Co).grid, 0, Co);
+}
+
+extern "C" int qea_c1_bn_stats(const float* x, const float* w, int32_t B, int32_t H, int32_t W, int32_t Co, const float* gamma, const float* beta,
+                               float eps, float momentum, float* running_mean, float* running_var, float* mean_out, float* invstd_out,
+                               float* scale_out, float* shift_out, double* stat64, void* workspace, size_t workspace_bytes, void* stream) {
+  if (int rc = c1_bn_check("qea_c1_bn_stats", x, w, B, H, W, Co)) return rc;
+  QEA_REQUIRE(mean_out && invstd_out && scale_out && shift_out, "qea_c1_bn_stats: null pointer");
+  const long long M = (long long)B * H * W;
+  const ColGeom g = col_geom(M, Co);
+  QEA_REQUIRE(workspace && workspace_bytes >= ws_need(g.grid, 0, Co), "qea_c1_bn_stats: workspace too small (%zu bytes)", ws_need(g.grid, 0, Co));
+  hipStream_t s = (hipStream_t)stream;
+  const size_t lds = (size_t)g.rt * Co * 2 * sizeof(double);
+  hipLaunchKernelGGL(c1_bn_reduce_kernel<0>, dim3(g.grid), dim3(RED_THREADS), lds, s, x, w, (const float*)nullptr, 0, (const float*)nullptr,
+                     (const float*)nullptr, (const double*)nullptr, (const float*)nullptr, (const float*)nullptr, B, H, W, Co, g.rows_per_block,
+                     g.rt, (double*)workspace);
+  hipLaunchKernelGGL(bn_stats_finalize_kernel, dim3(qea_cdiv(Co, 4)), dim3(256), 0, s, (const double*)workspace, g.grid, Co, M, gamma, beta, eps,
+                     momentum, running_mean, running_var, mean_out, invstd_out, scale_out, shift_out, stat64);
+  QEA_CHECK_LAUNCH();
+  return QEA_OK;
+}
+
+extern "C" int qea_c1_bn_apply(const float* x, const float* w, const float* scale, const float* shift, float* a, int32_t lda, int32_t B, int32_t H,
+                               int32_t W, int32_t Co, int32_t relu, float* absmax_out, void* stream) {
+  if (int rc = c1_bn_check("qea_c1_bn_apply", x, w, B, H, W, Co)) return rc;
+  QEA_REQUIRE(scale && shift && a && lda % 4 == 0 && lda >= Co && ((uintptr_t)a & 15) == 0 && ((uintptr_t)scale & 15) == 0 &&
+                  ((uintptr_t)shift & 15) == 0,
+              "qea_c1_bn_apply: needs scale, shift and a (16-byte aligned), lda %% 4 == 0, lda >= Co");
+  const int cols = Co / 4;
+  const long long groups = (long long)B * H * (W / 4);
+  const long long blocks = (groups + 256 / cols - 1) / (256 / cols);
+  const int grid = (int)(blocks > 16384 ? 16384 : blocks);
+  hipStream_t s = (hipStream_t)stream;
+  if (Co == 32) hipLaunchKernelGGL(c1_bn_apply_kernel<8>, dim3(grid), dim3(256), 0, s, x, w, scale, shift, a, lda, B, H, W, relu, absmax_out);
+  else if (Co == 64) hipLaunchKernelGGL(c1_bn_apply_kernel<16>, dim3(grid), dim3(256), 0, s, x, w, scale, shift, a, lda, B, H, W, relu, absmax_out);
+  else hipLaunchKernelGGL(c1_bn_apply_kernel<32>, dim3(grid), dim3(256), 0, s, x, w, scale, shift, a, lda, B, H, W, relu, absmax_out);
+  QEA_CHECK_LAUNCH();
+  return QEA_OK;
+}
+
+extern "C" size_t qea_c1_bn_bwd_workspace_bytes(int32_t B, int32_t H, int32_t W, int32_t Co) {
+  if (B <= 0 || H <= 0 || W <= 0 || (Co != 32 && Co != 64 && Co != 128)) return 0;
+  int rt, rpt;
+  const long long M = (long long)B * H * W;
+  return ws_need(col_geom(M, Co).grid, 3, Co) + (size_t)c1_wgrad_geom(M, Co, &rt, &rpt) * 10 * Co * sizeof(float);
+}
+
+extern "C" int qea_c1_bn_bwd(const float* da, int32_t ldda, const float* x, const float* w, const float* relu_scale, const float* relu_shift,
+                             int32_t B, int32_t H, int32_t W, int32_t Co, const float* gamma, const float* mean, const float* invstd,
+                             const double* stat64, int32_t training, float* dgamma, float* dbeta, int32_t accumulate_param_grads, float* dw,
+                             int32_t accumulate_dw, void* workspace, size_t workspace_bytes, void* stream) {
+  if (int rc = c1_bn_check("qea_c1_bn_bwd", x, w, B, H, W, Co)) return rc;
+  QEA_REQUIRE(da && relu_scale && relu_shift && mean && invstd && dw && ldda % 4 == 0 && ldda >= Co && ((uintptr_t)da & 15) == 0 &&
+                  ((uintptr_t)relu_scale & 15) == 0 && ((uintptr_t)relu_shift & 15) == 0,
+              "qea_c1_bn_bwd: needs da (16-byte aligned, ldda %% 4 == 0, ldda >= Co), relu_scale / relu_shift (16-byte aligned), mean, invstd, dw");
+  const long long M = (long long)B * H * W;
+  const ColGeom g = col_geom(M, Co);
+  int rt, rpt;
+  const int wgrid = c1_wgrad_geom(M, Co, &rt, &rpt);
+  const size_t need = ws_need(g.grid, 3, Co) + (size_t)wgrid * 10 * Co * sizeof(float);
+  QEA_REQUIRE(workspace && workspace_bytes >= need && ((uintptr_t)workspace & 7) == 0, "qea_c1_bn_bwd: workspace of %zu bytes (8-byte aligned) required",
+              need);
+  hipStream_t s = (hipStream_t)stream;
+  double* rows = (double*)workspace;
+  double *k0 = rows + (size_t)g.grid * Co * 2, *k1 = k0 + Co, *k2 = k1 + Co;
+  float* part = (float*)(k2 + Co);
+  hipLaunchKernelGGL(c1_bn_reduce_kernel<1>, dim3(g.grid), dim3(RED_THREADS), (size_t)g.rt * Co * 2 * sizeof(double), s, x, w, da, ldda, mean, invstd,
+                     stat64, relu_scale, relu_shift, B, H, W, Co, g.rows_per_block, g.rt, rows);
+  hipLaunchKernelGGL(bn_bwd_finalize_kernel, dim3(qea_cdiv(Co, 4)), dim3(256), 0, s, (const double*)rows, g.grid, Co, M, gamma, mean, invstd, stat64,
+                     training, dgamma, dbeta, accumulate_param_grads, k0, k1, k2);
+  hipLaunchKernelGGL(c1_bn_bwd_wgrad_kernel, dim3(wgrid), dim3(256), (size_t)rt * 10 * Co * sizeof(float), s, x, w, da, ldda, relu_scale, relu_shift,
+                     (const double*)k0, (const double*)k1, (const double*)k2, B, H, W, Co, rt, rpt, part);
+  hipLaunchKernelGGL(conv_c1_wgrad_finalize_kernel, dim3(qea_cdiv(10 * Co, 4)), dim3(256), 0, s, (const float*)part, wgrid, Co, dw, (float*)nullptr,
+                     accumulate_dw);
   QEA_CHECK_LAUNCH();
   return QEA_OK;
 }
diff --git a/query-efficient-approx-to-improve-ocr_amd/csrc/norm_pool.hip b/query-efficient-approx-to-improve-ocr_amd/csrc/norm_pool.hip
--- a/query-efficient-approx-to-improve-ocr_amd/csrc/norm_pool.hip
+++ b/query-efficient-approx-to-improve-ocr_amd/csrc/norm_pool.hip
@@ -1,72 +1,6 @@
-#include "common.h"
+#include "bn_core.h"
 
 namespace {
-
-constexpr int RED_THREADS = 256;
-
-struct ColGeom {
-  int cols;
-  int rt;
-  int grid;
-  int rows_per_block;
-};
-
-ColGeom col_geom(long long M, int C) {
-  ColGeom g;
-  g.cols = C / 4;
-  g.rt = RED_THREADS / g.cols;
-  if (g.rt < 1) g.rt = 1;
-  long long want = (M + (long long)g.rt * 16 - 1) / ((long long)g.rt * 16);
-  if (want > 1024) want = 1024;
-  if (want < 1) want = 1;
-  g.grid = (int)want;
-  g.rows_per_block = (int)((M + g.grid - 1) / g.grid);
-  g.grid = (int)((M + g.rows_per_block - 1) / g.rows_per_block);
-  return g;
-}
-
-__device__ __forceinline__ float bn_affine(float v, float sc, float sh) { return __fmaf_rn(v, sc, sh); }
-
-__device__ __forceinline__ float bn_masked_dz(float d, bool has_a, float av, bool remask = false, float yv = 0.f, float sc = 0.f, float sh = 0.f) {
-  if (has_a) return av > 0.f ? d : 0.f;
-  if (remask) return bn_affine(yv, sc, sh) > 0.f ? d : 0.f;
-  return d;
-}
-__device__ __forceinline__ void bn_bwd_acc(double& s0, double& s1, float dz, float yv, double mu, double is) {
-  s0 += (double)dz;
-  s1 += (double)dz * (((double)yv - mu) * is);
-}
-__device__ __forceinline__ float bn_dy(double c0, double c1, double c2, float dz, float yv) {
-  return (float)(c0 * (double)dz + (c1 * (double)yv + c2));
-}
-__device__ __forceinline__ void bn_load_mu_is(const double* __restrict__ stat64, const float* __restrict__ mean, const float* __restrict__ invstd,
-                                              int C, int c4, double (&mu)[4], double (&is)[4]) {
-#pragma unroll
-  for (int k = 0; k < 4; ++k) {
-    mu[k] = stat64 ? stat64[c4 + k] : (double)mean[c4 + k];
-    is[k] = stat64 ? stat64[C + c4 + k] : (double)invstd[c4 + k];
-  }
-}
-__device__ __forceinline__ void block_partials_store(double* sred, const double (&s0)[4], const double (&s1)[4], int rt, int rt_n, int ct, int C,
-                                                     double* __restrict__ ws) {
-  if (rt < rt_n) {
-#pragma unroll
-    for (int k = 0; k < 4; ++k) {
-      sred[((size_t)rt * C + ct * 4 + k) * 2 + 0] = s0[k];
-      sred[((size_t)rt * C + ct * 4 + k) * 2 + 1] = s1[k];
-    }
-  }
-  __syncthreads();
-  for (int c = threadIdx.x; c < C; c += blockDim.x) {
-    double t0 = 0, t1 = 0;
-    for (int r = 0; r < rt_n; ++r) {
-      t0 += sred[((size_t)r * C + c) * 2 + 0];
-      t1 += sred[((size_t)r * C + c) * 2 + 1];
-    }
-    ws[((size_t)blockIdx.x * C + c) * 2 + 0] = t0;
-    ws[((size_t)blockIdx.x * C + c) * 2 + 1] = t1;
-  }
-}
 
 __device__ __forceinline__ bool pool_take(float v, float m) { return v > m || v != v; }
 __device__ __forceinline__ long long pool_window_origin(long long op, int OW, int W, int kh, int kw) {
@@ -104,10 +38,7 @@
       const f32x4 v = *reinterpret_cast<const f32x4*>(x + r * ldx + ct * 4);
       if (MODE == 0) {
 #pragma unroll
-        for (int k = 0; k < 4; ++k) {
-          s0[k] += (double)v[k];
-          s1[k] += (double)v[k] * (double)v[k];
-        }
+        for (int k = 0; k < 4; ++k) bn_stats_acc(s0[k], s1[k], v[k]);
       } else if (MODE == 1) {
         const f32x4 yv = *reinterpret_cast<const f32x4*>(y + r * ldy + ct * 4);
         const f32x4 av = a ? *reinterpret_cast<const f32x4*>(a + r * lda + ct * 4) : zero;
@@ -121,47 +52,6 @@
     }
   }
   block_partials_store(sred, s0, s1, rt, rt_n, ct, C, ws);
-}
-
-__device__ __forceinline__ void partial_sums(const double* __restrict__ ws, int nblk, int C, int c, double& s, double& q) {
-  const int lane = threadIdx.x & 63;
-  double a = 0, b = 0;
-  for (int k = lane; k < nblk; k += 64) {
-    a += ws[((size_t)k * C + c) * 2 + 0];
-    b += ws[((size_t)k * C + c) * 2 + 1];
-  }
-  s = qea_wave_sum_d(a);
-  q = qea_wave_sum_d(b);
-}
-
-__global__ void bn_stats_finalize_kernel(const double* __restrict__ ws, int nblk, int C, long long M, const float* __restrict__ gamma,
-                                         const float* __restrict__ beta, float eps, float momentum, float* running_mean,
-                                         float* running_var, float* mean_out, float* invstd_out, float* scale_out, float* shift_out,
-                                         double* stat64) {
-  const int c = blockIdx.x * (blockDim.x >> 6) + (threadIdx.x >> 6);
-  if (c >= C) return;
-  double s, q;
-  partial_sums(ws, nblk, C, c, s, q);
-  if ((threadIdx.x & 63) != 0) return;
-  const double mean = s / (double)M;
-  double var = q / (double)M - mean * mean;
-  if (var < 0) var = 0;
-  const double invstd_d = 1.0 / sqrt(var + (double)eps);
-  if (stat64) {
-    stat64[c] = mean;
-    stat64[C + c] = invstd_d;
-  }
-  const float invstd = (float)invstd_d;
-  const float g = gamma ? gamma[c] : 1.f, b = beta ? beta[c] : 0.f;
-  mean_out[c] = (float)mean;
-  invstd_out[c] = invstd;
-  scale_out[c] = g * invstd;
-  shift_out[c] = b - (float)mean * g * invstd;
-  if (running_mean) {
-    const double unb = (M > 1) ? var * (double)M / (double)(M - 1) : var;
-    running_mean[c] = (1.f - momentum) * running_mean[c] + momentum * (float)mean;
-    running_var[c] = (1.f - momentum) * running_var[c] + momentum * (float)unb;
-  }
 }
 
 __global__ void bn_eval_coeff_kernel(int C, const float* __restrict__ gamma, const float* __restrict__ beta,
@@ -185,27 +75,6 @@
   partial_sums(ws, nblk, C, c, s, q);
   if ((threadIdx.x & 63) != 0) return;
   out[c] = accumulate ? out[c] + (float)s : (float)s;
-}
-
-__global__ void bn_bwd_finalize_kernel(const double* __restrict__ ws, int nblk, int C, long long M, const float* __restrict__ gamma,
-                                       const float* __restrict__ mean, const float* __restrict__ invstd,
-                                       const double* __restrict__ stat64, int training, float* dgamma, float* dbeta, int accumulate,
-                                       double* k0, double* k1, double* k2) {
-  const int c = blockIdx.x * (blockDim.x >> 6) + (threadIdx.x >> 6);
-  if (c >= C) return;
-  double s, q;
-  partial_sums(ws, nblk, C, c, s, q);
-  if ((threadIdx.x & 63) != 0) return;
-  if (dgamma) dgamma[c] = accumulate ? dgamma[c] + (float)q : (float)q;
-  if (dbeta) dbeta[c] = accumulate ? dbeta[c] + (float)s : (float)s;
-  const double g = gamma ? (double)gamma[c] : 1.0;
-  const double is = stat64 ? stat64[C + c] : (double)invstd[c];
-  const double mu = stat64 ? stat64[c] : (double)mean[c];
-  const double m0 = training ? s / (double)M : 0.0;
-  const double m1 = training ? q / (double)M : 0.0;
-  k0[c] = g * is;
-  k1[c] = -g * is * is * m1;
-  k2[c] = g * is * (mu * is * m1 - m0);
 }
 
 __global__ void bn_apply_kernel(const float* __restrict__ y, int ldy, float* __restrict__ a, int lda, long long M, int C,
@@ -488,8 +357,6 @@
     if (c < Cc && r < R) out[(size_t)c * R + r] = t[tx][j];
   }
 }
-
-size_t ws_need(int rows, int consts, int C) { return ((size_t)rows * 2 + consts) * C * sizeof(double); }
 
 int check_cols(const char* who, long long M, int C, int strides, const void* ws, size_t ws_bytes, int consts, ColGeom* g) {
   QEA_REQUIRE(M > 0 && C > 0 && C % 4 == 0 && C / 4 <= RED_THREADS, "%s: need C %% 4 == 0 and C <= %d (C=%d)", who, 4 * RED_THREADS, C);
diff --git a/query-efficient-approx-to-improve-ocr_amd/qea/batchnorm.py b/query-efficient-approx-to-improve-ocr_amd/qea/batchnorm.py
--- a/query-efficient-approx-to-improve-ocr_amd/qea/batchnorm.py
+++ b/query-efficient-approx-to-improve-ocr_amd/qea/batchnorm.py
@@ -20,8 +20,9 @@
 
 class Stage:
 
-    def __init__(self, y, h, w, C, parts, coef, stat64, training):
+    def __init__(self, y, h, w, C, parts, coef, stat64, training, src=None):
         self.y, self.h, self.w, self.C, self.parts, self.coef, self.stat64, self.training = y, h, w, C, parts, coef, stat64, training
+        self.src = src
 
     @property
     def single(self):
@@ -31,13 +32,16 @@
         per = per or self.h * self.w
         return t[b0 * per:(b0 + nb) * per] if t is not None else None
 
+    def source(self, b0, nb):
+        return (self.src[0][b0:b0 + nb], self.src[1]) if self.src is not None else None
+
     def restricted(self, b0, nb):
         g = self.parts.index((b0, nb)) if self.training else 0
         return Stage(self.rows(self.y, b0, nb), self.h, self.w, self.C, [(0, nb)], self.coef[g:g + 1],
-                     self.stat64[g:g + 1] if self.stat64 is not None else None, self.training)
+                     self.stat64[g:g + 1] if self.stat64 is not None else None, self.training, self.source(b0, nb))
 
     def producer_sums(self):
-        have = self.training and self.single and self.stat64 is not None
+        have = self.training and self.single and self.stat64 is not None and self.y is not None
         return (self.y, self.C, self.stat64[0], self.coef[0, 2], self.coef[0, 3]) if have else None
 
 
@@ -47,26 +51,33 @@
     return coef[2], coef[3]
 
 
-def forward(y, out, ldo, h, w, C, gamma, beta, running_mean, running_var, training, parts, keep, amax=None, partials=None, pool=None):
+def forward(y, out, ldo, h, w, C, gamma, beta, running_mean, running_var, training, parts, keep, amax=None, partials=None, pool=None, src=None):
+    if src is not None and (y is not None or partials is not None or pool is not None):
+        raise ValueError("a stage rebuilt from its source has no y, no partials from a producer and no fused pool")
     if not training:
         parts = [(0, sum(nb for _, nb in parts))]
     if partials is not None and len(parts) > 1:
         raise ValueError("statistics from the conv's partials cover the whole batch: one statistics group only")
-    coef = torch.empty(len(parts), 4, C, device=y.device)
-    stat64 = torch.empty(len(parts), 2, C, device=y.device, dtype=torch.float64) if (training and keep) else None
-    st = Stage(y, h, w, C, parts, coef, stat64, training)
+    coef = torch.empty(len(parts), 4, C, device=out.device)
+    stat64 = torch.empty(len(parts), 2, C, device=out.device, dtype=torch.float64) if (training and keep) else None
+    st = Stage(y, h, w, C, parts, coef, stat64, training, src)
     for g, (b0, nb) in enumerate(parts):
         mean, invstd, scale, shift = coef[g]
         yg, s64 = st.rows(y, b0, nb), stat64[g] if stat64 is not None else None
         if not training:
             ops.bn_eval_coeff(C, gamma, beta, running_mean, running_var, BN_EPS, None, mean, invstd, scale, shift)
+        elif src is not None:
+            ops.c1_bn_stats(*st.source(b0, nb), nb, h, w, C, gamma, beta, BN_EPS, BN_MOMENTUM, running_mean, running_var, mean, invstd,
+                            scale, shift, s64)
         elif partials is not None:
             ops.bn_train_stats_from_partials(partials[0], partials[1], nb * h * w, C, gamma, beta, BN_EPS, BN_MOMENTUM, running_mean,
                                              running_var, mean, invstd, scale, shift, s64)
         else:
             ops.bn_train_stats(yg, C, nb * h * w, C, gamma, beta, BN_EPS, BN_MOMENTUM, running_mean, running_var, mean, invstd, scale,
                                shift, s64)
-        if pool is not None:
+        if src is not None:
+            ops.c1_bn_apply(*st.source(b0, nb), scale, shift, st.rows(out, b0, nb), ldo, nb, h, w, C, relu=True, amax=amax)
+        elif pool is not None:
             pooled, ldp, kh, kw, pooled_amax = pool
             ops.bn_apply_pool(yg, C, st.rows(out, b0, nb), ldo, st.rows(pooled, b0, nb, (h // kh) * (w // kw)), ldp, nb, h, w, C, scale,
                               shift, kh, kw, relu=True, amax=amax, pooled_amax=pooled_amax)
@@ -75,11 +86,24 @@
     return st, pool is not None
 
 
-def backward(st, da, ldda, dy, gamma, dgamma, dbeta, amax=None, partials=None, pool=None):
+def backward(st, da, ldda, dy, gamma, dgamma, dbeta, amax=None, partials=None, pool=None, dw=None):
+    y = st.y
+    if st.src is not None:
+        if dy is not None or dw is None or partials is not None or pool is not None:
+            raise ValueError("a stage rebuilt from its source yields dw, not dy, and takes neither partials nor a pool")
+        x, wt = st.src
+        if st.single:
+            mean, invstd, scale, shift = st.coef[0]
+            ops.c1_bn_bwd(da, ldda, x, wt, scale, shift, x.shape[0], st.h, st.w, st.C, gamma, mean, invstd, st.training, dgamma, dbeta, dw,
+                          accumulate=True, accumulate_dw=True, stat64=st.stat64[0] if st.stat64 is not None else None)
+            return
+        y = torch.empty(x.shape[0] * st.h * st.w, st.C, device=x.device)
+        ops.conv_c1_fwd(x, wt, None, y, st.C, x.shape[0], st.h, st.w, st.C, relu=False)
+        dy = torch.empty_like(y)
     for g, (b0, nb) in enumerate(st.parts):
         mean, invstd, scale, shift = st.coef[g]
         rest = dict(accumulate=True, stat64=st.stat64[g] if st.stat64 is not None else None, relu_scale=scale, relu_shift=shift, amax=amax)
-        yg, dyg = st.rows(st.y, b0, nb), st.rows(dy, b0, nb)
+        yg, dyg = st.rows(y, b0, nb), st.rows(dy, b0, nb)
         if pool is not None:
             dpool, lddp, kw = pool
             ops.bn_bwd_pool(st.rows(da, b0, nb), ldda, st.rows(dpool, b0, nb, (st.h // 2) * (st.w // kw)), lddp, kw, yg, st.C, nb, st.h, st.w,
@@ -87,3 +111,5 @@
         else:
             ops.bn_bwd(st.rows(da, b0, nb), ldda, None, 0, yg, st.C, nb * st.h * st.w, st.C, gamma, mean, invstd, st.training, dgamma, dbeta,
                        dyg, st.C, partials=partials, **rest)
+    if st.src is not None:
+        ops.conv_c1_wgrad(x, dy, st.C, dw, None, x.shape[0], st.h, st.w, st.C, accumulate=True)
diff --git a/query-efficient-approx-to-improve-ocr_amd/qea/ops.py b/query-efficient-approx-to-improve-ocr_amd/qea/ops.py
--- a/query-efficient-approx-to-improve-ocr_amd/qea/ops.py
+++ b/query-efficient-approx-to-improve-ocr_amd/qea/ops.py
@@ -573,6 +573,28 @@
                                    ws.data_ptr(), ws.numel(), _stream()), "qea_conv_c1_wgrad")
 
 
+def c1_bn_stats(x, w, B, H, W, Co, gamma, beta, eps, momentum, running_mean, running_var, mean, invstd, scale, shift, stat64=None):
+    L = _lib.lib()
+    ws = workspace(L.qea_c1_bn_stats_workspace_bytes(B, H, W, Co), x.device)
+    _lib.check(L.qea_c1_bn_stats(_ptr(x), _ptr(w), B, H, W, Co, _ptr(gamma), _ptr(beta), eps, momentum, _ptr(running_mean), _ptr(running_var),
+                                 _ptr(mean), _ptr(invstd), _ptr(scale), _ptr(shift), _ptr(stat64), ws.data_ptr(), ws.numel(), _stream()),
+               "qea_c1_bn_stats")
+
+
+def c1_bn_apply(x, w, scale, shift, a, lda, B, H, W, Co, relu=True, amax=None):
+    _lib.check(_lib.lib().qea_c1_bn_apply(_ptr(x), _ptr(w), _ptr(scale), _ptr(shift), _ptr(a), lda, B, H, W, Co, int(relu), _ptr(amax), _stream()),
+               "qea_c1_bn_apply")
+
+
+def c1_bn_bwd(da, ldda, x, w, relu_scale, relu_shift, B, H, W, Co, gamma, mean, invstd, training, dgamma, dbeta, dw, accumulate=False,
+              accumulate_dw=False, stat64=None):
+    L = _lib.lib()
+    ws = workspace(L.qea_c1_bn_bwd_workspace_bytes(B, H, W, Co), x.device)
+    _lib.check(L.qea_c1_bn_bwd(_ptr(da), ldda, _ptr(x), _ptr(w), _ptr(relu_scale), _ptr(relu_shift), B, H, W, Co, _ptr(gamma), _ptr(mean),
+                               _ptr(invstd), _ptr(stat64), int(training), _ptr(dgamma), _ptr(dbeta), int(accumulate), _ptr(dw),
+                               int(accumulate_dw), ws.data_ptr(), ws.numel(), _stream()), "qea_c1_bn_bwd")
+
+
 def conv_c1_dgrad(dy, lddy, w, dx, B, H, W, Co, accumulate=False):
     _lib.check(_lib.lib().qea_conv_c1_dgrad(_ptr(dy), lddy, _ptr(w), _ptr(dx), B, H, W, Co, int(accumulate), _stream()),
                "qea_conv_c1_dgrad")
diff --git a/query-efficient-approx-to-improve-ocr_amd/qea/unet_engine.py b/query-efficient-approx-to-improve-ocr_amd/qea/unet_engine.py
--- a/query-efficient-approx-to-improve-ocr_amd/qea/unet_engine.py
+++ b/query-efficient-approx-to-improve-ocr_amd/qea/unet_engine.py
@@ -7,6 +7,19 @@
 FUSE_BN_BWD_SUMS = True
 FUSE_BN_POOL = True
 FUSE_POOL_BWD = True
+C1_REBUILD_MIN_BYTES = 32 << 20
+
+
+class _BlockRecord(dict):
+
+    def __missing__(self, key):
+        if key != "y1" or self["bn1"].src is None:
+            raise KeyError(key)
+        c1, (x, w) = self["c1"], self["bn1"].src
+        y = torch.empty(c1.B * c1.H * c1.W, c1.N, device=x.device)
+        ops.conv_c1_fwd(x, w, None, y, c1.N, c1.B, c1.H, c1.W, c1.N, relu=False)
+        self[key] = y
+        return y
 
 
 class _Block:
@@ -41,6 +54,8 @@
                 fused_pool = (pool[0], cout, 2, pool[1])
             cv.fwd(x, ldx, w, out, ldo, scale=scale, bias=shift, relu=True, x_amax=x_amax, y_amax=out_amax, pool=fused_pool)
             return None, fused_pool is not None
+        if cin == 1 and pool is None and W % 4 == 0 and cout in (32, 64, 128) and B * H * W * cout * 4 >= C1_REBUILD_MIN_BYTES:
+            return batchnorm.forward(None, out, ldo, H, W, cout, *bn, training, parts, keep, amax=out_amax, src=(x, w))
         y = torch.empty(B * H * W, cout, device=x.device)
         fused = None
         if cin == 1:
@@ -70,9 +85,12 @@
             bn1, _ = self._conv_bn_relu(P, Bf, blk, 1, xin, ldx, c1, a1, blk.cout, training, need_grad, parts, xin_amax, a1_amax)
             bn2, pooled_here = self._conv_bn_relu(P, Bf, blk, 2, a1, blk.cout, c2, out, ldo, training, need_grad, parts, a1_amax, out_amax, pool)
             if need_grad:
-                ctx["blocks"][blk.mod] = {"xin": xin, "ldx": ldx, "c1": c1, "c2": c2, "h": h, "w": w, "a1": a1, "out": out, "ldo": ldo,
-                                          "bn1": bn1, "bn2": bn2, "xin_amax": xin_amax, "a1_amax": a1_amax,
-                                          "y1": bn1.y, "y2": bn2.y}
+                rec = _BlockRecord({"xin": xin, "ldx": ldx, "c1": c1, "c2": c2, "h": h, "w": w, "a1": a1, "out": out, "ldo": ldo,
+                                    "bn1": bn1, "bn2": bn2, "xin_amax": xin_amax, "a1_amax": a1_amax,
+                                    "y1": bn1.y, "y2": bn2.y})
+                if bn1.y is None:
+                    del rec["y1"]
+                ctx["blocks"][blk.mod] = rec
             return pooled_here
 
         cats, cat_amax = {}, {}
@@ -140,6 +158,10 @@
             da1 = torch.empty(M, cout, device=dev)
             bst = s["bn1"].producer_sums() if FUSE_BN_BWD_SUMS else None
             part = c2.dgrad(dy2, cout, P[blk.key(2, "w")], da1, cout, x_amax=dy2_amax, bwd_stats=bst)
+            if s["bn1"].src is not None:
+                batchnorm.backward(s["bn1"], da1, cout, None, P[blk.key(1, "gamma")], G[blk.key(1, "gamma")], G[blk.key(1, "beta")],
+                                   dw=G[blk.key(1, "w")])
+                return None
             dy1 = torch.empty(M, cout, device=dev)
             batchnorm.backward(s["bn1"], da1, cout, dy1, P[blk.key(1, "gamma")], G[blk.key(1, "gamma")], G[blk.key(1, "beta")], amax=dy1_amax,
                                partials=part if bst is not None else None)
```

Measured after the change: 22810 patch-images/s, median of 3. Within noise of the previous version (+0.5%).
